# JADGardner/RENI

Hardware: AMD Instinct MI355X
Metric: directional-samples/sec (fwd+bwd), 128x256 equirect, ND=36 latent (higher is better)
Workload: dtype bf16

## Files before the change

### reni_amd/csrc/reni_capi.inc

```
#include <dlfcn.h>

#include <cmath>
#include <cstdarg>
#include <cstdio>
#include <cstdlib>
#include <atomic>
#include <cstring>
#include <mutex>
#include <new>
#include <string>
#include <vector>

#include "../../include/reni_hip.h"

struct reni_plan {
  reni_desc d;
  int F_in;
  int64_t n_params;
  int64_t n_first;
  unsigned p_off_w[reni::MAX_LAYERS + 2];
  unsigned p_off_b[reni::MAX_LAYERS + 2];
  int M_in, N_out;
  int64_t n_map_params;
  unsigned mw_off[reni::MAX_MAP_LAYERS + 1], mb_off[reni::MAX_MAP_LAYERS + 1];
  int no_persist, no_side_stream, dw1_old;
  int no_l0x;
  int env_overrides;
  size_t frag_ws_cap;
};

namespace {

thread_local std::string g_err;

std::atomic<long long> g_launches{0};
thread_local hipEvent_t g_ev_rest = nullptr;
#define RENI_LAUNCH(...) do { g_launches.fetch_add(1, std::memory_order_relaxed); hipLaunchKernelGGL(__VA_ARGS__); HIP_TRY(hipGetLastError()); } while (0)

int fail(int code, const char* fmt, ...) {
  char buf[512];
  va_list ap;
  va_start(ap, fmt);
  vsnprintf(buf, sizeof(buf), fmt, ap);
  va_end(ap);
  g_err = buf;
  return code;
}

#define HIP_TRY(expr)                                                                      \
  do {                                                                                     \
    hipError_t e_ = (expr);                                                                \
    if (e_ != hipSuccess) return fail(RENI_EHIP, "%s failed: %s", #expr, hipGetErrorString(e_)); \
  } while (0)

size_t al256(size_t x) { return (x + 255) & ~(size_t)255; }
size_t al1k(size_t x) { return (x + 1023) & ~(size_t)1023; }

bool has_persistent(int dtype, int H, int L) {
  return dtype == RENI_BF16 && H == 128 && L >= 1 && L <= 5;
}
bool has_wide(int dtype, int H, int L, uint32_t flags, bool film, bool backward) {
  if (film && (backward || L > 5)) return false;
  return dtype == RENI_BF16 && H == 256 && L >= 2 && L <= reni::MAX_LAYERS - 1 && !(flags & RENI_NEED_DW);
}
bool has_wide_train(int dtype, int H, int L, uint32_t flags, bool film) {
  if (film) return dtype == RENI_BF16 && H == 256 && L >= 2 && L <= 4;
  return dtype == RENI_BF16 && H == 256 && L >= 2 && L <= reni::MAX_LAYERS - 1 && (flags & RENI_NEED_DW);
}

int device_cus() {
  int dev = 0, n = 0;
  if (hipGetDevice(&dev) != hipSuccess) return 256;
  if (hipDeviceGetAttribute(&n, hipDeviceAttributeMultiprocessorCount, dev) != hipSuccess || n <= 0) return 256;
  return n;
}

struct GeoRt {
  int img_hid, img_hf, img_hb, bias_hid, bias_head, lds_bytes, stash_layer_bytes, nks, nrb, head_bwd_ks;
};

template <class Pol, int H>
GeoRt geo_of() {
  using G = reni::Geo<Pol, H>;
  return {G::IMG_HID, G::IMG_HF, G::IMG_HB, G::BIAS_HID, G::BIAS_HEAD, G::LDS_BYTES, G::STASH_LAYER_BYTES,
          G::NKS, G::NRB, Pol::HEAD_BWD_KS};
}

bool geo_for(const reni_plan* p, GeoRt* g) {
  const int H = p->d.hidden_features;
  if (p->d.dtype == RENI_F32) {
    if (H == 32) *g = geo_of<reni::PolF32, 32>();
    else if (H == 64) *g = geo_of<reni::PolF32, 64>();
    else if (H == 128) *g = geo_of<reni::PolF32, 128>();
    else if (H == 256) *g = geo_of<reni::PolF32, 256>();
    else return false;
  } else {
    if (H == 32) *g = geo_of<reni::PolBF16, 32>();
    else if (H == 64) *g = geo_of<reni::PolBF16, 64>();
    else if (H == 128) *g = geo_of<reni::PolBF16, 128>();
    else if (H == 256) *g = geo_of<reni::PolBF16, 256>();
    else return false;
  }
  return true;
}

struct Layout {
  int tpi, n_tiles, nwg, persist, stream, kmax, frag;
  int wide_train;
  int pdw;
  int consistent_bwd;
  size_t o_tflag, o_tlist, o_tcount, o_imgcos;
  size_t o_pcnt, o_pscan, o_plist, o_nlive;
  size_t o_skip;
  size_t o_idxc, o_Zc, o_A, o_afrag, o_xconst, o_wimg, o_stash, o_dwp, o_dA_part, o_loss_part, o_img_loss, o_stats, o_dA, o_g1, o_dw1p, o_part2, o_mcol, o_ucol, o_dfp, o_dws, o_dfr, o_runimg, o_pruns, o_prunimg, total;
  int pkmax;
  int nch, rt_chunk;
  size_t stash_per_wg, dwp_per_wg;
  unsigned fwd_off[reni::MAX_LAYERS + 2], bwd_off[reni::MAX_LAYERS + 2];
  size_t wimg_bytes;
};

Layout make_layout(const reni_plan* p, const GeoRt& g, int64_t B, int64_t P, uint32_t flags, bool backward,
                   bool allow_persist = true, int stage = 0) {
  Layout l;
  memset(&l, 0, sizeof(l));
  const int H = p->d.hidden_features, L = p->d.hidden_layers;
  l.tpi = (int)((P + 127) / 128);
  l.n_tiles = (int)(B * l.tpi);
  const bool film = p->d.conditioning == RENI_COND_FILM;
  l.wide_train = (backward && allow_persist && !p->no_persist && has_wide_train(p->d.dtype, H, L, flags, film)) ? 1 : 0;
  l.persist = (allow_persist && !p->no_persist && (has_persistent(p->d.dtype, H, L) || has_wide(p->d.dtype, H, L, flags, film, backward) || l.wide_train)) ? 1 : 0;
  l.pdw = (l.persist && !l.wide_train && (film || (flags & RENI_NEED_DW))) ? 1 : 0;
  l.consistent_bwd = (l.persist && !film && backward) ? 1 : 0;
  const int per_cu = (p->d.dtype == RENI_BF16 && !l.persist && H <= 128) ? 2 : 1;
  const int cap = device_cus() * per_cu;
  l.nwg = l.n_tiles < cap ? l.n_tiles : cap;
  if (l.pdw && l.n_tiles > cap) {
    const int rounds = (l.n_tiles + cap - 1) / cap;
    l.nwg = (l.n_tiles + rounds - 1) / rounds;
  }
  if (l.nwg < 1) l.nwg = 1;
  size_t o = 0;
  for (int st = 0; st < 2; ++st) {
    const bool mine = st == stage;
    if (mine) l.o_idxc = o;
    o += al256((size_t)B * 8);
    if (mine) l.o_Zc = o;
    o += al256((size_t)B * p->d.ndims * 3 * 4);
    if (mine) l.o_A = o;
    o += al256((size_t)B * H * 8 * 4);
    if (mine) l.o_afrag = o;
    if (l.persist) o += al256((size_t)B * (H / 32) * 1024);
    if (mine) l.o_xconst = o;
    o += al256((size_t)B * p->F_in * 4);
  }
  size_t w = 0;
  for (int i = 1; i <= L; ++i) { l.fwd_off[i] = (unsigned)w; w += al1k((size_t)g.img_hid + g.bias_hid); }
  l.fwd_off[L + 1] = (unsigned)w; w += al1k((size_t)g.img_hf + g.bias_head);
  for (int i = 1; i <= L; ++i) { l.bwd_off[i] = (unsigned)w; w += al1k((size_t)g.img_hid); }
  l.bwd_off[L + 1] = (unsigned)w; w += al1k((size_t)g.img_hb);
  l.wimg_bytes = w;
  w += 8192;
  l.o_wimg = o; o += al256(w);
  l.o_skip = o; o += 256;
  l.o_img_loss = o; o += al256((size_t)B * 16 * 4);
  l.o_stats = o; o += al256((size_t)B * 16 * 4);
  if (backward) {
    l.stash_per_wg = (size_t)(L + 1) * g.stash_layer_bytes * ((l.persist && !l.pdw && !l.wide_train) ? 2 : 1);
    l.frag = (p->d.dtype == RENI_BF16 && H == 256 && L >= 1 && (film || (flags & RENI_NEED_DW))) ? 1 : 0;
    if (p->d.dtype == RENI_F32 && H == 256 && L >= 1 && !film && (flags & RENI_NEED_DW)) l.frag = 2;
    l.o_stash = o; o += al256(l.stash_per_wg * (l.frag ? (size_t)l.n_tiles : (size_t)l.nwg));
    l.dwp_per_wg = (flags & RENI_NEED_DW) ? (size_t)(p->n_params - p->n_first) : 0;
    if (l.pdw) l.dwp_per_wg = (l.dwp_per_wg + 63) & ~(size_t)63;
    l.pkmax = ((l.n_tiles + l.nwg - 1) / l.nwg + l.tpi - 1) / l.tpi + 1;
    const size_t run_slots = (film && l.persist && !l.wide_train) ? (size_t)l.pkmax : 1;
    l.o_dwp = o; o += al256(l.dwp_per_wg * 4 * l.nwg * run_slots);
    l.o_dA_part = o; if (!l.pdw) o += al256((size_t)l.n_tiles * H * 8 * 4);
    l.o_tflag = l.o_tlist = l.o_tcount = l.o_imgcos = o;
    if (!film && !(flags & RENI_NEED_DW)) {
      l.o_tflag = o; o += al256((size_t)l.n_tiles * 4);
      l.o_tlist = o; o += al256((size_t)2 * l.n_tiles * 4);
      l.o_tcount = o; o += 256;
      l.o_imgcos = o; o += al256((size_t)B * 4);
      l.o_pcnt = o; o += al256((size_t)l.n_tiles * 4);
      l.o_pscan = o; o += al256((size_t)(l.n_tiles + 1) * 4);
      l.o_nlive = o; o += al256((size_t)B * 4);
      l.o_plist = o; o += al256((size_t)B * P * 4);
    }
    l.o_loss_part = o; o += al256((size_t)l.n_tiles * 4 * 16 * 4);
    l.o_dA = o; o += al256((size_t)B * H * 8 * 4);
    l.o_dw1p = o; if (l.pdw && (flags & RENI_NEED_DW)) o += al256((size_t)2 * l.nwg * run_slots * ((size_t)H * H + H) * 4);
    l.o_g1 = o; if (l.pdw) o += al256((size_t)((l.n_tiles + l.nwg - 1) / l.nwg) * l.nwg * (H / 16) * 4096);
    l.o_pruns = o; if (l.pdw) o += al256((size_t)l.nwg * l.pkmax * (H * 8 + 16) * 4);
    l.o_prunimg = o; if (l.pdw) o += al256((size_t)l.nwg * l.pkmax * (film ? 3 : 1) * 4);
    l.rt_chunk = reni::RT_CHUNK;
    l.nch = (l.tpi + l.rt_chunk - 1) / l.rt_chunk;
    l.o_part2 = o; o += al256((size_t)B * l.nch * (H * 8 + 16) * 4);
    l.o_mcol = o; o += al256((size_t)B * p->F_in * 4);
    l.o_ucol = o; o += al256((size_t)B * p->d.ndims * 3 * 4);
    l.o_dfp = o; if (film && !l.persist) o += al256((size_t)l.n_tiles * L * 2 * H * 4);
    const bool can = p->d.dtype == RENI_BF16 && L >= 1;
    l.stream = can && (H == 128 || H == 256) && (!l.persist || l.wide_train) && (film || (flags & RENI_NEED_DW)) ? 1 : 0;
    l.o_dws = o;
    l.o_dfr = o;
    l.o_runimg = o;
    if (l.frag == 2) o += al256((size_t)L * l.n_tiles * g.stash_layer_bytes);
    if (l.stream) {
      const int nround = (H == 256) ? 2 : 1;
      const size_t rec = (size_t)2 * (H == 256 ? 36864 : 34816);
      o += al256(l.frag ? (size_t)L * l.n_tiles * g.stash_layer_bytes + (l.wide_train ? (size_t)l.n_tiles * 2048 : 0)
                        : (size_t)L * l.n_tiles * nround * rec);
      const long long nrec = (long long)l.n_tiles * nround;
      const long long range = (nrec + l.nwg - 1) / l.nwg;
      l.kmax = (int)(range / ((long long)l.tpi * nround)) + 2;
      if (film) {
        l.o_dfr = o; o += al256((size_t)l.nwg * l.kmax * L * 2 * H * 4);
        l.o_runimg = o; o += al256((size_t)l.nwg * l.kmax * 4);
      }
    }
    if (film && l.persist && !l.wide_train) {
      l.o_dfr = o; o += al256((size_t)3 * l.nwg * l.pkmax * L * 2 * H * 4);
      l.o_runimg = l.o_prunimg;
    }
  }
  l.total = o;
  return l;
}

Layout backward_layout(const reni_plan* p, const GeoRt& g, int64_t B, int64_t P, uint32_t flags) {
  return make_layout(p, g, B, P, flags | RENI_NEED_DZ, true, true);
}

enum { PROF_FWD_BWD = 0, PROF_STATS = 1, PROF_FWD = 2, PROF_DW1 = 3, PROF_DWS = 4, PROF_COMM = 5 };
struct EvPair { hipEvent_t a, b; int kind; };
bool g_prof_on = false;
std::vector<EvPair> g_prof_pool;
size_t g_prof_used = 0;

bool prof_begin(hipStream_t s, EvPair* out, int kind) {
  if (!g_prof_on) return false;
  if (g_prof_used == g_prof_pool.size()) {
    EvPair e;
    if (hipEventCreate(&e.a) != hipSuccess || hipEventCreate(&e.b) != hipSuccess) return false;
    g_prof_pool.push_back(e);
  }
  g_prof_pool[g_prof_used].kind = kind;
  *out = g_prof_pool[g_prof_used++];
  return hipEventRecord(out->a, s) == hipSuccess;
}

template <class Go>
int timed_launch(hipStream_t s, int kind, const char* what, Go go) {
  EvPair ev;
  const bool timed = prof_begin(s, &ev, kind);
  g_launches.fetch_add(1, std::memory_order_relaxed);
  const hipError_t e = go();
  if (e != hipSuccess) return fail(RENI_EHIP, "%s launch failed: %s", what, hipGetErrorString(e));
  if (timed) HIP_TRY(hipEventRecord(ev.b, s));
  return RENI_OK;
}
int timed_launch(void (*fn)(const reni::MainArgs), int grid, int block, int lds, hipStream_t s, const reni::MainArgs& a, int kind) {
  if (lds) HIP_TRY(hipFuncSetAttribute((const void*)fn, hipFuncAttributeMaxDynamicSharedMemorySize, lds));
  return timed_launch(s, kind, "kernel", [&] { hipLaunchKernelGGL(fn, dim3(grid), dim3(block), lds, s, a); return hipGetLastError(); });
}

bool spec_head(bool need_dw, int last_linear, int act) { return need_dw && last_linear && act == RENI_ACT_TANH; }
bool train_spec(const reni::MainArgs& a, bool stats) {
  return !stats && spec_head(a.need_dw, a.last_linear, a.act) && a.loss_kind == 0 && a.out == nullptr;
}

int launch_train(const reni_plan* p, const reni::MainArgs& a, int nwg, hipStream_t s, bool stats = false, bool l0x = false) {
  using G = reni::GeoP<128>;
  const int kind = !stats ? PROF_FWD_BWD : a.target ? PROF_STATS : PROF_FWD;
  const bool film = p->d.conditioning == RENI_COND_FILM;
  if (p->d.hidden_features == 256) {
    if (film && p->d.hidden_layers > (stats ? reni::wide256_film_max_layers() : reni::wide256_film_train_max_layers()))
      return fail(RENI_EINVAL, "internal: k_reni_wide256's FiLM instances hold <= 5 (forward) / <= 4 (training form) hidden layers' tables");
    if ((a.need_dw || film) && !stats && a.gfs == nullptr) return fail(RENI_EINVAL, "internal: the training form of k_reni_wide256 needs the fragment stream");
    const int mode = film ? (stats ? 3 : 4) : stats ? 0 : a.need_dw ? 2 : 1;
    return timed_launch(s, kind, "k_reni_wide256", [&] { return reni::launch_wide256(mode, a, nwg, s); });
  }
  if (!has_persistent(p->d.dtype, p->d.hidden_features, p->d.hidden_layers))
    return fail(RENI_EUNSUPPORTED, "no persistent training kernel for this configuration");
  if (p->d.hidden_layers >= 2 && (a.fwd_off[2] - a.fwd_off[1] != G::FWD_STRIDE || a.bwd_off[2] - a.bwd_off[1] != G::BWD_STRIDE))
    return fail(RENI_EINVAL, "packed weight images are not at the stride the persistent kernels assume");
  const bool spec = train_spec(a, stats);
  const int pairs = (a.n_tiles + 1) / 2, nwg2 = nwg < pairs ? nwg : pairs;
  if (film)
    return timed_launch(s, kind, "FiLM persistent kernel", [&] { return reni::launch_train_film(stats ? 1 : spec ? 2 : 0, a, stats ? nwg2 : nwg, s); });
  if (l0x && !spec) return fail(RENI_EINVAL, "internal: the L0X form exists for the SPEC instance only");
  void (*fn)(const reni::MainArgs) = stats ? reni::k_reni_train_bf16<128, false, true>
                                     : l0x ? reni::k_reni_train_bf16<128, true, false, false, true, true>
                                     : spec ? reni::k_reni_train_bf16<128, true, false, false, true>
                                     : a.need_dw ? reni::k_reni_train_bf16<128, true> : reni::k_reni_train_bf16<128, false>;
  const int lacc = spec ? G::LACC_BYTES + (l0x ? G::L0X_TW_BYTES : 0) : 0;
#ifdef RENI_TRACE
  const int LDS = G::LDS_BYTES + lacc + 4096;
#else
  const int LDS = G::LDS_BYTES + lacc;
#endif
  if (a.need_dw && !stats) return timed_launch(fn, nwg, 256, LDS, s, a, kind);
  return timed_launch(fn, nwg2, 512, LDS, s, a, kind);
}

bool dw1_ring_plan_ok(const reni_plan* p, int64_t P) { return !p->dw1_old && p->d.conditioning != RENI_COND_FILM && P % 128 == 0; }
bool dw1_ring_call_ok(const reni::MainArgs& a) { return (((uintptr_t)a.D | (uintptr_t)(a.d_bstride * 4)) & 15) == 0; }
int dw1_slots(bool ring, int nwg) { return ring ? nwg : 2 * nwg; }
bool l0x_rows_ok(const float* base, long long s0, long long s1, long long s2) {
  if (((uintptr_t)base | (uintptr_t)(s0 * 4)) & 15) return false;
  if (s1 == 3 && s2 == 1) return true;
  return s1 == 1 && ((uintptr_t)(s2 * 4) & 15) == 0;
}
bool l0x_plan_ok(const reni_plan* p, const Layout& l, int64_t P, uint32_t flags) {
  const int L = p->d.hidden_layers;
  return l.pdw && !p->no_l0x && dw1_ring_plan_ok(p, P) && spec_head(flags & RENI_NEED_DW, p->d.last_layer_linear, p->d.output_activation) &&
         L >= 3 && (L & 1) == 1;
}
bool l0x_call_ok(const reni::MainArgs& a) {
  return dw1_ring_call_ok(a) && train_spec(a, false) && l0x_rows_ok(a.target, a.ts0, a.ts1, a.ts2) && l0x_rows_ok(a.weight, a.ws0, a.ws1, a.ws2);
}
bool side_stream_plan_ok(const reni_plan* p, const Layout& l) { return l.pdw && !p->no_side_stream; }

int launch_dw1(const reni::MainArgs& a, int nwg, bool ring, hipStream_t s, bool l0x = false) {
#ifdef RENI_TRACE_DW1
  constexpr int TRACE = 8192;
#else
  constexpr int TRACE = 0;
#endif
  if (l0x)
    return timed_launch(reni::k_reni_l0_ring<128>, nwg, reni::L0Ring::THREADS, reni::L0Ring::LDS_BYTES + TRACE, s, a, PROF_DW1);
  if (a.film != nullptr) return timed_launch(s, PROF_DW1, "k_reni_dw1 (FiLM)", [&] { return reni::launch_dw1_film(a, 2 * nwg, s); });
  if (ring)
    return timed_launch(reni::k_reni_dw1_ring<128>, nwg, reni::Dw1Ring::THREADS, reni::Dw1Ring::LDS_BYTES + TRACE, s, a, PROF_DW1);
  return timed_launch(reni::k_reni_dw1<128>, 2 * nwg, 256, 2 * reni::TS_BYTES + TRACE, s, a, PROF_DW1);
}

int reduce_partials(const float* part, size_t per_wg, int nslot, float* out, int lo, int hi, const int* valid, const reni::LayerScale& lsc,
                    hipStream_t s, int quad_H = 0) {
  if (quad_H > 0) {
    if (valid != nullptr || (per_wg & 3) || (lo & 3) || ((uintptr_t)part & 15)) return fail(RENI_EINVAL, "internal: quad-row partials need untagged, 16-byte aligned slots");
    RENI_LAUNCH(reni::k_reduce_partials_quad, dim3((unsigned)((hi - lo + reni::QUAD_BLK_WORDS - 1) / reni::QUAD_BLK_WORDS)), dim3(256), 0, s, part, per_wg, nslot, out, lo, hi, quad_H, lsc);
    return RENI_OK;
  }
  RENI_LAUNCH(reni::k_reduce_partials, dim3((unsigned)((hi - lo + 63) / 64)), dim3(256), 0, s, part, per_wg, nslot, out, lo, hi, valid, lsc);
  return RENI_OK;
}

struct SideStream { hipStream_t s; hipEvent_t ev[3]; bool ok; };
std::mutex g_side_mu;
SideStream* side_stream() {
  static SideStream tab[16];
  static std::mutex mu;
  int dev = 0;
  if (hipGetDevice(&dev) != hipSuccess || dev < 0 || dev >= 16) return nullptr;
  std::lock_guard<std::mutex> lk(mu);
  SideStream& t = tab[dev];
  if (!t.ok) {
    if (hipStreamCreateWithFlags(&t.s, hipStreamNonBlocking) != hipSuccess) return nullptr;
    for (int i = 0; i < 3; ++i)
      if (hipEventCreateWithFlags(&t.ev[i], hipEventDisableTiming) != hipSuccess) return nullptr;
    t.ok = true;
  }
  return &t;
}

int launch_main(const reni_plan* p, int mode, const reni::MainArgs& a, int nwg, hipStream_t s) {
  const int H = p->d.hidden_features;
  const bool film = p->d.conditioning == RENI_COND_FILM, f32 = p->d.dtype == RENI_F32;
  return timed_launch(s, mode == reni::MODE_FWD_BWD ? PROF_FWD_BWD : mode == reni::MODE_STATS ? PROF_STATS : PROF_FWD, "fused kernel", [&] {
    if (f32) return film ? reni::launch_film_f32(H, mode, a, nwg, s) : reni::launch_main_f32(H, mode, a, nwg, s);
    return film ? reni::launch_film_bf16(H, mode, a, nwg, s) : reni::launch_main_bf16(H, mode, a, nwg, s);
  });
}

struct DeviceGuard {
  int prev = -1;
  bool switched = false;
  int enter(const void* ptr) {
    hipPointerAttribute_t at;
    if (hipPointerGetAttributes(&at, ptr) == hipSuccess) {
      if (hipGetDevice(&prev) == hipSuccess && prev != at.device) {
        HIP_TRY(hipSetDevice(at.device));
        switched = true;
      }
    } else {
      (void)hipGetLastError();
    }
    return RENI_OK;
  }
  ~DeviceGuard() {
    if (switched) (void)hipSetDevice(prev);
  }
};

int run_prologue(const reni_plan* p, const GeoRt& g, const Layout& l, int64_t B, const float* Z,
                 const float* params, char* ws, bool backward, hipStream_t s, const int64_t* idx = nullptr,
                 const float* film_A = nullptr, int64_t n_rows = 0) {
  const int H = p->d.hidden_features, L = p->d.hidden_layers;
  const bool film = p->d.conditioning == RENI_COND_FILM;
  reni::PrepArgs pa;
  memset(&pa, 0, sizeof(pa));
  if (!film) {
    pa.idx = (const long long*)idx; pa.n_rows = (long long)n_rows; pa.Zc = (float*)(ws + l.o_Zc);
    pa.idx_copy = idx ? (long long*)(ws + l.o_idxc) : nullptr;
    pa.Z = Z; pa.W0 = params; pa.b0 = params + (size_t)H * p->F_in;
    pa.xconst = (float*)(ws + l.o_xconst); pa.A = (float*)(ws + l.o_A);
    pa.afrag = l.persist ? ws + l.o_afrag : nullptr;
    pa.afrag_scale = p->d.first_omega_0 * 0.15915494309189535f;
    pa.eq = p->d.equivariance; pa.nd = p->d.ndims; pa.F_in = p->F_in; pa.H = H;
  }

  reni::PackArgs ka;
  ka.params = params; ka.wimg = ws + l.o_wimg;
  int n = 0;
  for (int i = 1; i <= L + 1; ++i) {
    const bool head = (i == L + 1);
    reni::PackDesc d;
    d.src = p->p_off_w[i]; d.bias_src = p->p_off_b[i]; d.dst = l.fwd_off[i];
    d.M = head ? 3 : H; d.K = H; d.transposed = 0;
    d.nrb = head ? 1 : g.nrb; d.nks = g.nks;
    d.bias_n = head ? 3 : H; d.bias_n_pad = head ? 32 : H;
    d.scale = (l.persist && !head && !film) ? p->d.hidden_omega_0 * 0.15915494309189535f : 1.f;
    if (film && l.persist && H == 256 && !head) d.scale = 0.15915494309189535f;
    ka.d[n++] = d;
    if (backward) {
      d.dst = l.bwd_off[i]; d.transposed = 1;
      d.nrb = g.nrb; d.nks = head ? g.head_bwd_ks : g.nks;
      d.bias_n = 0; d.bias_n_pad = 0;
      d.scale = !l.persist ? 1.f : film ? ((i == 1 || H == 256) ? 1.f : 6.283185307179586f) : (i == 1 ? p->d.first_omega_0 : p->d.hidden_omega_0);
      if (l.consistent_bwd) d.scale = (head ? 1.f : p->d.hidden_omega_0 * 0.15915494309189535f) * 8.f;
      ka.d[n++] = d;
    }
  }
  const bool f32 = p->d.dtype == RENI_F32;
  if (!film || l.persist) {
    reni::PrologueArgs ga;
    memset(&ga, 0, sizeof(ga));
    ga.prep = pa;
    ga.prep_gy = (H + 7) / 8; ga.n_prep = (int)B * ga.prep_gy; ga.pack_gx = f32 ? 16 : 8;
    if (film) {
      ga.film_A = film_A; ga.film_afrag = ws + l.o_afrag; ga.film_scale = 0.15915494309189535f; ga.film_B = (int)B;
      ga.prep.H = H; ga.n_prep = (int)((B * H + 255) / 256);
    }
    const unsigned grid = (unsigned)(ga.n_prep + ga.pack_gx * n);
    if (f32) RENI_LAUNCH(reni::k_prologue<reni::PolF32>, dim3(grid), dim3(256), (size_t)p->F_in * 4, s, ga, ka);
    else RENI_LAUNCH(reni::k_prologue<reni::PolBF16>, dim3(grid), dim3(256), (size_t)p->F_in * 4, s, ga, ka);
    return RENI_OK;
  }
  if (f32) RENI_LAUNCH(reni::k_pack<reni::PolF32>, dim3(16, n), dim3(256), 0, s, ka);
  else RENI_LAUNCH(reni::k_pack<reni::PolBF16>, dim3(8, n), dim3(256), 0, s, ka);
  return RENI_OK;
}

void fill_main_args(reni::MainArgs& a, const reni_plan* p, const Layout& l, int64_t B, int64_t P,
                    const float* Z, const float* D, int64_t dbs, char* ws) {
  memset(&a, 0, sizeof(a));
  a.B = (int)B; a.P = (int)P; a.tiles_per_image = l.tpi; a.n_tiles = l.n_tiles;
  a.L = p->d.hidden_layers; a.last_linear = p->d.last_layer_linear; a.act = p->d.output_activation;
  a.w_first = p->d.first_omega_0; a.w_hidden = p->d.hidden_omega_0;
  a.gy_scale = 1.f;
  if (l.consistent_bwd) {
    double sc = (double)p->d.first_omega_0 / 8.0;
    for (int i = 0; i < p->d.hidden_layers; ++i) sc *= 6.283185307179586 / 8.0;
    a.gy_scale = (float)sc;
  }
  a.Z = Z; a.D = D; a.d_bstride = dbs;
  a.Apre = (const float*)(ws + l.o_A);
  a.afrag = ws + l.o_afrag;
  a.wimg = ws + l.o_wimg;
  for (int i = 0; i < reni::MAX_LAYERS + 2; ++i) {
    a.fwd_off[i] = l.fwd_off[i]; a.bwd_off[i] = l.bwd_off[i];
    a.p_off_w[i] = p->p_off_w[i] >= (unsigned)p->n_first ? p->p_off_w[i] - (unsigned)p->n_first : 0;
    a.p_off_b[i] = p->p_off_b[i] >= (unsigned)p->n_first ? p->p_off_b[i] - (unsigned)p->n_first : 0;
  }
  a.stash = ws + l.o_stash; a.stash_per_wg = l.stash_per_wg;
  a.dwp = (float*)(ws + l.o_dwp); a.dwp_per_wg = l.dwp_per_wg;
  a.dA_part = (float*)(ws + l.o_dA_part);
  a.loss_part = (float*)(ws + l.o_loss_part);
  a.g1 = ws + l.o_g1;
  a.dw1p = (float*)(ws + l.o_dw1p);
  a.stats = (const float*)(ws + l.o_stats);
  a.n_first = (unsigned)p->n_first;
  a.dfp_part = (float*)(ws + l.o_dfp);
  a.dws = l.stream ? ws + l.o_dws : nullptr;
  a.gfs = l.frag ? ws + l.o_dws : nullptr;
  a.dfr = (float*)(ws + l.o_dfr);
  a.run_image = (int*)(ws + l.o_runimg);
  a.kmax = l.kmax;
  a.pruns = (float*)(ws + l.o_pruns);
  a.prun_image = (int*)(ws + l.o_prunimg);
  a.pkmax = l.pkmax;
  a.nwg_main = l.nwg;
}

int check_common(const reni_plan* p, int64_t B, int64_t P, const void* Z, const void* D, const void* params,
                 const void* ws) {
  if (!p) return fail(RENI_EINVAL, "plan is NULL");
  if (B < 1 || P < 1) return fail(RENI_EINVAL, "B=%lld P=%lld must be >= 1", (long long)B, (long long)P);
  if (B * ((P + 127) / 128) > 0x3fffffffLL || P > 0x3fffffffLL) return fail(RENI_EINVAL, "problem too large");
  if (!Z || !D || !params) return fail(RENI_EINVAL, "Z, D and params must be non-NULL");
  if (!ws) return fail(RENI_EWORKSPACE, "workspace is NULL");
  if (((uintptr_t)ws & 255) != 0) return fail(RENI_EINVAL, "workspace must be 256-byte aligned");
  return RENI_OK;
}

struct FilmIO {
  const float* A = nullptr;
  const float* film = nullptr;
  float* dA = nullptr;
  float* dfilm = nullptr;
  const float* Zp = nullptr;
  float alpha = 0.f;
  int64_t nz = 0;
  int keep_first = 0;
};

int check_film(const reni_plan* p, const FilmIO* f, bool backward) {
  if (!p) return fail(RENI_EINVAL, "plan is NULL");
  if (p->d.conditioning != RENI_COND_FILM) return fail(RENI_EINVAL, "plan was not created with RENI_COND_FILM");
  if (!f->A) return fail(RENI_EINVAL, "A is NULL");
  if (p->d.hidden_layers > 0 && !f->film) return fail(RENI_EINVAL, "film is NULL");
  if (backward && (!f->dA || (p->d.hidden_layers > 0 && !f->dfilm))) return fail(RENI_EINVAL, "dA / dfilm is NULL");
  return RENI_OK;
}

int rccl_allreduce_inplace(void* comm, float* buf, size_t n, hipStream_t s);
int rccl_allreduce_max_i32(void* comm, int* buf, size_t n, hipStream_t s);

struct ListLayout { size_t o_hdr, o_tflag, o_tlist, o_tcount, o_imgcos, o_pcnt, o_pscan, o_nlive, o_plist, o_zstats, total; };
ListLayout make_list_layout(int64_t B, int64_t P) {
  ListLayout l;
  const size_t n_tiles = (size_t)(B * ((P + 127) / 128));
  size_t o = 0;
  l.o_hdr = o; o += 256;
  l.o_tflag = o; o += al256(n_tiles * 4);
  l.o_tlist = o; o += al256(2 * n_tiles * 4);
  l.o_tcount = o; o += 256;
  l.o_imgcos = o; o += al256((size_t)B * 4);
  l.o_pcnt = o; o += al256(n_tiles * 4);
  l.o_pscan = o; o += al256((n_tiles + 1) * 4);
  l.o_nlive = o; o += al256((size_t)B * 4);
  l.o_plist = o; o += al256((size_t)B * P * 4);
  l.o_zstats = o; o += al256((size_t)B * 16 * 4);
  l.total = o;
  return l;
}
constexpr long long LIST_MAGIC = 0x52454e494c495354ll;
struct ListDst { int *tflag, *imgcos, *tlist, *tcount, *pcnt, *pscan, *nlive, *plist; };
template <class L>
ListDst list_dst(char* base, const L& l) {
  return {(int*)(base + l.o_tflag), (int*)(base + l.o_imgcos), (int*)(base + l.o_tlist), (int*)(base + l.o_tcount),
          (int*)(base + l.o_pcnt), (int*)(base + l.o_pscan), (int*)(base + l.o_nlive), (int*)(base + l.o_plist)};
}
int build_weight_lists(const float* weight, const int64_t* wst, int64_t P, int tpi, int n_tiles, bool compact, const ListDst& d,
                       hipStream_t s) {
  RENI_LAUNCH(reni::k_tile_flags, dim3((unsigned)((n_tiles + 3) / 4)), dim3(256), 0, s, weight, (long long)wst[0], (long long)wst[1],
              (long long)wst[2], (int)P, tpi, n_tiles, d.tflag, d.imgcos, compact ? d.pcnt : (int*)nullptr);
  RENI_LAUNCH(reni::k_tile_compact, dim3(1), dim3(1024), 0, s, d.tflag, (const int*)d.imgcos, tpi, n_tiles, d.tlist, d.tlist + n_tiles,
              d.tcount, compact ? (const int*)d.pcnt : (const int*)nullptr, (int)P, d.pscan, d.nlive);
  if (compact) {
    RENI_LAUNCH(reni::k_pix_scatter, dim3((unsigned)((n_tiles + 3) / 4)), dim3(256), 0, s, weight, (long long)wst[0], (long long)wst[1],
                (long long)wst[2], (int)P, tpi, n_tiles, (const int*)d.imgcos, (const int*)d.pscan, d.plist);
  }
  return RENI_OK;
}
struct WeightLists { const char* buf; uint32_t flags; };
struct ListRecord { const void* buf; int64_t B, P; uint32_t mode; };
std::mutex g_lists_mu;
std::vector<ListRecord> g_lists;
void lists_remember(const void* buf, int64_t B, int64_t P, uint32_t mode) {
  std::lock_guard<std::mutex> lk(g_lists_mu);
  for (size_t i = 0; i < g_lists.size(); ++i)
    if (g_lists[i].buf == buf) { g_lists.erase(g_lists.begin() + (long)i); break; }
  g_lists.insert(g_lists.begin(), ListRecord{buf, B, P, mode});
  if (g_lists.size() > 64) g_lists.pop_back();
}
int lists_check(const void* buf, int64_t B, int64_t P, uint32_t mode, ListRecord* found) {
  std::lock_guard<std::mutex> lk(g_lists_mu);
  for (const ListRecord& r : g_lists)
    if (r.buf == buf) { *found = r; return (r.B == B && r.P == P && r.mode == mode) ? 0 : 2; }
  return 1;
}

struct StepFuse {
  void* comm = nullptr;
  int overlap = 0;
  float* params; float* table;
  float *m_dec, *v_dec, *m_lat, *v_lat;
  float lr, b1, b2, eps, bc1, bc2_sqrt, gscale;
  const int64_t* idx_next;
  uint32_t* state;
};

constexpr int LOSS_DOUT = 2;
struct BwdCall {
  int64_t B = 0, P = 0;
  const float *Z = nullptr, *D = nullptr, *params = nullptr;
  int64_t dbs = 0;
  const float *target = nullptr, *weight = nullptr, *dout = nullptr;
  const int64_t *ts = nullptr, *wst = nullptr;
  int loss_kind = RENI_LOSS_MSE;
  float alpha = 0.f, beta = 0.f;
  uint32_t flags = 0;
  float *out = nullptr, *loss_terms = nullptr, *dZ = nullptr, *dparams = nullptr;
  void* ws = nullptr;
  size_t ws_bytes = 0;
  void* stream = nullptr;
  const FilmIO* fio = nullptr;
  const int64_t* idx = nullptr;
  int64_t n_rows = 0;
  const StepFuse* fuse = nullptr;
  const WeightLists* lists = nullptr;
};

struct BwdPath {
  bool staged;
  int stage;
  bool use_cos;
  bool sparse;
  bool compact;
  bool cos_const;
  bool dw1_ring;
  bool l0x;
  bool part_quad;
  bool fork;
  bool early_rest;
  bool dp_early;
  bool fused_tail;
  bool fuse_on;
  bool fpers;
  bool red2;
  int n_rest;
  int n_l1;
  bool rp_in_tail;
  bool ev_rest_done;
  bool dp_early_done;
};

struct Bwd {
  const reni_plan* p;
  const BwdCall& c;
  GeoRt g; Layout l; reni::MainArgs a;
  char* ws;
  hipStream_t s, se;
  const float* Z;
  int stage_in;
  float *img_loss, *stats, *dA, *part2;
  ListDst ld;
  reni::LayerScale lsc;
  BwdPath path;
};

bool call_uses_cos(const BwdCall& c) { return c.loss_kind == RENI_LOSS_TEST && c.beta != 0.f; }

BwdPath bwd_path(const reni_plan* p, const Layout& l, const BwdCall& c, const reni::MainArgs& a, int stage_in) {
  BwdPath t{};
  const int H = p->d.hidden_features, L = p->d.hidden_layers;
  const bool need_dw = (c.flags & RENI_NEED_DW) != 0;
  t.staged = stage_in >= 0;
  t.stage = t.staged ? stage_in : 0;
  t.n_rest = (int)(p->n_params - p->n_first);
  t.n_l1 = H * H + H;
  t.use_cos = call_uses_cos(c);
  t.sparse = (c.flags & (RENI_WEIGHT_SPARSE | RENI_WEIGHT_COMPACT)) && !c.fio && !need_dw && c.loss_kind != LOSS_DOUT &&
             c.weight != nullptr && c.out == nullptr;
  t.compact = t.sparse && (c.flags & RENI_WEIGHT_COMPACT);
  t.cos_const = t.sparse && c.lists && (c.lists->flags & RENI_WEIGHT_COS_CONSTANT);
  t.dw1_ring = dw1_ring_plan_ok(p, c.P) && dw1_ring_call_ok(a);
  t.l0x = l0x_plan_ok(p, l, c.P, c.flags) && l0x_call_ok(a);
  t.part_quad = t.l0x;
  t.fork = side_stream_plan_ok(p, l) && !t.l0x && (c.fio || l.n_tiles >= 8 * l.nwg);
  t.early_rest = l.pdw && !c.fio && need_dw && L >= 1 && t.n_rest > t.n_l1;
  t.dp_early = c.fuse && c.fuse->comm && c.fuse->overlap;
  t.fused_tail = l.pdw && !c.fio;
  t.fuse_on = c.fuse && !c.fuse->comm && t.fused_tail && need_dw && (c.flags & RENI_NEED_DZ) && L >= 1;
  t.fpers = l.persist && !l.wide_train;
  t.red2 = L > 0 && t.fpers && need_dw;
  return t;
}

int bwd_validate(Bwd& x) {
  const reni_plan* p = x.p; const BwdCall& c = x.c;
  if (const int rc = c.fio ? check_film(p, c.fio, true) : RENI_OK) return rc;
  if (!c.fio && p && p->d.conditioning != RENI_COND_CONCAT) return fail(RENI_EINVAL, "FiLM plan: use the reni_film_* entry points");
  if (const int rc = check_common(p, c.B, c.P, c.fio ? c.fio->A : c.Z, c.D, c.params, c.ws)) return rc;
  if ((c.flags & RENI_NEED_DW) && !c.dparams) return fail(RENI_EINVAL, "RENI_NEED_DW set but dparams is NULL");
  if (!c.fio && (c.flags & RENI_NEED_DZ) && !c.dZ) return fail(RENI_EINVAL, "RENI_NEED_DZ set but dZ is NULL");
  if (c.loss_kind == LOSS_DOUT) {
    if (!c.dout) return fail(RENI_EINVAL, "dout is NULL");
  } else {
    if (c.loss_kind != RENI_LOSS_MSE && c.loss_kind != RENI_LOSS_TEST) return fail(RENI_EINVAL, "unknown loss_kind %d", c.loss_kind);
    if (!c.target || !c.weight || !c.ts || !c.wst) return fail(RENI_EINVAL, "target/weight (and their strides) must be non-NULL");
    if (!c.loss_terms) return fail(RENI_EINVAL, "loss_terms is NULL");
  }
  if (!geo_for(p, &x.g)) return fail(RENI_EUNSUPPORTED, "hidden_features=%d unsupported", p->d.hidden_features);
  return RENI_OK;
}

int bwd_layout(Bwd& x) {
  const BwdCall& c = x.c;
  const bool staged = c.fuse && (*c.fuse->state & 1u);
  x.stage_in = staged ? (int)((*c.fuse->state >> 1) & 1u) : -1;
  x.l = make_layout(x.p, x.g, c.B, c.P, c.flags, true, true, staged ? x.stage_in : 0);
  const Layout& l = x.l;
  if (c.ws_bytes < l.total) return fail(RENI_EWORKSPACE, "workspace too small: need %zu bytes, got %zu", l.total, c.ws_bytes);
  if (c.fuse) *c.fuse->state = 0;
  x.ws = (char*)c.ws;
  x.s = x.se = (hipStream_t)c.stream;
  x.Z = c.idx ? (const float*)(x.ws + l.o_Zc) : c.Z;
  x.img_loss = (float*)(x.ws + l.o_img_loss); x.stats = (float*)(x.ws + l.o_stats);
  x.dA = c.fio ? c.fio->dA : (float*)(x.ws + l.o_dA); x.part2 = (float*)(x.ws + l.o_part2);
  return RENI_OK;
}

void bwd_layer_scales(Bwd& x) {
  const reni_plan* p = x.p; reni::LayerScale& lsc = x.lsc;
  lsc.n_hid = p->d.hidden_features * p->d.hidden_features + p->d.hidden_features; lsc.L = p->d.hidden_layers;
  for (int i = 0; i <= reni::MAX_LAYERS; ++i) lsc.c[i] = 1.f;
  if (x.l.consistent_bwd && (x.c.flags & RENI_NEED_DW)) {
    double gy = (double)p->d.first_omega_0 / 8.0, cl = (double)p->d.hidden_omega_0 / (double)p->d.first_omega_0;
    for (int i = 0; i < p->d.hidden_layers; ++i) {
      gy *= 6.283185307179586 / 8.0;
      cl *= 8.0 / 6.283185307179586;
      lsc.c[i] = (float)cl;
    }
    lsc.c[p->d.hidden_layers] = (float)(1.0 / gy);
  }
}

void bwd_main_args(Bwd& x) {
  const BwdCall& c = x.c; reni::MainArgs& a = x.a;
  fill_main_args(a, x.p, x.l, c.B, c.P, x.Z, c.D, c.dbs, x.ws);
  if (c.fio) { a.Apre = c.fio->A; a.film = c.fio->film; a.params = c.params; a.Z = nullptr; }
  a.need_dw = (c.flags & RENI_NEED_DW) ? 1 : 0;
#ifdef RENI_DEBUG
  if (const char* e = getenv("RENI_DEBUG_MASK")) a.dbg = c.fio ? 0 : atoi(e);
#endif
#if defined(RENI_TRACE) || defined(RENI_TRACE_DW1)
  if (const char* e = getenv("RENI_TRACE_PTR")) a.trace = (long long*)strtoull(e, nullptr, 0);
#endif
  a.out = c.out; a.dout = c.dout; a.beta = c.beta;
  if (c.loss_kind != LOSS_DOUT) {
    a.target = c.target; a.ts0 = c.ts[0]; a.ts1 = c.ts[1]; a.ts2 = c.ts[2];
    a.weight = c.weight; a.ws0 = c.wst[0]; a.ws1 = c.wst[1]; a.ws2 = c.wst[2];
  }
  a.loss_kind = (c.loss_kind == LOSS_DOUT) ? LOSS_DOUT : (call_uses_cos(c) ? 1 : 0);
  x.path = bwd_path(x.p, x.l, c, a, x.stage_in);
}

int bwd_weight_lists(Bwd& x) {
  const BwdCall& c = x.c; const BwdPath& path = x.path; reni::MainArgs& a = x.a;
  if (!path.sparse) return RENI_OK;
  if (c.lists) {
    x.ld = list_dst(const_cast<char*>(c.lists->buf), make_list_layout(c.B, c.P));
  } else {
    x.ld = list_dst(x.ws, x.l);
    if (const int rc = build_weight_lists(c.weight, c.wst, c.P, x.l.tpi, x.l.n_tiles, path.compact, x.ld, x.s)) return rc;
  }
  a.tlist = x.ld.tlist; a.tcount = x.ld.tcount;
  if (path.compact) { a.plist = x.ld.plist; a.nlive = x.ld.nlive; }
  if (path.cos_const) a.stats = x.stats = (float*)(const_cast<char*>(c.lists->buf) + make_list_layout(c.B, c.P).o_zstats);
  return RENI_OK;
}

int bwd_stats_pass(Bwd& x) {
  const BwdCall& c = x.c; const Layout& l = x.l;
  if (!x.path.use_cos || x.path.cos_const) return RENI_OK;
  reni::MainArgs st = x.a;
  st.out = nullptr; st.loss_kind = 0;
  if (x.path.sparse) { st.tlist = x.a.tlist + l.n_tiles; st.tcount = x.a.tcount + 1; }
  if (const int rc = l.persist ? launch_train(x.p, st, l.nwg, x.s, true) : launch_main(x.p, reni::MODE_STATS, st, l.nwg, x.s)) return rc;
  RENI_LAUNCH(reni::k_stats_image, dim3((unsigned)c.B), dim3(256), 0, x.s, (const float*)x.a.loss_part, l.tpi, c.weight, (long long)c.wst[0],
                     (long long)c.wst[2], c.beta, x.img_loss, x.stats, (const int*)x.ld.imgcos);
  return RENI_OK;
}

struct SideJoin {
  SideStream* side = nullptr;
  hipStream_t s = nullptr;
  ~SideJoin() { if (side && hipEventRecord(side->ev[2], side->s) == hipSuccess) (void)hipStreamWaitEvent(s, side->ev[2], 0); }
};

int bwd_fork_dw1(Bwd& x, std::unique_lock<std::mutex>& side_lock, SideJoin& side_join) {
  const reni_plan* p = x.p; const BwdCall& c = x.c; const Layout& l = x.l; BwdPath& path = x.path; hipStream_t s = x.s;
  if (!l.pdw) return RENI_OK;
  SideStream* side = path.fork ? side_stream() : nullptr;
  if (side) {
    side_lock.lock();
    HIP_TRY(hipEventRecord(side->ev[0], s));
    HIP_TRY(hipStreamWaitEvent(side->s, side->ev[0], 0));
    x.se = side->s;
    side_join.side = side; side_join.s = s;
  }
  path.rp_in_tail = path.early_rest && !side && !g_ev_rest && !path.dp_early;
  if (path.early_rest && !path.rp_in_tail) {
    int rc = reduce_partials(x.a.dwp, l.dwp_per_wg, l.nwg, c.dparams + p->n_first, path.n_l1, path.n_rest, nullptr, x.lsc, s, path.part_quad ? p->d.hidden_features : 0);
    if (rc) return rc;
    if (g_ev_rest) { HIP_TRY(hipEventRecord(g_ev_rest, s)); path.ev_rest_done = true; }
    if (path.dp_early) {
      SideStream* cs = side_stream();
      if (!cs) return fail(RENI_EHIP, "no communication stream");
      if (!side_lock.owns_lock()) side_lock.lock();
      HIP_TRY(hipEventRecord(cs->ev[1], s));
      HIP_TRY(hipStreamWaitEvent(cs->s, cs->ev[1], 0));
      rc = rccl_allreduce_inplace(c.fuse->comm, c.dparams + p->n_first + path.n_l1, (size_t)(path.n_rest - path.n_l1), cs->s);
      if (rc) return rc;
      if (!side_join.side) { side_join.side = cs; side_join.s = s; }
      path.dp_early_done = true;
    }
  }
  return launch_dw1(x.a, l.nwg, path.dw1_ring, s, path.l0x);
}

int bwd_dw_consumers(Bwd& x) {
  const Layout& l = x.l; const reni::MainArgs& a = x.a; hipStream_t s = x.s;
  const int H = x.p->d.hidden_features;
  if (l.frag == 2) {
    const int lds = 4 * ((reni::Geo<reni::PolF32, 256>::T_BYTES + 1023) & ~1023);
    if (const int rc = timed_launch(reni::k_dw_frag32<256>, l.nwg, 256, lds, s, a, PROF_DWS)) return rc;
  }
  if (l.wide_train && (x.c.flags & RENI_NEED_DW)) {
    if (const int rc = timed_launch(s, PROF_DWS, "k_wide_head_dw", [&] { return reni::launch_wide_head_dw(a, l.nwg, s); })) return rc;
  }
  if (l.stream) {
    static_assert(reni::Geo<reni::PolBF16, 256>::T_BYTES_AL == 36864 && reni::Geo<reni::PolBF16, 128>::T_BYTES_AL == 34816,
                  "stream record sizes (make_layout)");
    const bool film = x.c.fio != nullptr;
    void (*fn)(const reni::MainArgs) = nullptr;
    if (H == 256) fn = film ? reni::k_dw_frag<256, true> : reni::k_dw_frag<256, false>;
    else fn = film ? reni::k_dw_stream<128, true> : reni::k_dw_stream<128, false>;
    if (film) HIP_TRY(hipMemsetAsync(a.run_image, 0xff, (size_t)l.nwg * l.kmax * 4, s));
    return timed_launch(fn, l.nwg, 256, 4 * (H == 256 ? 36864 : 34816), s, a, PROF_DWS);
  }
  return RENI_OK;
}

int bwd_image_sums(Bwd& x) {
  const BwdCall& c = x.c; const Layout& l = x.l; const reni::MainArgs& a = x.a;
  const int H = x.p->d.hidden_features;
  if (x.path.fused_tail) return RENI_OK;
  if (l.pdw) {
    RENI_LAUNCH(reni::k_reduce_runs, dim3((unsigned)c.B, c.B < 16 ? (unsigned)((H * 8 + 16 + 63) / 64) : 1u), dim3(256), 0, x.se, (const float*)a.pruns, (const int*)a.prun_image,
                       l.nwg, l.pkmax, H, l.tpi, l.n_tiles, x.dA, x.img_loss);
    return RENI_OK;
  }
  RENI_LAUNCH(reni::k_reduce_tiles_a, dim3((unsigned)c.B, (unsigned)l.nch), dim3(256), 0, x.se, (const float*)a.dA_part,
                     (const float*)a.loss_part, l.tpi, H, x.part2, 1, l.rt_chunk, (const int*)x.ld.tflag);
  RENI_LAUNCH(reni::k_reduce_tiles_b, dim3((unsigned)c.B, (unsigned)((H * 8 + 16 + 255) / 256)), dim3(256), 0, x.se, (const float*)x.part2, l.nch, H, x.dA, x.img_loss, 1);
  return RENI_OK;
}

int bwd_epilogue_film(Bwd& x) {
  const reni_plan* p = x.p; const BwdCall& c = x.c; const Layout& l = x.l; const BwdPath& path = x.path; const reni::MainArgs& a = x.a;
  hipStream_t s = x.s, se = x.se;
  const int H = p->d.hidden_features, L = p->d.hidden_layers;
  if (path.red2) {
  } else if (L > 0 && (l.stream || path.fpers)) {
    RENI_LAUNCH(reni::k_reduce_film_runs, dim3((unsigned)c.B, (unsigned)((L * H + 255) / 256)), dim3(256), 0, s, a, H,
                       path.fpers ? 3 * l.nwg * l.pkmax : l.nwg * l.kmax, c.fio->dfilm);
  } else if (L > 0) {
    RENI_LAUNCH(reni::k_reduce_film, dim3((unsigned)c.B, (unsigned)((L * 2 * H + 255) / 256)), dim3(256), 0, s,
                       (const float*)a.dfp_part, l.tpi, L * 2 * H, c.fio->dfilm);
  }
  if (c.flags & RENI_NEED_DW) {
    if (!c.fio->keep_first) HIP_TRY(hipMemsetAsync(c.dparams, 0, (size_t)p->n_first * 4, s));
    if (path.fpers) {
      const int n_l1 = path.n_l1, nslot = l.nwg * l.pkmax;
      reni::FilmReduce2 r2;
      r2.H = H; r2.nruns = 3 * l.nwg * l.pkmax; r2.B = (int)c.B; r2.gy = (L * H + 255) / 256; r2.dfilm = c.fio->dfilm;
      r2.part = a.dw1p; r2.per_wg = (size_t)n_l1; r2.nslot = 2 * nslot; r2.dparams = c.dparams + p->n_first; r2.n = n_l1;
      r2.valid = (const int*)a.prun_image + nslot;
      RENI_LAUNCH(reni::k_film_reduce2, dim3((unsigned)(r2.B * r2.gy + (n_l1 + 63) / 64)), dim3(256), 0, s, a, r2);
      if (const int rc = reduce_partials(a.dwp, l.dwp_per_wg, nslot, c.dparams + p->n_first, n_l1, path.n_rest, a.prun_image, x.lsc, se)) return rc;
    } else if (const int rc = reduce_partials(a.dwp, l.dwp_per_wg, l.nwg, c.dparams + p->n_first, 0, path.n_rest, nullptr, x.lsc, s)) {
      return rc;
    }
  }
  if (c.loss_kind != LOSS_DOUT) {
    RENI_LAUNCH(reni::k_finalize_loss, dim3(1), dim3(256), 0, se, (const float*)x.img_loss, (const float*)x.stats,
                       c.fio->Zp, (int)c.B, (int)c.P, (int)c.fio->nz, path.use_cos ? 1 : 0,
                       (c.fio->Zp != nullptr && c.loss_kind == RENI_LOSS_TEST) ? 1 : 0, c.fio->alpha, c.beta, c.loss_terms);
  }
  return RENI_OK;
}

int bwd_epilogue_concat(Bwd& x) {
  const reni_plan* p = x.p; const BwdCall& c = x.c; const Layout& l = x.l; const BwdPath& path = x.path; const reni::MainArgs& a = x.a;
  hipStream_t s = x.s, se = x.se;
  const int H = p->d.hidden_features;
  const bool need_dw = (c.flags & RENI_NEED_DW) != 0;
  reni::TailArgs t;
  t.dA = x.dA; t.W0 = c.params; t.Z = x.Z; t.xconst = (const float*)(x.ws + l.o_xconst);
  t.mcol = (float*)(x.ws + l.o_mcol); t.ucol = (float*)(x.ws + l.o_ucol);
  t.dZ = c.dZ; t.dW0 = c.dparams; t.db0 = c.dparams ? c.dparams + (size_t)H * p->F_in : nullptr;
  t.alpha2 = (c.loss_kind == RENI_LOSS_TEST) ? c.alpha : 0.f;
  t.eq = p->d.equivariance; t.nd = p->d.ndims; t.F_in = p->F_in; t.H = H; t.B = (int)c.B;
  if (!path.fuse_on && need_dw && l.pdw && p->d.hidden_layers >= 1) {
    if (const int rc = reduce_partials(a.dw1p, (size_t)path.n_l1, dw1_slots(path.dw1_ring, l.nwg), c.dparams + p->n_first, 0, path.n_l1, nullptr, x.lsc, s)) return rc;
  }
  reni::TailFusedArgs f;
  memset(&f, 0, sizeof(f));
  f.t = t;
  f.img_loss = x.img_loss; f.stats = x.stats; f.P = (int)c.P; f.nz = (int)(c.B * p->d.ndims * 3); f.has_cos = path.use_cos ? 1 : 0;
  f.has_prior = (c.loss_kind == RENI_LOSS_TEST) ? 1 : 0; f.alpha = c.alpha; f.beta = c.beta;
  f.loss_terms = (c.loss_kind != LOSS_DOUT) ? c.loss_terms : nullptr;
  f.need_dz = (c.flags & RENI_NEED_DZ) ? 1 : 0;
  f.need_dw0 = need_dw ? 1 : 0;
  f.dw0_gx = (p->F_in + 1 + 255) / 256;
  f.idx_now = path.staged ? (const long long*)c.idx : nullptr;
  f.idx_staged = path.staged ? (const long long*)(x.ws + l.o_idxc) : nullptr;
  f.skip_flag = c.fuse ? (int*)(x.ws + l.o_skip) : nullptr;
  const unsigned nb = (unsigned)((f.need_dz ? c.B : 0) + 1 + (f.need_dw0 ? f.dw0_gx * H : 0));
  if (path.fused_tail) {
    f.pruns = a.pruns; f.prun_image = a.prun_image; f.nwg = l.nwg; f.kmax = l.pkmax; f.tpi = l.tpi; f.n_tiles = l.n_tiles;
    f.dA_out = x.dA;
    const unsigned ny = f.need_dz ? (unsigned)((p->F_in + 63) / 64) : 1u;
    unsigned gx = (unsigned)c.B;
    if (path.rp_in_tail) {
      f.rp_part = a.dwp; f.rp_per_wg = l.dwp_per_wg; f.rp_nwg = l.nwg; f.rp_out = c.dparams + p->n_first; f.rp_lo = path.n_l1; f.rp_n = path.n_rest; f.rp_ls = x.lsc;
      f.rp_quad = path.part_quad ? 1 : 0;
      if (f.rp_quad && ((l.dwp_per_wg | (size_t)path.n_l1) & 3)) return fail(RENI_EINVAL, "internal: quad-row partials need 16-byte aligned slots");
      const int per_blk = f.rp_quad ? reni::QUAD_BLK_WORDS : 64;
      gx += ((unsigned)((path.n_rest - path.n_l1 + per_blk - 1) / per_blk) + ny - 1) / ny;
    }
    RENI_LAUNCH(reni::k_tail_a, dim3(gx, ny), dim3(256), (size_t)reni::tail_a_lds_bytes(H), se, f);
  } else if (c.flags & RENI_NEED_DZ) {
    RENI_LAUNCH(reni::k_tail_m, dim3((unsigned)c.B, (unsigned)((p->F_in + 63) / 64)), dim3(256), 0, se, t);
  }
  RENI_LAUNCH(reni::k_tail_b, dim3(nb), dim3(256), 0, se, f);
  if (need_dw && !path.fused_tail && path.n_rest > 0) {
    if (const int rc = reduce_partials(a.dwp, l.dwp_per_wg, l.nwg, c.dparams + p->n_first, 0, path.n_rest, nullptr, x.lsc, s)) return rc;
  }
  if (g_ev_rest && !path.ev_rest_done) HIP_TRY(hipEventRecord(g_ev_rest, s));
  return RENI_OK;
}

int bwd_fused_step(Bwd& x, SideJoin& side_join) {
  const reni_plan* p = x.p; const BwdCall& c = x.c; const Layout& l = x.l; const BwdPath& path = x.path; hipStream_t s = x.s;
  const StepFuse& fu = *c.fuse;
  if (side_join.side) {
    HIP_TRY(hipEventRecord(side_join.side->ev[2], side_join.side->s));
    HIP_TRY(hipStreamWaitEvent(s, side_join.side->ev[2], 0));
    side_join.side = nullptr;
  }
  if (fu.comm) {
    const size_t n_early = path.dp_early_done ? (size_t)(path.n_rest - path.n_l1) : 0;
    EvPair ev;
    const bool timed = prof_begin(s, &ev, PROF_COMM);
    int rc = rccl_allreduce_max_i32(fu.comm, (int*)(x.ws + l.o_skip), 1, s);
    if (rc) return rc;
    rc = rccl_allreduce_inplace(fu.comm, c.dparams, (size_t)p->n_params - n_early, s);
    if (rc) return rc;
    if (timed) HIP_TRY(hipEventRecord(ev.b, s));
  }
  reni::Adam2Args ad;
  ad.p = fu.params; ad.g = c.dparams; ad.m = fu.m_dec; ad.v = fu.v_dec; ad.n = p->n_params;
  ad.nb_dec = (int)((p->n_params + 255) / 256);
  ad.tp = fu.table; ad.g_rows = c.dZ; ad.idx = (const long long*)c.idx; ad.B = (int)c.B; ad.row_len = p->d.ndims * 3;
  ad.tm = fu.m_lat; ad.tv = fu.v_lat; ad.tn = c.n_rows * ad.row_len;
  ad.lr = fu.lr; ad.b1 = fu.b1; ad.b2 = fu.b2; ad.eps = fu.eps; ad.gscale = fu.gscale;
  ad.bc1 = fu.bc1; ad.bc2_sqrt = fu.bc2_sqrt;
  ad.skip_lo = 0; ad.skip_hi = 0; ad.l1_part = nullptr; ad.l1_per_wg = 0; ad.l1_nwg = 0; ad.nb_l1 = 0; ad.l1_scale = x.lsc.c[0];
  ad.skip_step = (const int*)(x.ws + l.o_skip);
  if (path.fuse_on) {
    ad.skip_lo = p->n_first; ad.skip_hi = p->n_first + path.n_l1;
    ad.l1_part = x.a.dw1p; ad.l1_per_wg = (size_t)path.n_l1; ad.l1_nwg = dw1_slots(path.dw1_ring, l.nwg); ad.nb_l1 = (path.n_l1 + 63) / 64;
  }
  RENI_LAUNCH(reni::k_adam2, dim3((unsigned)(ad.nb_dec + (ad.tn + 255) / 256 + ad.nb_l1)), dim3(256), 0, s, ad);
  if (fu.idx_next) {
    const Layout ln = make_layout(p, x.g, c.B, c.P, c.flags, true, true, 1 - path.stage);
    if (const int rc = run_prologue(p, x.g, ln, c.B, fu.table, fu.params, x.ws, true, s, fu.idx_next, nullptr, c.n_rows)) return rc;
    *fu.state = 1u | ((uint32_t)(1 - path.stage) << 1);
  }
  return RENI_OK;
}

int run_backward(const reni_plan* p, const BwdCall& c) {
  Bwd x{p, c};
  int rc = bwd_validate(x);
  if (rc) return rc;
  DeviceGuard dev_guard;
  if ((rc = dev_guard.enter(c.params))) return rc;
  if ((rc = bwd_layout(x))) return rc;
  bwd_layer_scales(x);
  bwd_main_args(x);
  if (!x.path.staged && (rc = run_prologue(p, x.g, x.l, c.B, c.Z, c.params, x.ws, true, x.s, c.idx, c.fio ? c.fio->A : nullptr, c.n_rows))) return rc;
  if ((rc = bwd_weight_lists(x))) return rc;
  if ((rc = bwd_stats_pass(x))) return rc;
  rc = x.l.persist ? launch_train(p, x.a, x.l.nwg, x.s, false, x.path.l0x) : launch_main(p, reni::MODE_FWD_BWD, x.a, x.l.nwg, x.s);
  if (rc) return rc;
  std::unique_lock<std::mutex> side_lock(g_side_mu, std::defer_lock);
  SideJoin side_join;
  if ((rc = bwd_fork_dw1(x, side_lock, side_join))) return rc;
  if ((rc = bwd_dw_consumers(x))) return rc;
  if ((rc = bwd_image_sums(x))) return rc;
  if (c.fio) return bwd_epilogue_film(x);
  if ((rc = bwd_epilogue_concat(x))) return rc;
  return c.fuse ? bwd_fused_step(x, side_join) : RENI_OK;
}

int64_t frag_chunk_images(const reni_plan* p, int64_t B, int64_t P, uint32_t flags) {
  GeoRt g;
  if (!p || p->d.conditioning != RENI_COND_CONCAT || p->d.hidden_features != 256 || !(flags & RENI_NEED_DW) || !geo_for(p, &g)) return B;
  const Layout l = backward_layout(p, g, 1, P, flags);
  if (!l.frag) return B;
  const size_t per_image = (size_t)l.tpi * (size_t)(2 * p->d.hidden_layers + 1) * g.stash_layer_bytes;
  int64_t bc = (int64_t)(p->frag_ws_cap / (per_image ? per_image : 1));
  if (bc < 1) bc = 1;
  if (bc >= B) return B;
  const int64_t n_chunks = (B + bc - 1) / bc;
  return (B + n_chunks - 1) / n_chunks;
}

int run_backward_chunked(const reni_plan* p, const BwdCall& c) {
  const int64_t B = c.B, P = c.P;
  const int64_t bc = (p && B >= 1 && P >= 1) ? frag_chunk_images(p, B, P, c.flags) : B;
  if (bc >= B) return run_backward(p, c);
  GeoRt g;
  geo_for(p, &g);
  DeviceGuard dev_guard;
  if (const int rcg = dev_guard.enter(c.params)) return rcg;
  const size_t core = al256(backward_layout(p, g, bc, P, c.flags).total);
  if (B % bc != 0 && backward_layout(p, g, B % bc, P, c.flags).total > core)
    return fail(RENI_EWORKSPACE, "internal: the last chunk's layout exceeds a full chunk's");
  const size_t extra = al256((size_t)p->n_params * 4) + 256;
  if (!c.ws) return fail(RENI_EWORKSPACE, "workspace is NULL");
  if (c.ws_bytes < core + extra) return fail(RENI_EWORKSPACE, "workspace too small: need %zu bytes, got %zu", core + extra, c.ws_bytes);
  float* dp_c = (float*)((char*)c.ws + core);
  float* lt_c = (float*)((char*)c.ws + core + al256((size_t)p->n_params * 4));
  hipStream_t s = (hipStream_t)c.stream;
  const int nd3 = p->d.ndims * 3;
  for (int64_t b0 = 0; b0 < B; b0 += bc) {
    const bool first = b0 == 0;
    BwdCall k = c;
    k.B = (B - b0 < bc) ? B - b0 : bc;
    if (c.idx) k.idx = c.idx + b0;
    else if (c.Z) k.Z = c.Z + b0 * nd3;
    if (c.D) k.D = c.D + b0 * c.dbs;
    if (c.target) k.target = c.target + b0 * c.ts[0];
    if (c.weight) k.weight = c.weight + b0 * c.wst[0];
    if (c.dout) k.dout = c.dout + b0 * P * 3;
    if (c.out) k.out = c.out + b0 * P * 3;
    if (c.dZ) k.dZ = c.dZ + b0 * nd3;
    if (c.loss_terms && !first) k.loss_terms = lt_c;
    if (c.dparams && !first) k.dparams = dp_c;
    k.ws_bytes = core;
    const int rc = run_backward(p, k);
    if (rc) return rc;
    if (!first) {
      if (c.dparams) {
        RENI_LAUNCH(reni::k_add_into, dim3((unsigned)((p->n_params + 255) / 256)), dim3(256), 0, s, c.dparams, (const float*)dp_c, (size_t)p->n_params);
      }
      if (c.loss_terms) {
        RENI_LAUNCH(reni::k_add_into, dim3(1), dim3(256), 0, s, c.loss_terms, (const float*)lt_c, (size_t)4);
      }
    }
  }
  return RENI_OK;
}

struct GlueLayout {
  size_t o_A, o_film, o_dA, o_dfilm, o_mapm, o_mapx, o_fo, o_dAb, o_dm, o_dly, total;
  unsigned dly_off[reni::MAX_MAP_LAYERS + 1];
};

GlueLayout make_glue_layout(const reni_plan* p, int64_t B) {
  GlueLayout g;
  memset(&g, 0, sizeof(g));
  const int H = p->d.hidden_features, L = p->d.hidden_layers, ML = p->d.mapping_layers, Hm = p->d.mapping_features;
  size_t o = 0;
  g.o_A = o; o += al256((size_t)B * H * 8 * 4);
  g.o_film = o; o += al256((size_t)B * (L > 0 ? L : 1) * 2 * H * 4);
  g.o_dA = o; o += al256((size_t)B * H * 8 * 4);
  g.o_dfilm = o; o += al256((size_t)B * (L > 0 ? L : 1) * 2 * H * 4);
  g.o_mapm = o; o += al256((size_t)B * p->M_in * 4);
  g.o_mapx = o; o += al256((size_t)B * ML * Hm * 4);
  g.o_fo = o; o += al256((size_t)B * p->N_out * 4);
  g.o_dAb = o; o += al256((size_t)B * H * 8 * 4);
  g.o_dm = o; o += al256((size_t)B * p->M_in * 4);
  g.o_dly = o;
  size_t d = 0;
  for (int i = 0; i <= ML; ++i) { g.dly_off[i] = (unsigned)d; d += (size_t)B * ((i < ML) ? Hm : p->N_out); }
  o += al256(d * 4);
  g.total = o;
  return g;
}

int check_film_model(const reni_plan* p, const void* Z, const void* map_params) {
  if (!p) return fail(RENI_EINVAL, "plan is NULL");
  if (p->d.conditioning != RENI_COND_FILM || p->d.mapping_layers < 1)
    return fail(RENI_EINVAL, "plan was not created with RENI_COND_FILM and a mapping network");
  if (!Z || !map_params) return fail(RENI_EINVAL, "Z and map_params must be non-NULL");
  return RENI_OK;
}

void fill_glue(reni::FilmGlueArgs& g, const reni_plan* p, const GlueLayout& gl, int64_t B, const float* Z,
               const float* params, const float* mparams, char* gw) {
  memset(&g, 0, sizeof(g));
  g.Z = Z; g.params = params; g.mparams = mparams;
  g.A = (float*)(gw + gl.o_A); g.film = (float*)(gw + gl.o_film);
  g.mapm = (float*)(gw + gl.o_mapm); g.mapx = (float*)(gw + gl.o_mapx); g.fo = (float*)(gw + gl.o_fo);
  g.dA = (const float*)(gw + gl.o_dA); g.dfilm = (const float*)(gw + gl.o_dfilm);
  g.dAb = (float*)(gw + gl.o_dAb); g.dly = (float*)(gw + gl.o_dly);
  g.eq = p->d.equivariance; g.nd = p->d.ndims; g.H = p->d.hidden_features; g.L = p->d.hidden_layers;
  g.F0 = p->F_in; g.M_in = p->M_in; g.Hm = p->d.mapping_features; g.ML = p->d.mapping_layers; g.N_out = p->N_out;
  g.B = (int)B;
  for (int i = 0; i <= g.ML; ++i) { g.mw_off[i] = p->mw_off[i]; g.mb_off[i] = p->mb_off[i]; g.dly_off[i] = gl.dly_off[i]; }
}

int run_film_glue_fwd(const reni::FilmGlueArgs& g, hipStream_t s) {
  const int B = g.B;
  RENI_LAUNCH(reni::k_film_minput, dim3((unsigned)B), dim3(256), 0, s, g);
  for (int i = 0; i <= g.ML; ++i) {
    const int N = (i < g.ML) ? g.Hm : g.N_out, K = (i == 0) ? g.M_in : g.Hm;
    const float* x = (i == 0) ? g.mapm : g.mapx + (size_t)(i - 1) * g.Hm;
    const int ldx = (i == 0) ? g.M_in : g.ML * g.Hm;
    float* y = (i < g.ML) ? g.mapx + (size_t)i * g.Hm : g.fo;
    const int ldy = (i < g.ML) ? g.ML * g.Hm : g.N_out;
    if ((long long)N * B >= 65536)
      RENI_LAUNCH(reni::k_film_linear<4>, dim3((unsigned)((N + 15) / 16), (unsigned)B), dim3(256), 0, s, x, ldx,
                         g.mparams + g.mw_off[i], g.mparams + g.mb_off[i], y, ldy, N, K, i < g.ML ? 1 : 0);
    else
      RENI_LAUNCH(reni::k_film_linear<1>, dim3((unsigned)((N + 3) / 4), (unsigned)B), dim3(256), 0, s, x, ldx,
                         g.mparams + g.mw_off[i], g.mparams + g.mb_off[i], y, ldy, N, K, i < g.ML ? 1 : 0);
  }
  RENI_LAUNCH(reni::k_film_fold, dim3((unsigned)B), dim3(256), 0, s, g);
  return RENI_OK;
}

size_t core_ws_bytes(const reni_plan* p, int64_t B, int64_t P, uint32_t flags) {
  GeoRt g;
  if (!geo_for(p, &g)) return 0;
  return al256(backward_layout(p, g, B, P, flags).total);
}

int film_model_backward(const reni_plan* p, const BwdCall& c, const float* mparams, float* dmparams) {
  const int64_t B = c.B;
  const uint32_t flags = c.flags;
  float* const dparams = c.dparams;
  int rc = check_film_model(p, c.Z, mparams);
  if (rc) return rc;
  if ((flags & RENI_NEED_DW) && (!dparams || !dmparams)) return fail(RENI_EINVAL, "RENI_NEED_DW set but dparams / dmap_params is NULL");
  if (!c.dZ) return fail(RENI_EINVAL, "dZ is NULL");
  if (!c.ws) return fail(RENI_EWORKSPACE, "workspace is NULL");
  const size_t core = core_ws_bytes(p, B, c.P, flags);
  const GlueLayout gl = make_glue_layout(p, B);
  if (core == 0 || c.ws_bytes < core + gl.total)
    return fail(RENI_EWORKSPACE, "workspace too small: need %zu bytes, got %zu", core + gl.total, c.ws_bytes);
  DeviceGuard dev_guard;
  rc = dev_guard.enter(c.params);
  if (rc) return rc;
  char* gw = (char*)c.ws + core;
  hipStream_t s = (hipStream_t)c.stream;
  reni::FilmGlueArgs g;
  fill_glue(g, p, gl, B, c.Z, c.params, mparams, gw);
  g.dZ = c.dZ;
  g.alpha2 = (c.loss_kind == RENI_LOSS_TEST) ? 2.f * c.alpha : 0.f;
  rc = run_film_glue_fwd(g, s);
  if (rc) return rc;
  FilmIO fio;
  fio.A = g.A; fio.film = g.film; fio.dA = (float*)(gw + gl.o_dA); fio.dfilm = (float*)(gw + gl.o_dfilm);
  fio.Zp = c.Z; fio.alpha = c.alpha; fio.nz = B * p->d.ndims * 3; fio.keep_first = 1;
  BwdCall k = c;
  k.Z = nullptr; k.dZ = nullptr; k.alpha = 0.f; k.flags = flags & RENI_NEED_DW;
  k.ws_bytes = core; k.fio = &fio;
  rc = run_backward(p, k);
  if (rc) return rc;
  RENI_LAUNCH(reni::k_film_dout, dim3((unsigned)B), dim3(256), 0, s, g);
  float* dm = (float*)(gw + gl.o_dm);
  for (int i = g.ML; i >= 0; --i) {
    const int N = (i < g.ML) ? g.Hm : g.N_out, K = (i == 0) ? g.M_in : g.Hm;
    const float* xact = (i == 0) ? nullptr : g.mapx + (size_t)(i - 1) * g.Hm;
    float* dx = (i == 0) ? dm : g.dly + gl.dly_off[i - 1];
    RENI_LAUNCH(reni::k_film_linear_t, dim3((unsigned)((K + 63) / 64), (unsigned)B), dim3(64 * reni::FLT_NG), 0, s,
                       (const float*)(g.dly + gl.dly_off[i]), N, g.mparams + g.mw_off[i], N, K, xact, g.ML * g.Hm, dx, K);
  }
  reni::FilmWgradAll wa;
  memset(&wa, 0, sizeof(wa));
  reni::FilmGrads fg;
  memset(&fg, 0, sizeof(fg));
  fg.dm = dm; fg.need_dw = (flags & RENI_NEED_DW) ? 1 : 0;
  unsigned nblk = (unsigned)B;
  if (flags & RENI_NEED_DW) {
    const int H = g.H, ML = g.ML, Hm = g.Hm;
    int nw = 0;
    for (int i = 0; i <= ML; ++i) {
      const int N = (i < ML) ? Hm : g.N_out, K = (i == 0) ? g.M_in : Hm;
      wa.delta[i] = g.dly + gl.dly_off[i]; wa.ldd[i] = N; wa.N[i] = N; wa.K[i] = K;
      wa.x[i] = (i == 0) ? g.mapm : g.mapx + (size_t)(i - 1) * Hm;
      wa.ldx[i] = (i == 0) ? g.M_in : ML * Hm;
      wa.out_w[i] = dmparams + p->mw_off[i]; wa.out_b[i] = dmparams + p->mb_off[i];
      fg.gxw[i] = (K + 1 + 255) / 256;
      nw += fg.gxw[i] * N;
      fg.blk_end[i] = nw;
    }
    wa.B = (int)B;
    fg.dW0 = dparams; fg.db0 = dparams + (size_t)H * g.F0;
    fg.gx0 = (g.F0 + 1 + 255) / 256; fg.nlayers = ML + 1;
    nblk += (unsigned)(fg.gx0 * H + nw);
  }
  RENI_LAUNCH(reni::k_film_grads, dim3(nblk), dim3(256), 0, s, g, wa, fg);
  return RENI_OK;
}

}

namespace reni {
int reni_set_error(int code, const char* msg) { return fail(code, "%s", msg); }
void note_launches(int n) { g_launches.fetch_add(n, std::memory_order_relaxed); }
}

extern "C" {

const char* reni_last_error(void) { return g_err.c_str(); }

int reni_plan_create(const reni_desc* d, reni_plan** out) {
  if (!d || !out) return fail(RENI_EINVAL, "desc/out_plan is NULL");
  *out = nullptr;
  if (d->equivariance < 0 || d->equivariance > 2) return fail(RENI_EINVAL, "equivariance %d not in {NONE,SO2,SO3}", d->equivariance);
  if (d->ndims < 1 || d->ndims > 256) return fail(RENI_EINVAL, "ndims=%d out of range", d->ndims);
  if (d->out_features != 3) return fail(RENI_EUNSUPPORTED, "out_features=%d (only 3 supported)", d->out_features);
  if (d->hidden_layers < 0 || d->hidden_layers > reni::MAX_LAYERS - 1) return fail(RENI_EUNSUPPORTED, "hidden_layers=%d unsupported", d->hidden_layers);
  if (d->hidden_features != 32 && d->hidden_features != 64 && d->hidden_features != 128 && d->hidden_features != 256)
    return fail(RENI_EUNSUPPORTED, "hidden_features=%d unsupported (32, 64, 128, 256)", d->hidden_features);
  if (d->output_activation < 0 || d->output_activation > 2) return fail(RENI_EINVAL, "output_activation %d", d->output_activation);
  if (d->dtype != RENI_F32 && d->dtype != RENI_BF16) return fail(RENI_EINVAL, "dtype %d", d->dtype);
  if (d->conditioning != RENI_COND_CONCAT && d->conditioning != RENI_COND_FILM) return fail(RENI_EINVAL, "conditioning %d", d->conditioning);
  if (d->conditioning == RENI_COND_FILM) {
    if (d->equivariance == RENI_EQ_NONE) return fail(RENI_EUNSUPPORTED, "FiLM with equivariance None is not runnable in the reference either");
    if (!d->last_layer_linear) return fail(RENI_EINVAL, "FiLM decoders end in a linear layer (RENI.py:570)");
  }
  reni_plan* p = new (std::nothrow) reni_plan;
  if (!p) return fail(RENI_EINVAL, "out of host memory");
  memset(p, 0, sizeof(*p));
  p->d = *d;
  auto env_on = [](const char* name) { const char* e = getenv(name); return e != nullptr && e[0] != '\0' && !(e[0] == '0' && e[1] == '\0'); };
  p->no_persist = env_on("RENI_NO_PERSIST");
  p->no_side_stream = env_on("RENI_NO_SIDE_STREAM");
  p->dw1_old = env_on("RENI_DW1_OLD");
  p->no_l0x = env_on("RENI_NO_L0X");
  p->frag_ws_cap = (size_t)16 << 30;
  {
    size_t fr = 0, tot = 0;
    if (hipMemGetInfo(&fr, &tot) == hipSuccess) {
      const size_t quarter = fr / 4 > ((size_t)1 << 30) ? fr / 4 : ((size_t)1 << 30);
      if (quarter < p->frag_ws_cap) p->frag_ws_cap = quarter;
    } else {
      (void)hipGetLastError();
    }
  }
  if (const char* e = getenv("RENI_FRAG_WS_CAP_MB")) { const long long mb = atoll(e); if (mb > 0) { p->frag_ws_cap = (size_t)mb << 20; p->env_overrides |= 4; } }
  p->env_overrides |= (p->no_persist ? 1 : 0) | (p->no_side_stream ? 2 : 0) | (p->dw1_old ? 8 : 0) | (p->no_l0x ? 16 : 0);
  const int nd = d->ndims, H = d->hidden_features, L = d->hidden_layers;
  if (d->conditioning == RENI_COND_FILM) {
    p->F_in = d->equivariance == RENI_EQ_SO2 ? 2 + nd : nd;
    p->d.first_omega_0 = 1.f;
  } else {
    p->F_in = d->equivariance == RENI_EQ_SO2 ? 2 * nd + nd * nd + 2 : d->equivariance == RENI_EQ_SO3 ? nd + nd * nd : 4 * nd;
  }
  size_t o = 0;
  p->p_off_w[0] = 0; o += (size_t)H * p->F_in;
  p->p_off_b[0] = (unsigned)o; o += H;
  p->n_first = (int64_t)o;
  for (int i = 1; i <= L; ++i) {
    p->p_off_w[i] = (unsigned)o; o += (size_t)H * H;
    p->p_off_b[i] = (unsigned)o; o += H;
  }
  p->p_off_w[L + 1] = (unsigned)o; o += 3 * (size_t)H;
  p->p_off_b[L + 1] = (unsigned)o; o += 3;
  p->n_params = (int64_t)o;
  if (d->conditioning == RENI_COND_FILM && d->mapping_layers > 0) {
    if (d->mapping_layers > reni::MAX_MAP_LAYERS) { delete p; return fail(RENI_EUNSUPPORTED, "mapping_layers=%d unsupported", d->mapping_layers); }
    if (d->mapping_features < 1 || d->mapping_features > 4096) { delete p; return fail(RENI_EINVAL, "mapping_features=%d", d->mapping_features); }
    p->M_in = d->equivariance == RENI_EQ_SO2 ? nd * nd + nd : nd * nd;
    p->N_out = 2 * (L + 1) * H;
    size_t m = 0;
    for (int i = 0; i <= d->mapping_layers; ++i) {
      const size_t N = (i < d->mapping_layers) ? d->mapping_features : p->N_out;
      const size_t K = (i == 0) ? p->M_in : d->mapping_features;
      p->mw_off[i] = (unsigned)m; m += N * K;
      p->mb_off[i] = (unsigned)m; m += N;
    }
    p->n_map_params = (int64_t)m;
  }
  *out = p;
  return RENI_OK;
}

void reni_plan_destroy(reni_plan* p) { delete p; }

int64_t reni_param_count(const reni_plan* p) { return p ? p->n_params : 0; }
int32_t reni_in_features(const reni_plan* p) { return p ? p->F_in : 0; }

size_t reni_workspace_bytes(const reni_plan* p, int64_t B, int64_t P, uint32_t flags) {
  GeoRt g;
  if (!p || B < 1 || P < 1 || !geo_for(p, &g)) return 0;
  size_t n = backward_layout(p, g, B, P, flags).total;
  const int64_t bc = frag_chunk_images(p, B, P, flags);
  if (bc < B) n = al256(backward_layout(p, g, bc, P, flags).total) + al256((size_t)p->n_params * 4) + 256;
  if (p->d.conditioning == RENI_COND_FILM && p->d.mapping_layers > 0) n = al256(n) + make_glue_layout(p, B).total;
  return n;
}

int reni_launch_info(const reni_plan* p, int64_t B, int64_t P, int32_t* info4) {
  GeoRt g;
  if (!p || !info4 || !geo_for(p, &g)) return fail(RENI_EINVAL, "bad argument");
  const Layout l = make_layout(p, g, B, P, RENI_NEED_DW | RENI_NEED_DZ, true);
  info4[0] = l.nwg; info4[1] = 256; info4[2] = l.persist ? -1 : g.lds_bytes; info4[3] = l.n_tiles;
  return RENI_OK;
}

int reni_path_info(const reni_plan* p, int64_t B, int64_t P, uint32_t flags, int32_t* info8) {
  GeoRt g;
  if (!p || !info8 || B < 1 || P < 1 || !geo_for(p, &g)) return fail(RENI_EINVAL, "bad argument");
  const Layout l = make_layout(p, g, B, P, flags, true);
  info8[0] = l.persist;
  info8[1] = !l.pdw ? 0 : l0x_plan_ok(p, l, P, flags) ? 3 : dw1_ring_plan_ok(p, P) ? 1 : 2;
  info8[2] = side_stream_plan_ok(p, l) ? 1 : 0;
  info8[3] = (int32_t)frag_chunk_images(p, B, P, flags);
  info8[4] = l.stream;
  info8[5] = l.frag;
  info8[6] = p->env_overrides;
  info8[7] = l.nwg;
  return RENI_OK;
}

int reni_set_grad_ready_event(void* hip_event) {
  g_ev_rest = (hipEvent_t)hip_event;
  return RENI_OK;
}

int64_t reni_launch_count(int32_t reset) {
  return reset ? g_launches.exchange(0, std::memory_order_relaxed) : g_launches.load(std::memory_order_relaxed);
}

static int forward_impl(const reni_plan* p, int64_t B, int64_t P, const float* Z, const float* D, int64_t dbs,
                        const float* params, float* out, void* ws_v, size_t ws_bytes, void* stream, const FilmIO* fio) {
  int rc = fio ? check_film(p, fio, false) : RENI_OK;
  if (rc) return rc;
  if (!fio && p && p->d.conditioning != RENI_COND_CONCAT) return fail(RENI_EINVAL, "FiLM plan: use the reni_film_* entry points");
  rc = check_common(p, B, P, fio ? fio->A : Z, D, params, ws_v);
  if (rc) return rc;
  if (!out) return fail(RENI_EINVAL, "out is NULL");
  GeoRt g;
  if (!geo_for(p, &g)) return fail(RENI_EUNSUPPORTED, "hidden_features=%d unsupported", p->d.hidden_features);
  DeviceGuard dev_guard;
  rc = dev_guard.enter(params);
  if (rc) return rc;
  const Layout l = make_layout(p, g, B, P, 0, false);
  if (ws_bytes < l.total) return fail(RENI_EWORKSPACE, "workspace too small: need %zu bytes, got %zu", l.total, ws_bytes);
  char* ws = (char*)ws_v;
  hipStream_t s = (hipStream_t)stream;
  rc = run_prologue(p, g, l, B, Z, params, ws, false, s, nullptr, fio ? fio->A : nullptr);
  if (rc) return rc;
  reni::MainArgs a;
  fill_main_args(a, p, l, B, P, Z, D, dbs, ws);
  if (fio) { a.Apre = fio->A; a.film = fio->film; a.params = params; a.Z = nullptr; }
  a.out = out;
  if (l.persist) return launch_train(p, a, l.nwg, s, true);
  return launch_main(p, reni::MODE_FWD, a, l.nwg, s);
}

int reni_forward(const reni_plan* p, int64_t B, int64_t P, const float* Z, const float* D, int64_t dbs,
                 const float* params, float* out, void* ws, size_t ws_bytes, void* stream) {
  return forward_impl(p, B, P, Z, D, dbs, params, out, ws, ws_bytes, stream, nullptr);
}

int reni_film_forward(const reni_plan* p, int64_t B, int64_t P, const float* D, int64_t dbs, const float* A,
                      const float* film, const float* params, float* out, void* ws, size_t ws_bytes, void* stream) {
  FilmIO fio;
  fio.A = A; fio.film = film;
  return forward_impl(p, B, P, nullptr, D, dbs, params, out, ws, ws_bytes, stream, &fio);
}

int reni_film_forward_loss_backward(const reni_plan* p, int64_t B, int64_t P, const float* D, int64_t dbs,
                                    const float* A, const float* film, const float* params, const float* target,
                                    const int64_t ts[3], const float* weight, const int64_t wst[3],
                                    int32_t loss_kind, float beta, uint32_t flags, float* out, float* loss_terms,
                                    float* dA, float* dfilm, float* dparams, void* ws, size_t ws_bytes,
                                    void* stream) {
  FilmIO fio;
  fio.A = A; fio.film = film; fio.dA = dA; fio.dfilm = dfilm;
  BwdCall c;
  c.B = B; c.P = P; c.D = D; c.dbs = dbs; c.params = params;
  c.target = target; c.ts = ts; c.weight = weight; c.wst = wst; c.loss_kind = loss_kind; c.beta = beta;
  c.flags = flags; c.out = out; c.loss_terms = loss_terms; c.dparams = dparams;
  c.ws = ws; c.ws_bytes = ws_bytes; c.stream = stream; c.fio = &fio;
  return run_backward(p, c);
}

int reni_film_backward(const reni_plan* p, int64_t B, int64_t P, const float* D, int64_t dbs, const float* A,
                       const float* film, const float* params, const float* dout, uint32_t flags, float* dA,
                       float* dfilm, float* dparams, void* ws, size_t ws_bytes, void* stream) {
  FilmIO fio;
  fio.A = A; fio.film = film; fio.dA = dA; fio.dfilm = dfilm;
  BwdCall c;
  c.B = B; c.P = P; c.D = D; c.dbs = dbs; c.params = params;
  c.dout = dout; c.loss_kind = LOSS_DOUT;
  c.flags = flags; c.dparams = dparams;
  c.ws = ws; c.ws_bytes = ws_bytes; c.stream = stream; c.fio = &fio;
  return run_backward(p, c);
}

int reni_forward_loss_backward(const reni_plan* p, int64_t B, int64_t P, const float* Z, const float* D,
// ... 466 lines not shown
```

### reni_amd/csrc/reni_dev_small.inc

```

DEV void reduce_film_runs_body(const MainArgs& a, int H, int nruns, float* dfilm, const int bx, const int by) {
  const float* dfr = a.dfr;
  const int* run_image = a.run_image;
  const int L = a.L;
  const float* params = a.params;
  const unsigned n_first = a.n_first;
  const unsigned* p_off_b = a.p_off_b;
  const int b = bx, i = by * 256 + threadIdx.x;
  const bool live = i < L * H;
  const int l = live ? i / H : 0, f = i - l * H;
  __shared__ int vl[1024];
  __shared__ int nv;
  float s0 = 0.f, s1 = 0.f;
  for (int base = 0; base < nruns; base += 1024) {
    const int cnt = nruns - base < 1024 ? nruns - base : 1024;
    __syncthreads();
    if (threadIdx.x < 64) {
      int c = 0;
      for (int w0 = 0; w0 < cnt; w0 += 64) {
        const int w = w0 + (int)threadIdx.x;
        const bool ok = w < cnt && run_image[base + w] == b;
        const unsigned long long m = __ballot(ok);
        if (ok) vl[c + __popcll(m & ((1ull << threadIdx.x) - 1ull))] = base + w;
        c += __popcll(m);
// ... 208 lines not shown
    film_row0(a, z, f, c);
    const float* g = a.dA + ((size_t)b * H + f) * 8;
    const float b0 = a.params[(size_t)H * a.F0 + f], fr = 15.f * fo[f] + 30.f;
    d[f] = 15.f * (g[0] * c[0] + g[1] * c[1] + g[2] * c[2] + g[3] * c[3] + g[4] * b0);
    d[nF * H + f] = g[4];
    float* o = a.dAb + ((size_t)b * H + f) * 8;
#pragma unroll
    for (int q = 0; q < 5; ++q) o[q] = fr * g[q];
    o[5] = 0.f; o[6] = 0.f; o[7] = 0.f;
  }
}

constexpr int FLT_NG = 16;
__global__ void __launch_bounds__(64 * FLT_NG) k_film_linear_t(const float* dy, int ldd, const float* W, int N, int K,
                                                              const float* xact, int ldxa, float* dx, int ldo) {
  __shared__ float red[FLT_NG][64];
  const int b = blockIdx.y, lane = threadIdx.x & 63, q = threadIdx.x >> 6;
  const int k = blockIdx.x * 64 + lane;
  const float* d = dy + (size_t)b * ldd;
  const int n0 = (int)((long long)q * N / FLT_NG), n1 = (int)((long long)(q + 1) * N / FLT_NG);
  float s[8];
#pragma unroll
  for (int u = 0; u < 8; ++u) s[u] = 0.f;
  if (k < K) {
    int n = n0;
    for (; n + 7 < n1; n += 8) {
      float w[8];
#pragma unroll
      for (int u = 0; u < 8; ++u) w[u] = W[(size_t)(n + u) * K + k];
#pragma unroll
      for (int u = 0; u < 8; ++u) s[u] += w[u] * d[n + u];
    }
    for (; n < n1; ++n) s[0] += W[(size_t)n * K + k] * d[n];
  }
  red[q][lane] = ((s[0] + s[1]) + (s[2] + s[3])) + ((s[4] + s[5]) + (s[6] + s[7]));
  __syncthreads();
  if (q == 0 && k < K) {
    float s = 0.f;
#pragma unroll
    for (int u = 0; u < FLT_NG; u += 4) s += (red[u][lane] + red[u + 1][lane]) + (red[u + 2][lane] + red[u + 3][lane]);
    if (xact != nullptr) s *= (xact[(size_t)b * ldxa + k] > 0.f) ? 1.f : 0.2f;
    dx[(size_t)b * ldo + k] = s;
  }
}

DEV void film_dz_body(const FilmGlueArgs& a, const float* dm_all, const int bx) {
  const int b = bx, nd = a.nd, H = a.H;
  const float* z = a.Z + (size_t)b * nd * 3;
  const float* dm = dm_all + (size_t)b * a.M_in;
  const float* dab = a.dAb + (size_t)b * H * 8;
  for (int t = threadIdx.x; t < nd * 3; t += 256) {
    const int k = t / 3, c = t - 3 * k;
    float v = 0.f;
    if (a.eq == 2 || c != 1) {
#pragma unroll 6
      for (int q = 0; q < nd; ++q) v += (dm[k * nd + q] + dm[q * nd + k]) * z[q * 3 + c];
      const int wcol = (a.eq == 1) ? 2 + k : k;
#pragma unroll 16
      for (int f = 0; f < H; ++f) v += dab[f * 8 + c] * a.params[(size_t)f * a.F0 + wcol];
    } else {
      v = dm[nd * nd + k];
    }
    a.dZ[(size_t)b * nd * 3 + t] = v + a.alpha2 * z[t];
  }
}

struct FilmWgradAll {
  const float* delta[MAX_MAP_LAYERS + 1]; const float* x[MAX_MAP_LAYERS + 1];
  float* out_w[MAX_MAP_LAYERS + 1]; float* out_b[MAX_MAP_LAYERS + 1];
  int ldd[MAX_MAP_LAYERS + 1], ldx[MAX_MAP_LAYERS + 1], N[MAX_MAP_LAYERS + 1], K[MAX_MAP_LAYERS + 1];
  int B;
};
DEV void film_wgrad_all_body(const FilmWgradAll& a, const int bx, const int by, const int bz) {
  const int i = bz, k = bx * 256 + threadIdx.x, n = by, K = a.K[i];
  if (n >= a.N[i] || k > K) return;
  const float* delta = a.delta[i];
  const size_t ldd = (size_t)a.ldd[i];
  float s = 0.f;
  if (k == K) {
#pragma unroll 8
    for (int b = 0; b < a.B; ++b) s += delta[(size_t)b * ldd + n];
    a.out_b[i][n] = s;
    return;
  }
  const float* x = a.x[i];
  const size_t ldx = (size_t)a.ldx[i];
#pragma unroll 8
  for (int b = 0; b < a.B; ++b) s += delta[(size_t)b * ldd + n] * x[(size_t)b * ldx + k];
  a.out_w[i][(size_t)n * K + k] = s;
}

DEV void film_w0grad_body(const FilmGlueArgs& a, float* dW0, float* db0, const int bx, const int by) {
  const int col = bx * 256 + threadIdx.x, f = by, nd = a.nd;
  if (col > a.F0) return;
  const float* g0 = a.dAb + (size_t)f * 8;
  const size_t gs = (size_t)a.H * 8;
  float s = 0.f;
  if (col == a.F0) {
#pragma unroll 8
    for (int b = 0; b < a.B; ++b) s += g0[b * gs + 4];
    db0[f] = s;
    return;
  }
  if (a.eq == 1 && col < 2) {
    const int q = (col == 0) ? 3 : 1;
#pragma unroll 8
    for (int b = 0; b < a.B; ++b) s += g0[b * gs + q];
  } else {
    const int k = (a.eq == 1) ? col - 2 : col;
    const float wy = (a.eq == 1) ? 0.f : 1.f;
#pragma unroll 8
    for (int b = 0; b < a.B; ++b) {
      const float* g = g0 + b * gs;
      const float* z = a.Z + ((size_t)b * nd + k) * 3;
      s += g[0] * z[0] + wy * g[1] * z[1] + g[2] * z[2];
    }
  }
  dW0[(size_t)f * a.F0 + col] = s;
}

struct FilmGrads { const float* dm; float* dW0; float* db0; int need_dw, gx0, nlayers; int gxw[MAX_MAP_LAYERS + 1], blk_end[MAX_MAP_LAYERS + 1]; };
__global__ void __launch_bounds__(256) k_film_grads(const FilmGlueArgs a, const FilmWgradAll wa, const FilmGrads r) {
  int i = (int)blockIdx.x;
  if (i < a.B) { film_dz_body(a, r.dm, i); return; }
  i -= a.B;
  if (!r.need_dw) return;
  const int n0 = r.gx0 * a.H;
  if (i < n0) { film_w0grad_body(a, r.dW0, r.db0, i % r.gx0, i / r.gx0); return; }
  i -= n0;
  int ly = 0, first = 0;
  while (ly < r.nlayers - 1 && i >= r.blk_end[ly]) { first = r.blk_end[ly]; ++ly; }
  i -= first;
  film_wgrad_all_body(wa, i % r.gxw[ly], i / r.gxw[ly], ly);
}

template <class Pol>
DEV void pack_body(const PackArgs& a, const int bx, const int by, const int gx) {
  const PackDesc d = a.d[by];
  const int nfrag_lanes = d.nrb * d.nks * 64;
  for (int t = bx * 256 + threadIdx.x; t < nfrag_lanes; t += gx * 256) {
    const int lane = t & 63, fr = t >> 6;
    const int ks = fr % d.nks, rb = fr / d.nks;
    const int R = 32 * rb + (lane & 31), hi = lane >> 5;
    if constexpr (Pol::BF) {
      bf16x8 o;
#pragma unroll
      for (int e = 0; e < 8; ++e) {
        const int Fk = kfeat<Pol>(ks, hi, e);
        float val = 0.f;
        if (!d.transposed) { if (R < d.M && Fk < d.K) val = a.params[d.src + (size_t)R * d.K + Fk]; }
        else { if (Fk < d.M && R < d.K) val = a.params[d.src + (size_t)Fk * d.K + R]; }
        o[e] = (__bf16)(val * d.scale);
      }
      *(bf16x8*)(a.wimg + d.dst + (size_t)t * 16) = o;
    } else {
      const int Fk = kfeat<Pol>(ks, hi, 0);
      float val = 0.f;
      if (!d.transposed) { if (R < d.M && Fk < d.K) val = a.params[d.src + (size_t)R * d.K + Fk]; }
      else { if (Fk < d.M && R < d.K) val = a.params[d.src + (size_t)Fk * d.K + R]; }
      *(float*)(a.wimg + d.dst + (size_t)t * 4) = val * d.scale;
    }
  }
  if (d.bias_n_pad > 0 && bx == 0) {
    float* bo = (float*)(a.wimg + d.dst + (size_t)nfrag_lanes * Pol::FRAGB);
    for (int i = threadIdx.x; i < d.bias_n_pad; i += 256) bo[i] = (i < d.bias_n) ? a.params[d.bias_src + i] * d.scale : 0.f;
  }
}
template <class Pol>
__global__ void __launch_bounds__(256) k_pack(const PackArgs a) { pack_body<Pol>(a, (int)blockIdx.x, (int)blockIdx.y, (int)gridDim.x); }
template __global__ void k_pack<PolF32>(const PackArgs);
template __global__ void k_pack<PolBF16>(const PackArgs);

struct PrologueArgs {
  PrepArgs prep;
  int prep_gy, n_prep, pack_gx;
  const float* film_A; char* film_afrag; float film_scale; int film_B;
};
template <class Pol>
__global__ void __launch_bounds__(256) k_prologue(const PrologueArgs a, const PackArgs ka) {
  extern __shared__ __attribute__((aligned(16))) char smem[];
  const int i = (int)blockIdx.x;
  if (i < a.n_prep && a.film_A != nullptr) afrag_from_A_body(a.film_A, a.film_afrag, a.film_scale, a.prep.H, a.film_B, i);
  else if (i < a.n_prep) prep_image_body(a.prep, i / a.prep_gy, i % a.prep_gy, smem);
  else pack_body<Pol>(ka, (i - a.n_prep) % a.pack_gx, (i - a.n_prep) / a.pack_gx, a.pack_gx);
}
template __global__ void k_prologue<PolF32>(const PrologueArgs, const PackArgs);
template __global__ void k_prologue<PolBF16>(const PrologueArgs, const PackArgs);

struct LayerScale { int n_hid, L; float c[MAX_LAYERS + 1]; };
DEV float layer_scale(const LayerScale& ls, int e) {
  int k = ls.n_hid > 0 ? e / ls.n_hid : 0;
  k = k < ls.L ? k : ls.L;
  return ls.c[k];
}
DEV void reduce_partials_body(const float* part, size_t per_wg, int nwg, float* dparams, int lo, int n, int blk, float (*red2)[64],
                              const LayerScale& ls) {
  const int lane = threadIdx.x & 63, grp = threadIdx.x >> 6;
  const int e = lo + blk * 64 + lane;
  float s[8];
#pragma unroll
  for (int q = 0; q < 8; ++q) s[q] = 0.f;
  if (e < n) {
    int q = grp;
    for (; q + 28 < nwg; q += 32) {
#pragma unroll
      for (int u = 0; u < 8; ++u) s[u] += part[(size_t)(q + 4 * u) * per_wg + e];
    }
    for (; q < nwg; q += 4) s[0] += part[(size_t)q * per_wg + e];
  }
  red2[grp][lane] = ((s[0] + s[1]) + (s[2] + s[3])) + ((s[4] + s[5]) + (s[6] + s[7]));
  __syncthreads();
  if (grp == 0 && e < n) dparams[e] = ((red2[0][lane] + red2[1][lane]) + (red2[2][lane] + red2[3][lane])) * layer_scale(ls, e);
}
DEV int quad_word_to_flat(int w, int H, int n_hid, int L) {
  const int k = w / n_hid, t = w - k * n_hid;
  if (k >= L || t >= H * H) return w;
  const int q = t >> 2, rq = q / H, col = q - rq * H;
  return k * n_hid + (4 * rq + (t & 3)) * H + col;
}
constexpr int QUAD_BLK_WORDS = 64;
template <class Emit>
DEV void reduce_partials_quad_body(const float* part, size_t per_wg, int nwg, int lo, int n, int blk, f32x4 (*red4)[64], int H, int n_hid, int L,
                                   Emit&& emit) {
  const int lane = threadIdx.x & 63, grp = threadIdx.x >> 6;
  const int l16 = lane & 15, uq = lane >> 4;
  const int w = lo + blk * QUAD_BLK_WORDS + 4 * l16;
  f32x4 s0 = f32x4{0.f, 0.f, 0.f, 0.f}, s1 = s0;
  if (w < n) {
    const float* const p = part + w + (size_t)(8 * uq) * per_wg;
    int q = grp;
    for (; q + 124 < nwg; q += 128) {
      f32x4 v[8];
#pragma unroll
      for (int k = 0; k < 4; ++k) {
        v[2 * k] = *(const f32x4*)(p + (size_t)(q + 32 * k) * per_wg);
        v[2 * k + 1] = *(const f32x4*)(p + (size_t)(q + 32 * k + 4) * per_wg);
      }
      __builtin_amdgcn_sched_barrier(0);
#pragma unroll
      for (int k = 0; k < 4; ++k) { s0 += v[2 * k]; s1 += v[2 * k + 1]; }
    }
    for (; q + 28 < nwg; q += 32) {
      const f32x4 a = *(const f32x4*)(p + (size_t)q * per_wg), b = *(const f32x4*)(p + (size_t)(q + 4) * per_wg);
      s0 += a; s1 += b;
    }
    if (uq == 0) {
      for (; q < nwg; q += 4) s0 += *(const f32x4*)(p + (size_t)q * per_wg);
    }
  }
  red4[grp][lane] = s0 + s1;
  __syncthreads();
  if (threadIdx.x < QUAD_BLK_WORDS) {
    const int m = (int)threadIdx.x >> 2, c = (int)threadIdx.x & 3, ww = lo + blk * QUAD_BLK_WORDS + (int)threadIdx.x;
    float g[4];
#pragma unroll
    for (int gg = 0; gg < 4; ++gg) g[gg] = (red4[gg][m][c] + red4[gg][16 + m][c]) + (red4[gg][32 + m][c] + red4[gg][48 + m][c]);
    if (ww < n) emit(quad_word_to_flat(ww, H, n_hid, L), (g[0] + g[1]) + (g[2] + g[3]));
  }
}
DEV void reduce_partials_valid_body(const float* part, size_t per_wg, int nwg, float* dparams, int lo, int n, const int* valid, int blk) {
  __shared__ int vl[2048];
  __shared__ int nv;
  __shared__ float red[4][64];
  const int lane = threadIdx.x & 63, grp = threadIdx.x >> 6;
  const int e = lo + blk * 64 + lane;
  float s[8];
#pragma unroll
  for (int q = 0; q < 8; ++q) s[q] = 0.f;
  for (int base = 0; base < nwg; base += 2048) {
    const int cnt = nwg - base < 2048 ? nwg - base : 2048;
    __syncthreads();
    if (threadIdx.x < 64) {
      int c = 0;
      for (int w0 = 0; w0 < cnt; w0 += 64) {
        const int w = w0 + (int)threadIdx.x;
        const bool ok = w < cnt && valid[base + w] >= 0;
        const unsigned long long m = __ballot(ok);
        if (ok) vl[c + __popcll(m & ((1ull << threadIdx.x) - 1ull))] = base + w;
        c += __popcll(m);
      }
      if (threadIdx.x == 0) nv = c;
    }
    __syncthreads();
    if (e < n) {
      const int m = nv;
      int q = grp;
      for (; q + 28 < m; q += 32) {
#pragma unroll
        for (int u = 0; u < 8; ++u) s[u] += part[(size_t)vl[q + 4 * u] * per_wg + e];
      }
      for (; q < m; q += 4) s[0] += part[(size_t)vl[q] * per_wg + e];
    }
  }
  red[grp][lane] = ((s[0] + s[1]) + (s[2] + s[3])) + ((s[4] + s[5]) + (s[6] + s[7]));
  __syncthreads();
  if (grp == 0 && e < n) dparams[e] = (red[0][lane] + red[1][lane]) + (red[2][lane] + red[3][lane]);
}
__global__ void __launch_bounds__(256) k_reduce_partials(const float* part, size_t per_wg, int nwg,
                                                          float* dparams, int lo, int n, const int* valid, const LayerScale ls) {
  const int i = lo + blockIdx.x * 256 + threadIdx.x;
  if (valid != nullptr) {
    reduce_partials_valid_body(part, per_wg, nwg, dparams, lo, n, valid, (int)blockIdx.x);
    return;
  }
  (void)i;
  __shared__ float red2[4][64];
  reduce_partials_body(part, per_wg, nwg, dparams, lo, n, (int)blockIdx.x, red2, ls);
// ... 764 lines not shown
```

### reni_amd/csrc/reni_dev_train.inc

```

constexpr int TAIL_RB2 = 1, TAIL_DWDX = 1, TAIL_DWDX_A = 1;
#ifdef RENI_TU_TRAIN_FILM
constexpr int TAIL_RB1 = 5;
#else
constexpr int TAIL_RB1 = 3;
#endif
template <int N, class F>
DEV void static_for_down(F&& f) {
  if constexpr (N >= 1) {
    f(std::integral_constant<int, N>{});
    static_for_down<N - 1>(f);
  }
}

template <int I, int N, class F>
DEV void static_for_up(F&& f) {
  if constexpr (I < N) {
    f(std::integral_constant<int, I>{});
    static_for_up<I + 1, N>(f);
  }
}

template <int H>
struct GeoP {
  using G = Geo<PolBF16, H>;
  static constexpr int WBSZ = ((G::IMG_HID + G::BIAS_HID + 3071) / 3072 * 3072 + 1023) & ~1023;
  static constexpr int TSZ = 128 * 256;
  static constexpr int HFSZ = (G::IMG_HF + G::BIAS_HEAD + 3071) / 3072 * 3072, HBSZ = (G::IMG_HB + 3071) / 3072 * 3072;
  static constexpr int DASZ = H * 8 * 4;
  static constexpr int LDS_BYTES = 2 * WBSZ + 2 * TSZ + 2048 + HFSZ + HBSZ + DASZ;
  static constexpr int LACC_BYTES = 128 * 16;
  static constexpr int L0X_TW_BYTES = 1536;
  static constexpr unsigned FWD_STRIDE = (G::IMG_HID + G::BIAS_HID + 1023) & ~1023, BWD_STRIDE = (G::IMG_HID + 1023) & ~1023;
};


template <int BYTES>
DEV void dma_image(char* lds_dst, const char* gsrc, int wave, int lane16) {
  constexpr int NP = (BYTES + 1023) / 1024;
  const unsigned dst = __builtin_amdgcn_readfirstlane((unsigned)(size_t)lds_dst);
#pragma unroll
  for (int pi = 0; pi < (NP + 3) / 4; ++pi) {
    const int piece = pi * 4 + wave;
    if (piece < NP) glds16(gsrc + piece * 1024, (unsigned)lane16, dst + piece * 1024);
  }
}

struct DmaJob {
  const char* src;
  unsigned lane_off;
  unsigned dst;
  int ng;
};
DEV void glds16x3(const char* gsrc_uniform, unsigned lane_off, unsigned lds_dst_uniform) {
  unsigned keep;
  asm volatile("s_mov_b32 %0, m0\n\ts_mov_b32 m0, %3\n\ts_nop 0\n\t"
               "global_load_lds_dwordx4 %1, %2\n\t"
               "global_load_lds_dwordx4 %1, %2 offset:1024\n\t"
               "global_load_lds_dwordx4 %1, %2 offset:2048\n\t"
               "s_mov_b32 m0, %0"
               : "=&s"(keep) : "v"(lane_off), "s"(gsrc_uniform), "s"(lds_dst_uniform) : "memory");
}
DEV void dma_group(const DmaJob& jb, int g, int wave, int nwaves = 4) {
  const int gi = g * nwaves + wave;
  if (gi < jb.ng) glds16x3(jb.src + gi * 3072, jb.lane_off, jb.dst + gi * 3072);
}
constexpr int DMA_GROUPS = 3;
struct NoFill { DEV void operator()(int) const {} DEV void operator()(int, int) const {} };

template <int NKS>
DEV f32x16 gemm_rb(const char* wb, int rbo, const bf16x8 (&bop)[NKS], f32x16 acc, int lane) {
  constexpr int D = NKS;
  bf16x8 a[D];
#pragma unroll
  for (int ks = 0; ks < D; ++ks) a[ks] = *(const bf16x8*)(wb + ((rbo * NKS + ks) * 64 + lane) * 16);
#pragma unroll
  for (int ks = 0; ks < NKS; ++ks) {
    const bf16x8 ak = a[ks % D];
    if (ks + D < NKS) a[ks % D] = *(const bf16x8*)(wb + ((rbo * NKS + ks + D) * 64 + lane) * 16);
    if (ks == NKS - 1) mfma_bf16_pin_v<true, NKS == 1>(acc, ak, bop[ks]);
    else if (ks == 0) mfma_bf16_pin_v<false, true>(acc, ak, bop[ks]);
    else mfma_bf16_pin_v<false, false>(acc, ak, bop[ks]);
  }
  return acc;
}

template <int NKS, class F = NoFill, bool ZERO = false>
DEV void gemm_rb2(const char* wb, int rbo0, const bf16x8 (&bop)[NKS], f32x16& acc0, f32x16& acc1, int lane,
                  const F& fill = F()) {
  auto fa = [&](int r, int ks) { return *(const bf16x8*)(wb + (((rbo0 + r) * NKS + ks) * 64 + lane) * 16); };
  constexpr int D = NKS >= 2 ? 2 : 1;
  bf16x8 q0[D], q1[D];
#pragma unroll
  for (int d = 0; d < D; ++d) { q0[d] = fa(0, d); q1[d] = fa(1, d); }
#pragma unroll
  for (int ks = 0; ks < NKS; ++ks) {
    const bf16x8 a0 = q0[ks % D], a1 = q1[ks % D];
    if (ks + D < NKS) { q0[ks % D] = fa(0, ks + D); q1[ks % D] = fa(1, ks + D); }
    if (ks == 0 && ZERO) mfma_bf16_zero_v<false>(acc0, a0, bop[ks]);
    else if (ks == 0) mfma_bf16_pin_v<false, true>(acc0, a0, bop[ks]);
    else mfma_bf16_pin_v<false, false>(acc0, a0, bop[ks]);
    fill(ks, 0);
    __builtin_amdgcn_sched_barrier(0);
    if (ks == 0 && ZERO) mfma_bf16_zero_v<NKS == 1>(acc1, a1, bop[ks]);
    else if (ks == NKS - 1) mfma_bf16_pin_v<true, NKS == 1, NKS == 1 ? -1 : TAIL_RB2>(acc1, a1, bop[ks]);
    else if (ks == 0) mfma_bf16_pin_v<false, true>(acc1, a1, bop[ks]);
    else mfma_bf16_pin_v<false, false>(acc1, a1, bop[ks]);
    fill(ks, 1);
    __builtin_amdgcn_sched_barrier(0);
  }
}

template <int NKS, class F = NoFill, bool ZERO = false>
DEV void gemm_rb1(const char* wb, int rbo, const bf16x8 (&bop)[NKS], f32x16& acc, int lane, const F& fill = F()) {
  auto fa = [&](int ks) { return *(const bf16x8*)(wb + ((rbo * NKS + ks) * 64 + lane) * 16); };
  constexpr int D = NKS >= 4 ? 3 : NKS >= 2 ? 2 : 1;
  bf16x8 q[D];
#pragma unroll
  for (int d = 0; d < D; ++d) q[d] = fa(d);
#pragma unroll
  for (int ks = 0; ks < NKS; ++ks) {
    const bf16x8 a = q[ks % D];
    if (ks + D < NKS) q[ks % D] = fa(ks + D);
    if (ks == 0 && ZERO) mfma_bf16_zero_v<NKS == 1>(acc, a, bop[ks]);
    else if (ks == NKS - 1) mfma_bf16_pin_v<true, NKS == 1, NKS == 1 ? -1 : TAIL_RB1>(acc, a, bop[ks]);
    else if (ks == 0) mfma_bf16_pin_v<false, true>(acc, a, bop[ks]);
    else mfma_bf16_pin_v<false, false>(acc, a, bop[ks]);
    fill(ks);
    __builtin_amdgcn_sched_barrier(0);
  }
}

template <int H, int NB>
DEV void t_write_b(char* T, const bf16x8 (&xb)[2 * NB], int wave, int hi, int j) {
  using G = Geo<PolBF16, H>;
#pragma unroll
  for (int rb = 0; rb < NB; ++rb)
#pragma unroll
    for (int r = 0; r < 16; ++r)
      *(__bf16*)(T + (32 * rb + rowmap(r, hi)) * G::T_ROWB + (wave * 32 + j) * 2) = xb[2 * rb + (r >> 3)][r & 7];
}


typedef short s16x4 __attribute__((ext_vector_type(4)));
typedef unsigned int u32x2 __attribute__((ext_vector_type(2)));
constexpr int TS_BYTES = 128 * 256;
DEV int tswz(int s) { return ((s & 1) << 4) | ((s & 2) << 2) | ((s & 1) << 2) | ((s & 8) >> 2) | ((s & 4) >> 2); }

DEV unsigned lds_u32(const char* p) { return (unsigned)(size_t)p; }
typedef __attribute__((address_space(3))) u32x2* lds_u32x2_p;

template <int NB>
DEV void ts_write(char* T, const bf16x8 (&xb)[2 * NB], int s, int hi) {
  unsigned base = lds_u32(T) + s * 256 + ((tswz(s) ^ hi) << 3);
  asm volatile("" : "+v"(base));
#pragma unroll
  for (int rb = 0; rb < NB; ++rb)
#pragma unroll
    for (int u = 0; u < 4; ++u) {
      const u32x4 w = __builtin_bit_cast(u32x4, xb[2 * rb + (u >> 1)]);
      const u32x2 h = (u & 1) ? u32x2{w[2], w[3]} : u32x2{w[0], w[1]};
      *(lds_u32x2_p)(uintptr_t)(base ^ (unsigned)((8 * rb + 2 * u) << 3)) = h;
    }
}
DEV unsigned ts_write_base(char* T, int s, int hi) {
  unsigned base = lds_u32(T) + s * 256 + ((tswz(s) ^ hi) << 3);
  asm volatile("" : "+v"(base));
  return base;
}
DEV void ts_write_chunk(unsigned base, bf16x8 v, int c) {
  const u32x4 w = __builtin_bit_cast(u32x4, v);
  const int rb = c >> 1, u0 = 2 * (c & 1);
  *(lds_u32x2_p)(uintptr_t)(base ^ (unsigned)((8 * rb + 2 * u0) << 3)) = u32x2{w[0], w[1]};
  *(lds_u32x2_p)(uintptr_t)(base ^ (unsigned)((8 * rb + 2 * (u0 + 1)) << 3)) = u32x2{w[2], w[3]};
}
struct TsBase { unsigned q[2]; };
DEV TsBase ts_base(const char* T, int lane) {
  const int khi = lane >> 5, g = (lane >> 4) & 1, u = lane & 15;
  const int s0 = (u >> 2) & 1, s1 = (u >> 3) & 1;
  TsBase b;
#pragma unroll
  for (int q = 0; q < 2; ++q) {
    const int x = (s0 << 4) | (s1 << 3) | (s0 << 2) | (khi << 1) | q;
    const int phys = ((4 * g + (u & 3)) ^ (x & 7)) | ((x >> 3) << 3);
    b.q[q] = lds_u32(T) + (8 * khi + 4 * q + (u >> 2)) * 256 + phys * 8;
  }
  asm volatile("" : "+v"(b.q[0]), "+v"(b.q[1]));
  return b;
}
DEV bf16x8 ts_read(const TsBase& b, int blk, int ks) {
  typedef __attribute__((address_space(3))) s16x4* lp;
  const s16x4 lo = __builtin_amdgcn_ds_read_tr16_b64_v4i16((lp)(uintptr_t)((b.q[0] ^ (unsigned)(blk << 6)) + (unsigned)(ks * 4096)));
  const s16x4 hi = __builtin_amdgcn_ds_read_tr16_b64_v4i16((lp)(uintptr_t)((b.q[1] ^ (unsigned)(blk << 6)) + (unsigned)(ks * 4096)));
  typedef short s16x8 __attribute__((ext_vector_type(8)));
  const s16x8 v = {lo[0], lo[1], lo[2], lo[3], hi[0], hi[1], hi[2], hi[3]};
  return __builtin_bit_cast(bf16x8, v);
}

template <int NBC, int KIND, int PIN, class F = NoFill>
DEV void dw_gemm_s(const char* TA, const char* TB, f32x16 (&acc)[NBC], float& dbacc, int wave, int lane,
                   const F& fill = F()) {
  const TsBase bA = ts_base(TA, lane), bB = ts_base(TB, lane);
  constexpr int PF = NBC == 1 ? 4 : 1;
  bf16x8 ra[PF], rbf[PF][NBC];
#pragma unroll
  for (int d = 0; d < PF; ++d) {
    ra[d] = ts_read(bA, wave, d);
#pragma unroll
    for (int m = 0; m < NBC; ++m) rbf[d][m] = ts_read(bB, m, d);
  }
#pragma unroll
  for (int ks = 0; ks < 8; ++ks) {
    const bf16x8 fa = ra[ks % PF];
    bf16x8 fbv[NBC];
#pragma unroll
    for (int m = 0; m < NBC; ++m) fbv[m] = rbf[ks % PF][m];
    if (ks + PF < 8) {
      ra[ks % PF] = ts_read(bA, wave, ks + PF);
#pragma unroll
      for (int m = 0; m < NBC; ++m) rbf[ks % PF][m] = ts_read(bB, m, ks + PF);
    }
#pragma unroll
    for (int m = 0; m < NBC; ++m) {
      const bf16x8 fb = fbv[m];
      if constexpr (PIN == 2) {
        if (ks == 7 && m == NBC - 1) mfma_bf16_pin_v<true, false>(acc[m], fa, fb);
        else if (ks == 0) mfma_bf16_zero_v<false>(acc[m], fa, fb);
        else mfma_bf16_pin_v<false, false>(acc[m], fa, fb);
      } else {
        acc[m] = PolBF16::mfma(fa, fb, acc[m]);
      }
      if (KIND == DW_HEAD && m == 0 && wave == 0) dbacc = frag_sum<PolBF16>(fb, dbacc);
    }
    if (KIND == DW_HIDDEN) dbacc = frag_sum<PolBF16>(fa, dbacc);
    fill(ks);
    if constexpr (PIN != 0) __builtin_amdgcn_sched_barrier(0);
  }
}

template <int H, bool DW, bool STATS = false, bool FILM = false, bool SPEC = false, bool L0X = false>
__global__ void __launch_bounds__(DW ? 256 : 512, 1) k_reni_train_bf16(const MainArgs a) {
  static_assert(!(DW && STATS), "the statistics instance has no backward pass");
  static_assert(!SPEC || DW, "SPEC is an instance of the training kernel");
  static_assert(!L0X || (SPEC && !FILM), "L0X is a form of the concat SPEC instance");
  static_assert(!FILM || DW || STATS, "FiLM: the training instance serves the frozen decoder too");
  using Pol = PolBF16;
  using G = Geo<Pol, H>;
  using GP = GeoP<H>;
  static_assert(H == 128, "sample-major transposition image is laid out for H = 128");
  constexpr int NRB = G::NRB, NKS = G::NKS;
  constexpr int MYB_H = (NRB * NRB + 3) / 4;
  constexpr int PMAX = 5;
  extern __shared__ __attribute__((aligned(1024))) char smem[];
  char* const TA = smem + 2 * GP::WBSZ;
  char* const TB = TA + GP::TSZ;
  float* const hdw = (float*)(TB + GP::TSZ);
  char* const HF = TB + GP::TSZ + 2048;
  char* const HB = HF + GP::HFSZ;
  float* const dAacc = (float*)(HB + GP::HBSZ);
  constexpr int FT_FLOATS = (PMAX + 1) * 2 * H;
  float* const ftab_base = FILM ? (DW ? dAacc + H * 8 : (float*)TB) : nullptr;

#ifdef RENI_TRACE
  unsigned long long* const trace_lds = (unsigned long long*)(smem + GP::LDS_BYTES + GP::LACC_BYTES);
  int trace_n = 0;
#ifndef RENI_TRACE_WAVE
#define RENI_TRACE_WAVE 0
#endif
  const bool trace_on = a.trace != nullptr && blockIdx.x == 0 && __builtin_amdgcn_readfirstlane(threadIdx.x >> 6) == RENI_TRACE_WAVE;
#define TRACE(tag) do { __builtin_amdgcn_sched_barrier(0); if (trace_on && trace_n < 500) { trace_lds[trace_n] = ((unsigned long long)__builtin_amdgcn_s_memtime() & 0xffffffffffffull) | ((unsigned long long)(tag) << 48); ++trace_n; } __builtin_amdgcn_sched_barrier(0); } while (0)
#define TRACE_FLUSH(slot, tag) do { __builtin_amdgcn_sched_barrier(0); if (trace_on) trace_lds[slot] = ((unsigned long long)__builtin_amdgcn_s_memtime() & 0xffffffffffffull) | ((unsigned long long)(tag) << 48); __builtin_amdgcn_sched_barrier(0); } while (0)
#else
#define TRACE(tag) do {} while (0)
#define TRACE_FLUSH(slot, tag) do {} while (0)
#endif
  const int tid = threadIdx.x;
  constexpr int NW = DW ? 4 : 8, NHALF = NW / 4, DG = DW ? DMA_GROUPS : 2;
  const int wave = __builtin_amdgcn_readfirstlane(tid >> 6);
  const int wq = wave & 3, half = wave >> 2;
  const int lane = tid & 63, hi = lane >> 5, j = lane & 31;
  char* const stash = a.stash + (size_t)blockIdx.x * (G::STASH_LAYER_BYTES * (DW ? 1 : 2));
  const size_t stash_layer_stride = (size_t)gridDim.x * (G::STASH_LAYER_BYTES * (DW ? 1 : 2));
  float* const dwp = a.dwp + (size_t)blockIdx.x * a.dwp_per_wg;
  const int L = a.L;
  const int nstep = L0X ? 2 * L + 1 : 2 * L + 2;
  int wpar_v = 0;

  static_assert(MYB_H == 4, "sixteen AGPR tiles = 4 layers x 4 column blocks");
  if constexpr (DW) agpr_zero_seq(std::make_integer_sequence<int, 256>{});
  float pdb[PMAX];
#pragma unroll
  for (int l = 0; l < PMAX; ++l) pdb[l] = 0.f;
  if constexpr (DW) {
    for (int i = tid; i < 3 * H + 32; i += 256) hdw[i] = 0.f;
    for (int i = tid; i < H * 8; i += 256) dAacc[i] = 0.f;
  }
  constexpr bool LACC = SPEC;
  f32x4* const lacc = (f32x4*)(dAacc + H * 8 + (FILM ? FT_FLOATS : 0));
  float* const hdb = hdw + 3 * H + 16;
  float* const loss_run = hdw + 3 * H + 8;
  if constexpr (DW) { if (tid < 4) loss_run[tid] = 0.f; }
  if constexpr (LACC) { if (tid < 128) lacc[tid] = f32x4{0.f, 0.f, 0.f, 0.f}; }
  const int act = SPEC ? 1 : a.act;
  const bool last_linear = SPEC ? true : (a.last_linear != 0);
  const int loss_kind = SPEC ? 0 : a.loss_kind;
  float* const out_img = SPEC ? nullptr : a.out;
  const float inv3p = 1.0f / (3.0f * (float)a.P);
  int run_k = 0;

  int lane16 = lane * 16, tid16 = tid * 16;
  const char* wimg_f1 = a.wimg + a.fwd_off[1];
  const char* wimg_b1 = a.wimg + a.bwd_off[1];
  auto make_job = [&](int k, bool next_tile = false) -> DmaJob {
    if (k == L || k == L + 1) k = STATS ? 0 : L + 2;
    const int wpar = L0X ? (wpar_v ^ (next_tile ? 1 : 0)) : 0;
    const unsigned dst = __builtin_amdgcn_readfirstlane((unsigned)(size_t)(smem + ((k ^ wpar) & 1) * GP::WBSZ));
    const char* img;
    int bytes;
    if constexpr (FILM && DW && !SPEC) {
      if (k < L) { img = a.wimg + a.fwd_off[k + 1]; bytes = G::IMG_HID + G::BIAS_HID; }
      else { img = a.wimg + a.bwd_off[2 * L + 2 - k]; bytes = G::IMG_HID; }
    } else {
      if (k < L) { img = wimg_f1 + (unsigned)k * GP::FWD_STRIDE; bytes = G::IMG_HID + G::BIAS_HID; }
      else { img = wimg_b1 + (unsigned)(2 * L + 1 - k) * GP::BWD_STRIDE; bytes = G::IMG_HID; }
    }
    return DmaJob{img, (unsigned)lane16, dst, (bytes + 3071) / 3072};
  };
  auto issue_dma = [&](int k) {
    const DmaJob jb = make_job(k);
#pragma unroll
    for (int g = 0; g < DG; ++g) dma_group(jb, g, wave, NW);
  };
  issue_dma(0);
  {
    const DmaJob jf{a.wimg + a.fwd_off[L + 1], (unsigned)lane16, (unsigned)__builtin_amdgcn_readfirstlane((unsigned)(size_t)HF), GP::HFSZ / 3072};
    const DmaJob jb{a.wimg + a.bwd_off[L + 1], (unsigned)lane16, (unsigned)__builtin_amdgcn_readfirstlane((unsigned)(size_t)HB), GP::HBSZ / 3072};
#pragma unroll
    for (int g = 0; g < DG; ++g) { dma_group(jf, g, wave, NW); dma_group(jb, g, wave, NW); }
  }
  dma_wait();

  constexpr bool CONTIG = DW || FILM;
  const int* const tlist = CONTIG ? nullptr : a.tlist;
  const int n_walk = (!CONTIG && tlist != nullptr) ? __builtin_amdgcn_readfirstlane(*a.tcount) : a.n_tiles;
  auto tile_at = [&](int i) -> int { return tlist != nullptr ? __builtin_amdgcn_readfirstlane(tlist[i]) : i; };
  const int t_first = CONTIG ? (int)((long long)blockIdx.x * a.n_tiles / gridDim.x) : (int)blockIdx.x * NHALF;
  const int t_stop = CONTIG ? (int)((long long)(blockIdx.x + 1) * a.n_tiles / gridDim.x) : n_walk;
  const int t_step = CONTIG ? NHALF : (int)gridDim.x * NHALF;
  if (!CONTIG && t_first >= t_stop) return;
  int ft_img0 = -1, ft_img1 = -1;
  bf16x8 aop0_n[NRB];
  float d3_n[3];
  constexpr bool INCR = DW && (!FILM || SPEC);
  int cur_b = 0, cur_tin = 0;
  if constexpr (INCR) { cur_b = t_first / a.tiles_per_image; cur_tin = t_first - cur_b * a.tiles_per_image; }
  int tile_pref = 0;
  int p_pref = 0;
  const int* const plist = CONTIG ? nullptr : a.plist;
  auto prefetch_tile = [&](int t0, int inc_b = -1, int inc_tin = 0) {
    const int tl = CONTIG ? (t0 + half < t_stop ? t0 + half : t_stop - 1) : tile_at(t0 + half < t_stop ? t0 + half : t_stop - 1);
    if constexpr (!CONTIG) tile_pref = tl;
    const int bi = (INCR && inc_b >= 0) ? inc_b : tl / a.tiles_per_image;
    int pi = ((INCR && inc_b >= 0) ? inc_tin : (tl - bi * a.tiles_per_image)) * 128 + wq * 32 + j;
    if constexpr (!CONTIG) {
      if (plist != nullptr) {
        const bool pv = pi < __builtin_amdgcn_readfirstlane(a.nlive[bi]);
        pi = pv ? plist[(size_t)bi * a.P + pi] : a.P;
      }
      p_pref = pi;
    }
    const float* dp = a.D + (size_t)bi * a.d_bstride + (size_t)((t0 + half < t_stop && pi < a.P) ? pi : 0) * 3;
#pragma unroll
    for (int rbo = 0; rbo < NRB; ++rbo) aop0_n[rbo] = *(const bf16x8*)(a.afrag + ((size_t)(bi * NRB + rbo) * 64) * 16 + (unsigned)(lane * 16));
    d3_n[0] = dp[0]; d3_n[1] = dp[1]; d3_n[2] = dp[2];
  };
  constexpr bool PREF = !(FILM && DW) || SPEC;
  if constexpr (PREF) prefetch_tile(t_first);
  char* const dnext = (char*)dAacc;
  auto dma_dirs = [&](int bi, int tin) {
    const char* src = (const char*)(a.D + (size_t)bi * a.d_bstride + (size_t)(tin * 128 + wq * 32) * 3);
    const unsigned dst = __builtin_amdgcn_readfirstlane((unsigned)(size_t)(dnext + wq * 384));
    if (lane < 24) glds16(src, (unsigned)lane16, dst);
  };
  char* const tnext = dnext + 1536;
  char* const wnext = (char*)lacc + GP::LACC_BYTES;
  const bool t_planar = a.ts1 == 1, w_planar = a.ws1 == 1;
  auto dma_rows = [&](const float* base, long long s0, long long s2, bool planar, char* buf, int bi, int tin) {
    if (planar) {
#pragma unroll
      for (int c = 0; c < 3; ++c) {
        const char* src = (const char*)(base + (size_t)bi * s0 + (size_t)c * s2 + (size_t)(tin * 128 + wq * 32));
        const unsigned dst = __builtin_amdgcn_readfirstlane((unsigned)(size_t)(buf + (c * 128 + wq * 32) * 4));
        if (lane < 8) glds16(src, (unsigned)lane16, dst);
      }
    } else {
      const char* src = (const char*)(base + (size_t)bi * s0 + (size_t)(tin * 128 + wq * 32) * 3);
      const unsigned dst = __builtin_amdgcn_readfirstlane((unsigned)(size_t)(buf + wq * 384));
      if (lane < 24) glds16(src, (unsigned)lane16, dst);
    }
  };
  auto dma_tw = [&](int bi, int tin) {
    dma_rows(a.target, a.ts0, a.ts2, t_planar, tnext, bi, tin);
    dma_rows(a.weight, a.ws0, a.ws2, w_planar, wnext, bi, tin);
  };
  if constexpr (L0X) { dma_dirs(cur_b, cur_tin); dma_tw(cur_b, cur_tin); dma_wait(); }
#pragma unroll 1
  for (int tile0 = t_first; tile0 < t_stop; tile0 += t_step) {
    const bool last_tile = tile0 + t_step >= t_stop;
    asm volatile("" : "+v"(lane16), "+v"(tid16));
    const int jx = L0X ? (int)(((unsigned)lane16 >> 4) & 31u) : j, hix = L0X ? (int)((unsigned)lane16 >> 9) : hi;
    const int j = jx, hi = hix;
    TRACE(1);
    const bool tvalid = tile0 + half < t_stop;
    const int tile = CONTIG ? (tvalid ? tile0 + half : t_stop - 1) : tile_pref;
    const int b = INCR ? cur_b : tile / a.tiles_per_image;
    const bool wrap = cur_tin + 1 == a.tiles_per_image;
    const int nxt_b = wrap ? cur_b + 1 : cur_b, nxt_tin = wrap ? 0 : cur_tin + 1;
    if constexpr (FILM) {
      const int i0 = INCR ? cur_b : tile0 / a.tiles_per_image;
      const int i1 = (tile0 + 1 < t_stop ? tile0 + 1 : t_stop - 1) / a.tiles_per_image;
      if (i0 != ft_img0 || (NHALF == 2 && i1 != ft_img1)) {
        __syncthreads();
        int t0 = tid;
        asm volatile("" : "+v"(t0));
        for (int hsel = 0; hsel < NHALF; ++hsel) {
          const int im = hsel == 0 ? i0 : i1;
          float* ft = ftab_base + hsel * FT_FLOATS;
#pragma unroll 1
          for (int i = t0; i < 2 * H; i += NW * 64) ft[i] = (i < H) ? 1.f : 0.f;
          const float* src = a.film + (size_t)im * L * 2 * H;
#pragma unroll 1
          for (int i = t0; i < L * 2 * H; i += NW * 64) ft[2 * H + i] = src[i] * 0.15915494309189535f;
        }
        __syncthreads();
        ft_img0 = i0; ft_img1 = i1;
      }
    }
    unsigned ft_off = FILM ? (unsigned)(half * FT_FLOATS) : 0u;
    if constexpr (FILM) asm volatile("" : "+s"(ft_off));
    const float* const ftab = FILM ? ftab_base + ft_off : nullptr;
    const int p = CONTIG ? (INCR ? cur_tin : (tile - b * a.tiles_per_image)) * 128 + wq * 32 + j : p_pref;
    const bool valid = tvalid && p < a.P;
    auto load_d = [&](float (&d3)[3]) {
      const float* dp = a.D + (size_t)b * a.d_bstride + (size_t)(valid ? p : 0) * 3;
      d3[0] = dp[0]; d3[1] = dp[1]; d3[2] = dp[2];
    };
    auto split_x = [&](const float (&d3)[3], __bf16 (&xh)[5], __bf16 (&xl)[4]) {
      float x[5];
      x[0] = d3[0]; x[1] = d3[1]; x[2] = d3[2];
      x[3] = sqrtf(x[0] * x[0] + x[2] * x[2]);
      x[4] = 1.f;
#pragma unroll
      for (int k = 0; k < 5; ++k) xh[k] = (__bf16)x[k];
#pragma unroll
      for (int k = 0; k < 4; ++k) xl[k] = (__bf16)(x[k] - (float)xh[k]);
    };
    bf16x8 aop0[NRB];
#pragma unroll
    for (int rbo = 0; rbo < NRB; ++rbo) {
      if constexpr (PREF) aop0[rbo] = aop0_n[rbo];
      else aop0[rbo] = *(const bf16x8*)(a.afrag + ((size_t)(b * NRB + rbo) * 64) * 16 + (unsigned)lane16);
    }
    bf16x8 bop0;
    {
      float d3[3] = {d3_n[0], d3_n[1], d3_n[2]};
      if constexpr (!PREF) load_d(d3);
      if constexpr (L0X) {
        typedef __attribute__((address_space(3))) float* lfp;
        const lfp dl = (lfp)(uintptr_t)(lds_u32(dnext) + (unsigned)((wq * 32 + j) * 12));
        d3[0] = dl[0]; d3[1] = dl[1]; d3[2] = dl[2];
      }
      __bf16 xh[5], xl[4];
      split_x(d3, xh, xl);
      if (hi == 0) { bop0[0] = xh[0]; bop0[1] = xh[1]; bop0[2] = xh[2]; bop0[3] = xh[3]; bop0[4] = xh[4]; bop0[5] = xh[0]; bop0[6] = xh[1]; bop0[7] = xh[2]; }
      else { bop0[0] = xh[3]; bop0[1] = xh[4]; bop0[2] = xl[0]; bop0[3] = xl[1]; bop0[4] = xl[2]; bop0[5] = xl[3]; bop0[6] = (__bf16)0.f; bop0[7] = (__bf16)0.f; }
    }
    asm volatile("" : "+v"(bop0) :: "memory");
    const bool owner = valid && (hi == 0);
    float tgt[3] = {0.f, 0.f, 0.f}, swt[3] = {0.f, 0.f, 0.f};
    if (!L0X && owner && (!STATS || a.target != nullptr)) {
      if (loss_kind == 2) {
#pragma unroll
        for (int c = 0; c < 3; ++c) tgt[c] = a.dout[((size_t)b * a.P + p) * 3 + c];
      } else {
#pragma unroll
        for (int c = 0; c < 3; ++c) {
          tgt[c] = a.target[(size_t)b * a.ts0 + (size_t)p * a.ts1 + (size_t)c * a.ts2];
          swt[c] = a.weight[(size_t)b * a.ws0 + (size_t)p * a.ws1 + (size_t)c * a.ws2];
        }
      }
    }

    bf16x8 hb[NKS];
    u32x4 wA[NRB * 2], wB[NRB * 2];
    constexpr bool KEEP1 = !STATS && !FILM;
    u32x4 qst[NRB * 2];

    auto red = [](float x) { if constexpr (!FILM) return x; else return __builtin_amdgcn_fractf(x); };
    struct FilmQ { f32x4 fq, ph; };
    auto act_pair = [&](const f32x16& acc, int rb, int q, bf16x8 (&dst)[NKS], const float* tp = nullptr, FilmQ* fs = nullptr) {
      float v0 = acc[2 * q], v1 = acc[2 * q + 1];
      if constexpr (FILM) {
        if ((q & 1) == 0) {
          const float* f4 = tp + 32 * rb + 4 * q + 4 * hi;
          fs->fq = *(const f32x4*)f4;
          fs->ph = *(const f32x4*)(f4 + H);
        }
        v0 = __builtin_fmaf(v0, fs->fq[2 * (q & 1)], fs->ph[2 * (q & 1)]);
        v1 = __builtin_fmaf(v1, fs->fq[2 * (q & 1) + 1], fs->ph[2 * (q & 1) + 1]);
      }
      const float t0 = red(v0), t1 = red(v1);
      unsigned pk, s1, ph;
      asm volatile("v_sin_f32 %0, %3\n\tv_sin_f32 %1, %4\n\tv_cvt_pk_f16_f32 %2, %3, %4\n\tv_cvt_pk_bf16_f32 %0, %0, %1"
                   : "=&v"(pk), "=&v"(s1), "=&v"(ph) : "v"(t0), "v"(t1));
      u32x4 d4 = __builtin_bit_cast(u32x4, dst[2 * rb + (q >> 2)]);
      d4[q & 3] = pk;
      dst[2 * rb + (q >> 2)] = __builtin_bit_cast(bf16x8, d4);
      qst[2 * rb + (q >> 2)][q & 3] = ph;
    };
    auto activate = [&](const f32x16& acc, int rb, auto sc, bf16x8 (&dst)[NKS], const float* tp = nullptr) {
      if constexpr (!FILM) {
#pragma unroll
        for (int q = 0; q < 8; ++q) act_pair(acc, rb, q, dst);
        return;
      }
      float th[16];
#pragma unroll
      for (int r = 0; r < 16; ++r) {
        float v = acc[r];
        if constexpr (FILM) { if (tp != nullptr) { const int f = 32 * rb + rowmap(r, hi); v = __builtin_fmaf(v, tp[f], tp[H + f]); } }
        if constexpr (std::is_same<decltype(sc), float>::value) th[r] = red(v * sc);
        else th[r] = red(v);
        dst[2 * rb + (r >> 3)][r & 7] = (__bf16)__builtin_amdgcn_sinf(th[r]);
      }
#pragma unroll
      for (int c = 0; c < 2; ++c)
#pragma unroll
        for (int d = 0; d < 4; ++d) qst[2 * rb + c][d] = phase_pack(th[8 * c + 2 * d], th[8 * c + 2 * d + 1]);
    };
    typedef __attribute__((address_space(1))) char gchar;
    typedef __attribute__((address_space(1))) u32x4 gu32x4;
    struct StashAt { gchar* base; unsigned off; };
    auto stash_mid = [&](int layer) -> StashAt {
      const unsigned off = ((unsigned)tid16 & 0x1f0u) | (((unsigned)tid16 >> 9) << 12);
      unsigned long long base = (unsigned long long)(stash + (size_t)layer * stash_layer_stride);
      base = ((unsigned long long)(unsigned)__builtin_amdgcn_readfirstlane((int)(base >> 32)) << 32) |
             (unsigned)__builtin_amdgcn_readfirstlane((int)(unsigned)base);
      asm volatile("" : "+s"(base));
      return StashAt{(gchar*)base, off};
    };
    auto stash_chunk = [&](const StashAt& sa, int c) -> gu32x4* { return (gu32x4*)(sa.base + (size_t)(sa.off + (unsigned)(c * 512))); };

    f32x16 pa, pb;
    {
#pragma unroll
      for (int rbo = 0; rbo < NRB; ++rbo) {
        f32x16 acc;
        mfma_bf16_zero_v<true>(acc, aop0[rbo], bop0);
        if (rbo == 2) pa = acc;
        else if (rbo == 3) pb = acc;
        else activate(acc, rbo, std::true_type{}, hb);
      }
    }

    TRACE(2);
    auto fwd_layer = [&](int l, bf16x8 (&hin)[NKS], bf16x8 (&hout)[NKS], f32x16& pia, f32x16& pib, f32x16& poa, f32x16& pob) {
      if (l == 1) {
        asm volatile("" ::: "memory");
        __builtin_amdgcn_s_barrier();
        asm volatile("" ::: "memory");
      } else {
        dma_wait();
        __syncthreads();
      }
      TRACE(10 + l);
      DmaJob jb = make_job(l);
      if (STATS && l == L && ((L & 1) || last_tile)) jb.ng = 0;
      const StashAt sl_prev = stash_mid(l - 1);
      const float* const tp_prev = FILM ? ftab + (l - 1) * 2 * H : nullptr;
      const float* const tp_cur = FILM ? ftab + l * 2 * H : nullptr;
      FilmQ fs0, fsA, fsB;
      const char* wb = smem + (((l - 1) ^ (L0X ? wpar_v : 0)) & 1) * GP::WBSZ;
      const float* bias = (const float*)(wb + G::IMG_HID);
      auto fill = [&](int ks, int part) {
        if (part == 0 && ks < DG) dma_group(jb, ks, wave, NW);
        constexpr bool SPREAD = !FILM || SPEC;
        if constexpr (SPREAD) {
          const int sl = 2 * ks + part;
          if (sl < 8) act_pair(pia, 2, sl, hin, tp_prev, &fsA);
          if (sl < 8 && (sl & 1) == 0) act_pair(pib, 3, sl >> 1, hin, tp_prev, &fsB);
          if (sl >= 8 && sl < 12) act_pair(pib, 3, sl - 4, hin, tp_prev, &fsB);
          if (sl >= 12) {
#pragma unroll
            for (int r = 0; r < 8; ++r) {
              if (sl < 14) poa[8 * (sl - 12) + r] = bias[64 + rowmap(8 * (sl - 12) + r, hi)];
              else pob[8 * (sl - 14) + r] = bias[96 + rowmap(8 * (sl - 14) + r, hi)];
            }
          }
        } else {
        if (part == 1 && ks >= 4) {
#pragma unroll
          for (int r = 0; r < 8; ++r) {
            if (ks < 6) poa[8 * (ks - 4) + r] = bias[64 + rowmap(8 * (ks - 4) + r, hi)];
            else pob[8 * (ks - 6) + r] = bias[96 + rowmap(8 * (ks - 6) + r, hi)];
          }
        }
        if (ks < 4) {
          FilmQ fs;
          if (part == 0) { act_pair(pia, 2, 2 * ks, hin, tp_prev, &fs); act_pair(pia, 2, 2 * ks + 1, hin, tp_prev, &fs); }
          else { act_pair(pib, 3, 2 * ks, hin, tp_prev, &fs); act_pair(pib, 3, 2 * ks + 1, hin, tp_prev, &fs); }
        }
        }
        if constexpr (!STATS) {
          if constexpr (KEEP1) {
            if (part == 1) {
              if (l == L) wB[ks] = qst[ks];
              else if (!(l == 1 && L >= 2)) *stash_chunk(sl_prev, ks) = qst[ks];
            }
          } else if constexpr (!FILM) { if (part == 1 && !(l == 1 && L >= 2)) *stash_chunk(sl_prev, ks) = qst[ks]; }
          else { if (part == 1) *stash_chunk(sl_prev, ks) = qst[ks]; }
        }
      };
      f32x16 acc0, acc1;
#pragma unroll
      for (int r = 0; r < 16; ++r) {
        acc0[r] = bias[rowmap(r, hi)];
        acc1[r] = bias[32 + rowmap(r, hi)];
      }
      TRACE(100 + l);
      gemm_rb2<NKS>(wb, 0, hin, acc0, acc1, lane, fill);
      TRACE(110 + l);
      gemm_rb2<NKS>(wb, 2, hin, poa, pob, lane, [&](int ks, int part) {
        if constexpr (FILM) {
          if ((ks & 1) == 0) act_pair(acc0, 0, ks + part, hout, tp_cur, &fs0);
          else act_pair(acc1, 1, ks - 1 + part, hout, tp_cur, &fs0);
        } else {
          if (part == 0) act_pair(acc0, 0, ks, hout); else act_pair(acc1, 1, ks, hout);
        }
      });
      TRACE(120 + l);
      if (STATS && l == L && (L & 1) && !last_tile) {
        __syncthreads();
        issue_dma(0);
      }
    };
    {
      bf16x8 hb2[NKS];
      f32x16 pa2, pb2;
      int l = 1;
#pragma unroll 1
      for (; l + 1 <= L; l += 2) {
        fwd_layer(l, hb, hb2, pa, pb, pa2, pb2);
        fwd_layer(l + 1, hb2, hb, pa2, pb2, pa, pb);
      }
      if (l == L) {
        fwd_layer(L, hb, hb2, pa, pb, pa2, pb2);
        pa = pa2; pb = pb2;
#pragma unroll
        for (int ks = 0; ks < NKS / 2; ++ks) hb[ks] = hb2[ks];
      }
    }
    {
      activate(pa, 2, std::true_type{}, hb, FILM ? ftab + L * 2 * H : nullptr);
      activate(pb, 3, std::true_type{}, hb, FILM ? ftab + L * 2 * H : nullptr);
      asm volatile("s_nop 1" : "+v"(hb[4]), "+v"(hb[5]), "+v"(hb[6]), "+v"(hb[7]));
    }

    TRACE(3);
    float ylin[3], outv[3];
    {
      TRACE(4);
      const char* wb = HF;
      const float* bias = (const float*)(wb + G::IMG_HF);
      f32x16 acc;
#pragma unroll
      for (int r = 0; r < 16; ++r) acc[r] = bias[rowmap(r, hi)];
      acc = gemm_rb<NKS>(wb, 0, hb, acc, lane);
#pragma unroll
      for (int c = 0; c < 3; ++c) {
        ylin[c] = acc[c];
        const float yv = last_linear ? ylin[c] : sin_f32(a.w_hidden * ylin[c]);
        const float y2 = yv * 2.885390081777927f;
        const float e2 = __builtin_amdgcn_exp2f(y2 > 60.f ? 60.f : y2);
        outv[c] = (act == 1) ? (1.f - 2.f * __builtin_amdgcn_rcpf(e2 + 1.f)) : (act == 2) ? expf(yv) : yv;
      }
    }
    if (out_img != nullptr && owner) {
      float* op = out_img + ((size_t)b * a.P + p) * 3;
      op[0] = outv[0]; op[1] = outv[1]; op[2] = outv[2];
    }

    TRACE(5);
    if constexpr (STATS) {
      if (a.target != nullptr) {
        float s9[9];
#pragma unroll
        for (int c = 0; c < 3; ++c) {
          const float t = owner ? tgt[c] : 0.f, o = owner ? outv[c] : 0.f;
          s9[c] = o * t; s9[3 + c] = o * o; s9[6 + c] = t * t;
        }
#pragma unroll
        for (int q = 0; q < 9; ++q) {
          const float sq = wave_sum(s9[q]);
          if (lane == 0 && tvalid) a.loss_part[((size_t)tile * 4 + wq) * 16 + 1 + q] = sq;
        }
      }
      dma_wait();
      if constexpr (PREF) prefetch_tile(tile0 + t_step);
      continue;
    }
    if constexpr (L0X) {
      typedef __attribute__((address_space(3))) float* lfp;
      const int sl = wq * 32 + j;
      const unsigned to = lds_u32(tnext) + (unsigned)(t_planar ? sl * 4 : sl * 12), ts = t_planar ? 512u : 4u;
      const unsigned wo = lds_u32(wnext) + (unsigned)(w_planar ? sl * 4 : sl * 12), wsx = w_planar ? 512u : 4u;
      if (owner) {
#pragma unroll
        for (int c = 0; c < 3; ++c) {
          tgt[c] = *(lfp)(uintptr_t)(to + (unsigned)c * ts);
          swt[c] = *(lfp)(uintptr_t)(wo + (unsigned)c * wsx);
        }
      }
    }
    float gy[3] = {0.f, 0.f, 0.f};
    {
      float e = 0.f;
      if (loss_kind == 2) {
#pragma unroll
        for (int c = 0; c < 3; ++c) gy[c] = tgt[c];
      } else {
#pragma unroll
        for (int c = 0; c < 3; ++c) {
          if (owner) {
            const float t = tgt[c], sw = swt[c];
            const float d = outv[c] - t;
            e += sw * d * d;
            gy[c] = 2.f * sw * d * inv3p;
            if (loss_kind == 1) {
              const float cA = a.stats[(size_t)b * 16 + c], cB = a.stats[(size_t)b * 16 + 4 + c];
              gy[c] += cA * t - cB * outv[c];
            }
          }
        }
      }
      if constexpr (!LACC) {
        const float es = wave_sum(e);
        if constexpr (DW) { if (lane == 0) loss_run[wave] += es; }
        else if (lane == 0 && tvalid) a.loss_part[((size_t)tile * 4 + wq) * 16] = es;
      }
#pragma unroll
      for (int c = 0; c < 3; ++c) {
        if (act == 1) gy[c] *= (1.f - outv[c] * outv[c]);
        else if (act == 2) gy[c] *= outv[c];
        if (!last_linear) gy[c] *= a.w_hidden * cos_f32(a.w_hidden * ylin[c]);
        if (!owner) gy[c] = 0.f;
        if constexpr (!FILM) gy[c] *= a.gy_scale;
      }
      if constexpr (LACC) {
        if (hi == 0) {
          f32x4 v = lacc[wave * 32 + jx];
          v[0] += e; v[1] += gy[0]; v[2] += gy[1]; v[3] += gy[2];
          lacc[wave * 32 + jx] = v;
        }
      }
    }

    TRACE(6);
    bf16x8 gA[NKS], gB[NKS];
    auto dx_rowblock_g = [&](const char* wb, int rbi, auto& bop, auto nks_tag, const auto& fill, const u32x4 (&w)[NRB * 2], bf16x8 (&ghb)[NKS],
                             const float* tq = nullptr) {
      constexpr int NK = decltype(nks_tag)::value;
      f32x16 acc0, acc1;
      gemm_rb2<NK, std::decay_t<decltype(fill)>, true>(wb, rbi, bop, acc0, acc1, lane, fill);
#pragma unroll
      for (int r = 0; r < 16; r += 2) {
        float r0, r1;
        cos_mul2(w[2 * rbi + (r >> 3)][(r & 7) >> 1], acc0[r], acc0[r + 1], r0, r1);
        if constexpr (FILM) { const int f = 32 * rbi + rowmap(r, hi); r0 *= tq[f]; r1 *= tq[f + 1]; }
        ghb[2 * rbi + (r >> 3)][r & 7] = (__bf16)r0;
        ghb[2 * rbi + (r >> 3)][(r & 7) + 1] = (__bf16)r1;
        cos_mul2(w[2 * rbi + 2 + (r >> 3)][(r & 7) >> 1], acc1[r], acc1[r + 1], r0, r1);
        if constexpr (FILM) { const int f = 32 * (rbi + 1) + rowmap(r, hi); r0 *= tq[f]; r1 *= tq[f + 1]; }
        ghb[2 * rbi + 2 + (r >> 3)][r & 7] = (__bf16)r0;
        ghb[2 * rbi + 2 + (r >> 3)][(r & 7) + 1] = (__bf16)r1;
      }
    };
    auto epi_pair = [&](const f32x16& acc, int rb, int q, const u32x4 (&w)[NRB * 2], bf16x8 (&ghb)[NKS], const float* tq, f32x4& fq4) {
      const int r = 2 * q;
      if constexpr (!FILM) {
        u32x4 d4 = __builtin_bit_cast(u32x4, ghb[2 * rb + (r >> 3)]);
        d4[(r & 7) >> 1] = cos_mul2_pk(w[2 * rb + (r >> 3)][(r & 7) >> 1], acc[r], acc[r + 1]);
        ghb[2 * rb + (r >> 3)] = __builtin_bit_cast(bf16x8, d4);
        return;
      }
      float r0, r1;
      cos_mul2(w[2 * rb + (r >> 3)][(r & 7) >> 1], acc[r], acc[r + 1], r0, r1);
      if constexpr (FILM) {
        if ((q & 1) == 0) fq4 = *(const f32x4*)(tq + 32 * rb + 4 * q + 4 * hi);
        r0 *= fq4[2 * (q & 1)];
        r1 *= fq4[2 * (q & 1) + 1];
      }
      ghb[2 * rb + (r >> 3)][r & 7] = (__bf16)r0;
      ghb[2 * rb + (r >> 3)][(r & 7) + 1] = (__bf16)r1;
    };
    auto dx_layer = [&](const char* wb, const bf16x8 (&bop)[NKS], const auto& fillv, const u32x4 (&w)[NRB * 2], bf16x8 (&ghb)[NKS],
                        const float* tq = nullptr, int ltag = 0) {
      f32x16 a0, a1, a2, a3;
      f32x4 fq4;
      auto f0 = [&](int ks) { fillv(0, ks); };
      gemm_rb1<NKS, decltype(f0), true>(wb, 0, bop, a0, lane, f0);
      TRACE(200 + 10 * ltag);
      auto f1 = [&](int ks) { epi_pair(a0, 0, ks, w, ghb, tq, fq4); fillv(1, ks); };
      gemm_rb1<NKS, decltype(f1), true>(wb, 1, bop, a1, lane, f1);
      TRACE(201 + 10 * ltag);
      auto f2 = [&](int ks) { epi_pair(a1, 1, ks, w, ghb, tq, fq4); fillv(2, ks); };
      gemm_rb1<NKS, decltype(f2), true>(wb, 2, bop, a2, lane, f2);
      TRACE(202 + 10 * ltag);
      auto f3 = [&](int ks) { epi_pair(a2, 2, ks, w, ghb, tq, fq4); fillv(3, ks); };
      gemm_rb1<NKS, decltype(f3), true>(wb, 3, bop, a3, lane, f3);
      TRACE(203 + 10 * ltag);
#pragma unroll
      for (int q = 0; q < 8; ++q) epi_pair(a3, 3, q, w, ghb, tq, fq4);
      TRACE(204 + 10 * ltag);
    };
    auto dwdx_layer = [&](auto base_tag, const char* wb, const bf16x8 (&bop)[NKS], const DmaJob& jb, const u32x4 (&w)[NRB * 2],
                          bf16x8 (&ghb)[NKS], const float* tq, float& dbacc) {
      constexpr int BASE = decltype(base_tag)::value;
      constexpr bool G1ST = L0X && BASE == 0;
      unsigned long long g1b = 0;
      if constexpr (G1ST) {
        g1b = (unsigned long long)(a.g1 + ((size_t)(tile - t_first) * gridDim.x + blockIdx.x) * (NKS * 4096));
        g1b = ((unsigned long long)(unsigned)__builtin_amdgcn_readfirstlane((int)(g1b >> 32)) << 32) |
              (unsigned)__builtin_amdgcn_readfirstlane((int)(unsigned)g1b);
        asm volatile("" : "+s"(g1b));
      }
      auto g1_store = [&](int c) {
        unsigned t = (unsigned)tid16;
        asm volatile("" : "+v"(t));
        const unsigned off = ((t ^ ((t >> 3) & 64u)) ^ (unsigned)((c & 1) << 7)) + (unsigned)(c * 4096);
        asm volatile("global_store_dwordx4 %0, %1, %2" :: "v"(off), "v"(ghb[c]), "s"(g1b) : "memory");
      };
      const TsBase bA = ts_base(TA, lane), bB = ts_base(TB, lane);
      auto fx = [&](int i) { return *(const bf16x8*)(wb + (((i >> 3) * NKS + (i & 7)) * 64 + lane) * 16); };
      constexpr int D = 2;
      bf16x8 q[D];
#pragma unroll
      for (int d = 0; d < D; ++d) q[d] = fx(d);
      bf16x8 fa = ts_read(bA, wave, 0), fan = fa, fb0 = ts_read(bB, 0, 0), fb1 = ts_read(bB, 1, 0), fb2 = ts_read(bB, 2, 0), fb3 = ts_read(bB, 3, 0);
      f32x16 a0, a1, a2, a3;
      f32x4 fq4;
      auto slot = [&](auto ic, f32x16& acc, const f32x16& accp) {
        constexpr int i = decltype(ic)::value, rb = i >> 3, ks = i & 7, kk = i >> 2, m = i & 3;
        const bf16x8 ax = q[i % D];
        if (i + D < 32) q[i % D] = fx(i + D);
        if (ks == 0) mfma_bf16_zero_v<false>(acc, ax, bop[ks]);
        else if (ks == 7) mfma_bf16_pin_v<true, false, TAIL_DWDX>(acc, ax, bop[ks]);
        else mfma_bf16_pin_v<false, false>(acc, ax, bop[ks]);
        if constexpr (rb >= 1) epi_pair(accp, rb - 1, ks, w, ghb, tq, fq4);
        __builtin_amdgcn_sched_barrier(0);
        const bf16x8 bx = m == 0 ? fb0 : m == 1 ? fb1 : m == 2 ? fb2 : fb3;
        if (i == 31) mfma_bf16_agpr_tile<BASE + m, true, TAIL_DWDX_A>(fa, bx);
        else mfma_bf16_agpr_tile<BASE + m, false>(fa, bx);
        if constexpr (kk < 7) {
          if (m == 0) { fb0 = ts_read(bB, 0, kk + 1); fan = ts_read(bA, wave, kk + 1); }
          else if (m == 1) fb1 = ts_read(bB, 1, kk + 1);
          else if (m == 2) fb2 = ts_read(bB, 2, kk + 1);
          else fb3 = ts_read(bB, 3, kk + 1);
        }
        if constexpr (m == 3) { dbacc = frag_sum<PolBF16>(fa, dbacc); fa = fan; }
        if constexpr (i % 4 == 2 && i / 4 < DG) dma_group(jb, i / 4, wave, NW);
        if constexpr (G1ST && i >= 12 && i % 4 == 0) g1_store((i - 12) / 4);
        __builtin_amdgcn_sched_barrier(0);
      };
      static_for_up<0, 8>([&](auto ic) { slot(ic, a0, a0); });
      static_for_up<8, 16>([&](auto ic) { slot(ic, a1, a0); });
      static_for_up<16, 24>([&](auto ic) { slot(ic, a2, a1); });
      static_for_up<24, 32>([&](auto ic) { slot(ic, a3, a2); });
      if constexpr (G1ST) g1_store(5);
#pragma unroll
      for (int qq = 0; qq < 8; ++qq) epi_pair(a3, 3, qq, w, ghb, tq, fq4);
      if constexpr (G1ST) { g1_store(6); g1_store(7); }
    };
    auto load_phases = [&](const StashAt& sl, u32x4 (&w)[NRB * 2]) {
#pragma unroll
      for (int c = 0; c < NRB * 2; ++c) {
        w[c] = *stash_chunk(sl, c);
      }
      __builtin_amdgcn_sched_barrier(0);
    };
#pragma unroll
    for (int c = 0; c < NRB * 2; ++c) wA[c] = qst[c];
    {
      bf16x8 gyb[2];
#pragma unroll
      for (int e = 0; e < 8; ++e) { gyb[0][e] = (__bf16)((e < 3) ? gy[e] : 0.f); gyb[1][e] = (__bf16)0.f; }
      if constexpr (DW) {
        if constexpr (!LACC) {
          const float s0 = wave_sum(gy[0]), s1 = wave_sum(gy[1]), s2 = wave_sum(gy[2]);
          if (lane == 0) {
            f32x4 o = *(f32x4*)(hdb + 4 * wave);
            o[0] += s0; o[1] += s1; o[2] += s2;
            *(f32x4*)(hdb + 4 * wave) = o;
          }
        }
        ts_write<NRB>(TA, hb, wq * 32 + jx, hix);
        if constexpr (L0X) {
          const unsigned gbase = ts_write_base(TB, wq * 32 + jx, hix);
          u32x2 zz;
          asm volatile("v_mov_b32 %0, 0\n\tv_mov_b32 %1, 0" : "=v"(zz[0]), "=v"(zz[1]));
          const u32x4 w0 = __builtin_bit_cast(u32x4, gyb[0]);
          *(lds_u32x2_p)(uintptr_t)(gbase) = u32x2{w0[0], w0[1]};
          *(lds_u32x2_p)(uintptr_t)(gbase ^ 16u) = zz;
          *(lds_u32x2_p)(uintptr_t)(gbase ^ 32u) = zz;
          *(lds_u32x2_p)(uintptr_t)(gbase ^ 48u) = zz;
        } else
        ts_write<1>(TB, gyb, wq * 32 + jx, hix);
      }
      dma_wait();
      if constexpr (DW) __syncthreads();
      TRACE(7);
      if constexpr (!KEEP1) load_phases(stash_mid(L - 1), wB);
      if constexpr (DW) {
        f32x16 ah[1];
        float dbh = 0.f;
        TRACE(91);
        const int lane_h = L0X ? (int)((unsigned)lane16 >> 4) : lane;
        dw_gemm_s<1, DW_L0, 2>(TA, TB, ah, dbh, wave, lane_h);
        TRACE(92);
        if (j < 3) {
          float old[16];
#pragma unroll
          for (int r = 0; r < 16; ++r) old[r] = hdw[j * H + 32 * wave + rowmap(r, hi)];
#pragma unroll
          for (int r = 0; r < 16; ++r) hdw[j * H + 32 * wave + rowmap(r, hi)] = old[r] + ah[0][r];
        }

        TRACE(93);
      }
      const char* wb = HB;
      const bf16x8 g1[1] = {gyb[0]};
#pragma unroll
      for (int rbi = 0; rbi < NRB; rbi += 2)
        dx_rowblock_g(wb, rbi, g1, std::integral_constant<int, 1>{}, NoFill{}, wA, gA, FILM ? ftab + L * 2 * H : nullptr);
    }
    float dre[3] = {0.f, 0.f, 0.f};
    auto step = [&](int l, bf16x8 (&gb)[NKS], bf16x8 (&ghb)[NKS], u32x4 (&wph)[NRB * 2], u32x4 (&wnx)[NRB * 2]) {
      const bool LASTSTEP = L0X && l == 2;
      const int k = 2 * L + 2 - l;
      TRACE(20 + l);
      if constexpr (!FILM && !STATS && !L0X) {
        if (l == 1 && L >= 2) {
          const bf16x8 bop = bop0;
#pragma unroll
          for (int rbo = 0; rbo < NRB; ++rbo) {
            f32x16 acc;
            mfma_bf16_zero_v<true>(acc, __builtin_bit_cast(bf16x8, wph[2 * rbo]), bop);
#pragma unroll
            for (int c = 0; c < 2; ++c) {
              u32x4 w;
#pragma unroll
              for (int d = 0; d < 4; ++d)
                w[d] = phase_pack(red(acc[8 * c + 2 * d]), red(acc[8 * c + 2 * d + 1]));
              wph[2 * rbo + c] = w;
            }
          }
        }
      }
      if (DW && FILM && l == 1) {
        char* gp = a.g1 + ((size_t)(tile - t_first) * gridDim.x + blockIdx.x) * (NKS * 4096);
#pragma unroll
        for (int c = 0; c < NKS; ++c) {
          *(bf16x8*)(gp + c * 4096 + (unsigned)tid16) = gb[c];
        }
      }
      TRACE(30 + l);
      if (DW && l >= 2) {
        __syncthreads();
        TRACE(40 + l);
        ts_write<NRB>(TA, gb, wave * 32 + jx, hix);
        TRACE(80 + l);
        const unsigned hbase = ts_write_base(TB, wave * 32 + jx, hix);
#pragma unroll
        for (int c = 0; c < NRB * 2; ++c) {
          bf16x8 hv;
#pragma unroll
          for (int d = 0; d < 4; ++d) {
            hv[2 * d] = (__bf16)__builtin_amdgcn_sinf(phase_lo(wph[c][d]));
            hv[2 * d + 1] = (__bf16)__builtin_amdgcn_sinf(phase_hi(wph[c][d]));
          }
          ts_write_chunk(hbase, hv, c);
        }
      }
      TRACE(50 + l);
      dma_wait();
      __syncthreads();
      TRACE(60 + l);
      if (!DW && l >= 2) {
        if constexpr (!FILM) {
          load_phases(l == 2 ? StashAt{(gchar*)(unsigned long long)(a.afrag + (size_t)b * (NRB * 1024)), (unsigned)lane16} : stash_mid(l - 2), wnx);
        } else {
          load_phases(stash_mid(l - 2), wnx);
        }
      }
      DmaJob jb = make_job(k + 1 < nstep ? k + 1 : 0, LASTSTEP);
      if (k + 1 >= nstep && last_tile) jb.ng = 0;
      TRACE(70 + l);
      const StashAt sl_nx = [&]() -> StashAt {
        if constexpr (L0X) { if (l == 2) return StashAt{(gchar*)(unsigned long long)(a.afrag + (size_t)(last_tile ? cur_b : nxt_b) * (NRB * 1024)), (unsigned)lane16}; }
        if constexpr (DW && !FILM && !L0X) { if (l == 2) return StashAt{(gchar*)(unsigned long long)(a.afrag + (size_t)b * (NRB * 1024)), (unsigned)lane16}; }
        return stash_mid(l >= 2 ? l - 2 : 0);
      }();
      if constexpr (DW) load_phases(sl_nx, wnx);
      if constexpr (!L0X) { if (l == 1) load_d(dre); }
      if constexpr (L0X) { if (l == 2) dma_dirs(last_tile ? cur_b : nxt_b, last_tile ? cur_tin : nxt_tin); }
      if constexpr (L0X) { if (l == L) dma_tw(last_tile ? cur_b : nxt_b, last_tile ? cur_tin : nxt_tin); }
      const char* wb = smem + ((k ^ (L0X ? wpar_v : 0)) & 1) * GP::WBSZ;
      const float* const tq_prev = FILM ? ftab + (l - 1) * 2 * H : nullptr;
      {
        const bool had_dw = DW && l >= 2;
        auto fillv = [&](int rb, int ks) {
          if (!had_dw && rb == 0 && ks < DG) dma_group(jb, ks, wave, NW);
          if constexpr (DW && !FILM) {
            if (l == 1 && (ks & 3) == 2) {
              const int c = 2 * rb + (ks >> 2);
              *(bf16x8*)(a.g1 + ((size_t)(tile - t_first) * gridDim.x + blockIdx.x) * (NKS * 4096) + (size_t)((unsigned)tid16 + (unsigned)(c * 4096))) = gb[c];
            }
          }
        };
        TRACE(190 + l);
        if constexpr (DW) {
          switch (l) {
            case 5: dwdx_layer(std::integral_constant<int, 12>{}, wb, gb, jb, wph, ghb, tq_prev, pdb[4]); break;
            case 4: dwdx_layer(std::integral_constant<int, 8>{}, wb, gb, jb, wph, ghb, tq_prev, pdb[3]); break;
            case 3: dwdx_layer(std::integral_constant<int, 4>{}, wb, gb, jb, wph, ghb, tq_prev, pdb[2]); break;
            case 2: dwdx_layer(std::integral_constant<int, 0>{}, wb, gb, jb, wph, ghb, tq_prev, pdb[1]); break;
            default: if constexpr (!L0X) dx_layer(wb, gb, fillv, wph, ghb, tq_prev, l); break;
          }
        } else {
          dx_layer(wb, gb, fillv, wph, ghb, tq_prev, l);
        }
      }
    };
    {
      if constexpr (L0X) {
        int l = L;
#pragma unroll 1
        do { step(l, gA, gB, wB, wA); step(l - 1, gB, gA, wA, wB); } while ((l -= 2) >= 3);
      } else {
      int l = L;
      if ((L & 1) == 0) {
        step(l, gA, gB, wB, wA);
        --l;
#pragma unroll
        for (int c = 0; c < NKS; ++c) gA[c] = gB[c];
#pragma unroll
        for (int c = 0; c < NRB * 2; ++c) wB[c] = wA[c];
      }
#pragma unroll 1
      for (; l >= 3; l -= 2) { step(l, gA, gB, wB, wA); step(l - 1, gB, gA, wA, wB); }
      step(1, gA, gB, wB, wA);
      }
    }
    bf16x8 (&gb)[NKS] = gB;
    TRACE(8);
    if constexpr (L0X) {
      asm volatile("s_waitcnt vmcnt(8)" ::: "memory");
#pragma unroll
      for (int rbo = 0; rbo < NRB; ++rbo) aop0_n[rbo] = __builtin_bit_cast(bf16x8, wB[2 * rbo]);
      wpar_v ^= 1;
    } else
    {
      bf16x8 xcb[2];
#pragma unroll
      for (int e = 0; e < 8; ++e) { xcb[0][e] = (__bf16)0.f; xcb[1][e] = (__bf16)0.f; }
      {
        __bf16 xh[5], xl[4];
        split_x(dre, xh, xl);
        if (hi == 0) {
#pragma unroll
          for (int k2 = 0; k2 < 4; ++k2) { xcb[0][k2] = xh[k2]; xcb[0][4 + k2] = xl[k2]; }
        } else {
          xcb[0][0] = (__bf16)1.f;
        }
      }
#pragma unroll
      for (int hsel = 0; hsel < NHALF; ++hsel) {
        if (hsel > 0) __syncthreads();
        if (half == hsel) {
          ts_write<NRB>(TA, gb, wq * 32 + j, hi);
          ts_write<1>(TB, xcb, wq * 32 + j, hi);
        }
        if (hsel == 0) {
          if constexpr (DW && !FILM) asm volatile("s_waitcnt vmcnt(8)" ::: "memory");
          else dma_wait();
          if constexpr (INCR) {
            prefetch_tile(tile0 + t_step, last_tile ? cur_b : nxt_b, last_tile ? cur_tin : nxt_tin);
          } else if constexpr (PREF) prefetch_tile(tile0 + t_step);
        }
        TRACE(94);
        __syncthreads();
        TRACE(95);
        if (half == hsel) {
          f32x16 accA[1];
          float dummy = 0.f;
          dw_gemm_s<1, DW_L0, 2>(TA, TB, accA, dummy, wq, lane);
          TRACE(96);
          int lane_o = lane;
          asm volatile("" : "+v"(lane_o));
          if constexpr (DW) {
            float* const dl = dAacc + (32 * wq + 4 * (lane_o >> 5)) * 8 + (lane_o & 31);
            float add[16];
#pragma unroll
            for (int r = 0; r < 16; ++r) {
              const float lo = __builtin_bit_cast(float, __builtin_amdgcn_update_dpp(0, __builtin_bit_cast(int, accA[0][r]), 0x108, 0xf, 0xf, true));
              add[r] = accA[0][r] + (((lane_o & 31) < 4) ? lo : 0.f);
            }
            if ((lane_o & 31) < 8) {
              float old[16];
#pragma unroll
              for (int r = 0; r < 16; ++r) old[r] = dl[((r & 3) + 8 * (r >> 2)) * 8];
#pragma unroll
              for (int r = 0; r < 16; ++r) dl[((r & 3) + 8 * (r >> 2)) * 8] = old[r] + add[r];
            }
          } else {
            if (tvalid) dw_flush<Pol, H, NRB, 1, DW_L0, 1>(accA, 0.f, a.dA_part + (size_t)tile * H * 8, nullptr, 16, true, wq, lane_o);
          }
        }
      }
    }
    if constexpr (DW) {
      if (last_tile || (INCR ? nxt_b : (tile0 + 1) / a.tiles_per_image) != b) {
        char* const run = (char*)(a.pruns + ((size_t)blockIdx.x * a.pkmax + run_k) * (H * 8 + 16));
        unsigned eb = (unsigned)((32 * wave + 4 * hi) * 8 + j) * 4u;
        asm volatile("" : "+v"(eb));
        if (!L0X && j < 8) {
#pragma unroll
          for (int r = 0; r < 16; ++r) {
            const unsigned e = eb + (unsigned)(((r & 3) + 8 * (r >> 2)) * 32);
            float* const q = (float*)((char*)dAacc + e);
            *(float*)(run + e) = *q;
            *q = 0.f;
          }
        }
        if constexpr (LACC) {
          float ev = 0.f;
          if (hi == 0) { ev = lacc[wave * 32 + j][0]; lacc[wave * 32 + j][0] = 0.f; }
          const float es = wave_sum(ev);
          if (lane == 0) *(float*)(run + (H * 8 + wave) * 4) = es;
        } else {
          if (lane == 0) { *(float*)(run + (H * 8 + wave) * 4) = loss_run[wave]; loss_run[wave] = 0.f; }
        }
        if (tid == 0) a.prun_image[blockIdx.x * a.pkmax + run_k] = b;
        if constexpr (FILM) {
          const size_t slot = (size_t)blockIdx.x * a.pkmax + run_k;
          float* const dwr = a.dwp + slot * a.dwp_per_wg;
          float* const fr = a.dfr + slot * (size_t)L * 2 * H;
          for (int i = tid; i < 2 * H; i += 256) fr[i] = 0.f;
          if (a.need_dw && run_k > 0) {
            for (int i = tid; i < 3 * H; i += 256) dwr[a.p_off_w[L + 1] + i] = 0.f;
            if (tid < 3) dwr[a.p_off_b[L + 1] + tid] = 0.f;
          }
          asm volatile("s_nop 15\n\ts_nop 15" ::: "memory");
          int hio = hi, jo = j;
          asm volatile("" : "+v"(hio), "+v"(jo));
          auto film_flush = [&](auto lc) {
            constexpr int l = decltype(lc)::value;
            if (l <= L) {
              f32x16 t[MYB_H] = {agpr_read_tile<4 * (l - 2) + 0>(), agpr_read_tile<4 * (l - 2) + 1>(),
                                 agpr_read_tile<4 * (l - 2) + 2>(), agpr_read_tile<4 * (l - 2) + 3>()};
              const float* const tq = ftab + l * 2 * H;
              const float* const Wl = a.params + a.n_first + a.p_off_w[l];
              float dbs = pdb[l - 1];
              dbs += __shfl_xor(dbs, 32, 64);
#pragma unroll
              for (int r = 0; r < 16; ++r) {
                const int row = 32 * wave + rowmap(r, hio);
                float pr = 0.f;
#pragma unroll
                for (int m = 0; m < MYB_H; ++m) pr = __builtin_fmaf(Wl[(unsigned)(row * H + 32 * m + jo)], t[m][r], pr);
                pr = half_sum(pr);
                const float fq = tq[row] * 6.283185307179586f;
                if (jo == r) fr[(unsigned)((l - 1) * 2 * H + row)] = (fq != 0.f) ? pr / fq : 0.f;
              }
              if (hio == 0) {
                const int row = 32 * wave + jo;
                const float fq = tq[row] * 6.283185307179586f;
                fr[(unsigned)((l - 1) * 2 * H + H + row)] = (fq != 0.f) ? dbs / fq : 0.f;
              }
              if (a.need_dw) dw_flush<Pol, H, NRB, NRB, DW_HIDDEN, MYB_H>(t, pdb[l - 1], dwr + a.p_off_w[l], dwr + a.p_off_b[l], H, true, wave, hio * 32 + jo);
              agpr_zero_range<64 * (l - 2)>(std::make_integer_sequence<int, 64>{});
              pdb[l - 1] = 0.f;
            }
          };
          film_flush(std::integral_constant<int, 2>{});
          film_flush(std::integral_constant<int, 3>{});
          film_flush(std::integral_constant<int, 4>{});
          film_flush(std::integral_constant<int, 5>{});
        }
        ++run_k;
      }
    }
    if constexpr (INCR) { cur_b = nxt_b; cur_tin = nxt_tin; }
    TRACE(9);
  }
  int tid_e = L0X ? (int)((unsigned)tid16 >> 4) : tid;
  asm volatile("" : "+v"(tid_e));
  if constexpr (DW) {
    for (int k = run_k + tid_e; k < a.pkmax; k += 256) a.prun_image[blockIdx.x * a.pkmax + k] = -1;
  }
  if constexpr (DW && FILM) {
    if (a.need_dw) {
      if constexpr (LACC) {
        f32x4 v = f32x4{0.f, 0.f, 0.f, 0.f};
        if ((tid_e & 63) < 32) v = lacc[(tid_e >> 6) * 32 + (tid_e & 31)];
        const float s0 = wave_sum(v[1]), s1 = wave_sum(v[2]), s2 = wave_sum(v[3]);
        if ((tid_e & 63) == 0) { float* o = hdb + 4 * (tid_e >> 6); o[0] = s0; o[1] = s1; o[2] = s2; }
      }
      __syncthreads();
      float* const dw0 = a.dwp + (size_t)blockIdx.x * a.pkmax * a.dwp_per_wg;
      for (int i = tid_e; i < 3 * H; i += 256) dw0[a.p_off_w[L + 1] + i] = hdw[i];
      if (tid_e < 3) dw0[a.p_off_b[L + 1] + tid_e] = (hdb[tid_e] + hdb[4 + tid_e]) + (hdb[8 + tid_e] + hdb[12 + tid_e]);
    }
  } else if constexpr (DW) {
// ... 440 lines not shown
```

### reni_amd/csrc/reni_internal.h

```cpp
#pragma once
#include <hip/hip_runtime.h>
#include <stddef.h>
#include <stdint.h>

#include "../../include/reni_hip.h"

namespace reni {

constexpr int MAX_LAYERS = 15;

struct MainArgs {
  int B, P, tiles_per_image, n_tiles;
  int L, last_linear, act, loss_kind, need_dw;
  int dbg;
  float w_first, w_hidden, beta;
  float gy_scale;
  const float* Z;
  const float* D;
  long long d_bstride;
  const float* Apre;
  const char* afrag;
  const char* wimg;
  unsigned fwd_off[MAX_LAYERS + 2];
  unsigned bwd_off[MAX_LAYERS + 2];
  const float* target;
  long long ts0, ts1, ts2;
  const float* weight;
  long long ws0, ws1, ws2;
  const float* dout;
  const float* stats;
  float* out;
  char* stash;
  size_t stash_per_wg;
  float* dwp;
  size_t dwp_per_wg;
  unsigned p_off_w[MAX_LAYERS + 2];
  unsigned p_off_b[MAX_LAYERS + 2];
  float* dA_part;
  float* loss_part;
  char* g1;
  float* dw1p;
  long long* trace;
  const float* film;
  float* dfp_part;
  const float* params;
  unsigned n_first;
  char* dws;
  char* gfs;
  float* dfr;
  int* run_image;
  int kmax;
  float* pruns;
  int* prun_image;
  int pkmax;
  int nwg_main;
  const int* tlist;
  const int* tcount;
  const int* plist;
  const int* nlive;
};

int reni_set_error(int code, const char* msg);
void note_launches(int n);
inline int hip_status() {
  const hipError_t e = hipGetLastError();
  return e != hipSuccess ? reni_set_error(RENI_EHIP, hipGetErrorString(e)) : RENI_OK;
}

hipError_t launch_main_f32(int H, int mode, const MainArgs& a, int nwg, hipStream_t s);
hipError_t launch_main_bf16(int H, int mode, const MainArgs& a, int nwg, hipStream_t s);
hipError_t launch_film_f32(int H, int mode, const MainArgs& a, int nwg, hipStream_t s);
hipError_t launch_film_bf16(int H, int mode, const MainArgs& a, int nwg, hipStream_t s);
hipError_t launch_train_film(int which, const MainArgs& a, int grid, hipStream_t s);
hipError_t launch_dw1_film(const MainArgs& a, int grid, hipStream_t s);
int train_film_lds_bytes(int which);
hipError_t launch_wide256(int which, const MainArgs& a, int grid, hipStream_t s);
int wide256_film_max_layers();
int wide256_film_train_max_layers();
hipError_t launch_wide_head_dw(const MainArgs& a, int grid, hipStream_t s);

struct PrepArgs {
  const long long* idx;
  long long n_rows;
  float* Zc;
  long long* idx_copy;
  const float* Z;
  const float* W0;
  const float* b0;
  float* xconst;
  float* A;
  char* afrag;
  float afrag_scale;
  int eq, nd, F_in, H;
};

struct PackDesc {
  unsigned src;
  unsigned bias_src;
  unsigned dst;
  int M, K;
  int transposed;
  int nrb, nks;
  int bias_n, bias_n_pad;
  float scale;
};

struct PackArgs {
  const float* params;
  char* wimg;
  PackDesc d[2 * (MAX_LAYERS + 1)];
};

struct TailArgs {
  const float* dA;
  const float* W0;
  const float* Z;
  const float* xconst;
  float* mcol;
  float* ucol;
  float* dZ;
  float* dW0;
  float* db0;
  float alpha2;
  int eq, nd, F_in, H, B;
};

constexpr int MAX_MAP_LAYERS = 8;
struct FilmGlueArgs {
  const float* Z;
  const float* params;
  const float* mparams;
  float* A;
  float* film;
  float* mapm;
  float* mapx;
  float* fo;
  const float* dA;
  const float* dfilm;
  float* dAb;
  float* dly;
  float* dZ;
  float alpha2;
  int eq, nd, H, L, F0, M_in, Hm, ML, N_out, B;
  unsigned mw_off[MAX_MAP_LAYERS + 1], mb_off[MAX_MAP_LAYERS + 1];
  unsigned dly_off[MAX_MAP_LAYERS + 1];
};

}
```

### reni_amd/ops.py

```python
from __future__ import annotations

import ctypes
import math
import types
from typing import Optional, Tuple

import torch

from . import _lib


def _require_cuda(*tensors):
    for t in tensors:
        if t is not None and not t.is_cuda:
            raise _lib.RENILibraryError(
                "RENI HIP ops need tensors on a GPU device (got a CPU tensor); there is no CPU fallback")


def _f32c(t: torch.Tensor) -> torch.Tensor:
    if t.dtype != torch.float32:
        t = t.float()
    return t.contiguous()


def _loss_views(target, weight, B, P):
    target = (target if target.dtype == torch.float32 else target.float()).expand(B, P, 3)
    weight = (weight if weight.dtype == torch.float32 else weight.float()).expand(B, P, 3)
    return target, weight, (ctypes.c_int64 * 3)(*target.stride()), (ctypes.c_int64 * 3)(*weight.stride())


def _sparse_flags(sparse_weight):
    if sparse_weight not in (False, True, None, "tiles", "pixels"):
        raise ValueError('sparse_weight must be False, True / "tiles", or "pixels"')
    return _lib.WEIGHT_COMPACT if sparse_weight == "pixels" else _lib.WEIGHT_SPARSE if sparse_weight else 0


def _call(fn, device, *args):
    with torch.cuda.device(device):
        _lib.check(fn(*args, torch.cuda.current_stream(device).cuda_stream))


class Plan:

    def __init__(self, equivariance: str, ndims: int, hidden_features: int, hidden_layers: int,
                 out_features: int = 3, last_layer_linear: bool = True, output_activation=None,
                 first_omega_0: float = 30.0, hidden_omega_0: float = 30.0, dtype: str = "f32",
                 conditioning: str = "concat", mapping_layers: int = 0, mapping_features: int = 0):
        lib = _lib.load()
        if equivariance not in _lib.EQ:
            raise ValueError(f"equivariance {equivariance!r}")
        if output_activation not in _lib.ACT:
            raise ValueError(f"output_activation {output_activation!r}")
        self.desc = _lib.reni_desc(_lib.EQ[equivariance], ndims, hidden_features, hidden_layers, out_features,
                                   1 if last_layer_linear else 0, _lib.ACT[output_activation],
                                   float(first_omega_0), float(hidden_omega_0), _lib.DTYPE[dtype],
                                   {"concat": _lib.COND_CONCAT, "film": _lib.COND_FILM}[conditioning],
                                   int(mapping_layers), int(mapping_features))
        self.conditioning = conditioning
        self.hidden_features = hidden_features
        self.hidden_layers = hidden_layers
        self._h = ctypes.c_void_p()
        _lib.check(lib.reni_plan_create(ctypes.byref(self.desc), ctypes.byref(self._h)))
        self.lib = lib
        self.ndims = ndims
        self.dtype = dtype
        self.n_params = int(lib.reni_param_count(self._h))
        self.n_map_params = int(lib.reni_film_map_param_count(self._h))
        self.in_features = int(lib.reni_in_features(self._h))
        self.n_first = hidden_features * self.in_features + hidden_features
        self._ws = {}

    def __del__(self):
        try:
            if getattr(self, "_h", None) and self._h.value:
                self.lib.reni_plan_destroy(self._h)
                self._h = ctypes.c_void_p()
        except Exception:
            pass

    def workspace(self, B: int, P: int, flags: int, device) -> torch.Tensor:
        n = int(self.lib.reni_workspace_bytes(self._h, B, P, flags))
        if n == 0:
            raise _lib.RENILibraryError("reni_workspace_bytes returned 0 (unsupported configuration)")
        key = (torch.device(device).index, )
        ws = self._ws.get(key)
        if ws is None or ws.numel() < n:
            ws = torch.empty(n + 256, dtype=torch.uint8, device=device)
            self._ws[key] = ws
        self._ws_gen = getattr(self, "_ws_gen", 0) + 1
        return ws

    @staticmethod
    def _aligned_ptr(ws: torch.Tensor) -> Tuple[int, int]:
        p = ws.data_ptr()
        ap = (p + 255) & ~255
        return ap, ws.numel() - (ap - p)

    def _ws_args(self, B, P, flags, device):
        wp, wn = self._aligned_ptr(self.workspace(B, P, flags, device))
        return wp, wn, torch.cuda.current_stream(device).cuda_stream

    def launch_info(self, B: int, P: int):
        info = (ctypes.c_int32 * 4)()
        _lib.check(self.lib.reni_launch_info(self._h, B, P, info))
        return {"workgroups": info[0], "threads": info[1], "lds_bytes": info[2], "tiles": info[3]}

    def path_info(self, B: int, P: int, need_dw: bool = True, need_dz: bool = True):
        info = (ctypes.c_int32 * 8)()
        flags = (_lib.NEED_DW if need_dw else 0) | (_lib.NEED_DZ if need_dz else 0)
        _lib.check(self.lib.reni_path_info(self._h, B, P, flags, info))
        env = [n for b, n in ((1, "RENI_NO_PERSIST"), (2, "RENI_NO_SIDE_STREAM"), (4, "RENI_FRAG_WS_CAP_MB"), (8, "RENI_DW1_OLD"),
                              (16, "RENI_NO_L0X")) if info[6] & b]
        return {"persistent_kernels": bool(info[0]), "dw1_kernel": ("none", "k_reni_dw1_ring", "k_reni_dw1", "k_reni_l0_ring")[info[1]],
                "side_stream": bool(info[2]), "images_per_chunk": info[3], "operand_stream": bool(info[4]),
                "fragment_stream": ("none", "bf16", "f32")[info[5]], "env_overrides": env, "workgroups": info[7]}

    def _grid_args(self, Z, D):
        B = Z.shape[0]
        if D.dim() == 2:
            D = D.unsqueeze(0)
        if D.shape[0] not in (1, B):
            raise ValueError(f"directions batch {D.shape[0]} does not match latent batch {B}")
        P = D.shape[1]
        dbs = 0 if D.shape[0] == 1 or D.stride(0) == 0 else P * 3
        if dbs == 0:
            D = D[:1]
        return B, P, _f32c(D), dbs

    def _check_zp(self, Z, params, map_params=None):
        if Z.dim() != 3 or tuple(Z.shape[1:]) != (self.ndims, 3):
            raise ValueError(f"Z must be [B,{self.ndims},3], got {tuple(Z.shape)}")
        if params.numel() != self.n_params:
            raise ValueError(f"params must hold {self.n_params} floats, got {params.numel()}")
        if map_params is not None and map_params.numel() != self.n_map_params:
            raise ValueError(f"map_params must hold {self.n_map_params} floats, got {map_params.numel()}")

    def forward(self, Z: torch.Tensor, D: torch.Tensor, params: torch.Tensor) -> torch.Tensor:
        _require_cuda(Z, D, params)
        Z = _f32c(Z); params = _f32c(params)
        self._check_zp(Z, params)
        B, P, Dc, dbs = self._grid_args(Z, D)
        out = torch.empty(B, P, 3, dtype=torch.float32, device=Z.device)
        wp, wn, stream = self._ws_args(B, P, 0, Z.device)
        _lib.check(self.lib.reni_forward(self._h, B, P, Z.data_ptr(), Dc.data_ptr(), dbs, params.data_ptr(),
                                         out.data_ptr(), wp, wn, stream))
        return out

    def forward_loss_backward(self, Z, D, params, target, weight, loss_kind="mse", alpha=0.0, beta=0.0,
                              need_dw=True, need_dz=True, want_out=False, idx=None, sparse_weight=False):
        _require_cuda(Z, D, params, target, weight, idx)
        Z = _f32c(Z); params = _f32c(params)
        self._check_zp(Z, params)
        if idx is not None:
            if idx.dtype != torch.int64 or idx.dim() != 1 or idx.numel() < 1:
                raise ValueError("idx must be a non-empty 1-D int64 tensor")
            idx = idx.contiguous()
            B, P, Dc, dbs = self._grid_args(Z[:1].expand(idx.numel(), -1, -1), D)
        else:
            B, P, Dc, dbs = self._grid_args(Z, D)
        target, weight, ts, wst = _loss_views(target, weight, B, P)
        flags = (_lib.NEED_DW if need_dw else 0) | (_lib.NEED_DZ if need_dz else 0) | _sparse_flags(sparse_weight)
        dev = Z.device
        loss_terms = torch.empty(4, dtype=torch.float32, device=dev)
        dZ = torch.empty(B, self.ndims, 3, dtype=torch.float32, device=dev) if need_dz else None
        dparams = torch.empty(self.n_params, dtype=torch.float32, device=dev) if need_dw else None
        out = torch.empty(B, P, 3, dtype=torch.float32, device=dev) if want_out else None
        wp, wn, stream = self._ws_args(B, P, flags, dev)
        kind = _lib.LOSS_KIND[loss_kind]
        tail = (Dc.data_ptr(), dbs, params.data_ptr(), target.data_ptr(), ts, weight.data_ptr(), wst, kind, float(alpha),
                float(beta), flags, out.data_ptr() if out is not None else None, loss_terms.data_ptr(),
                dZ.data_ptr() if dZ is not None else None, dparams.data_ptr() if dparams is not None else None, wp, wn, stream)
        if idx is not None:
            _lib.check(self.lib.reni_forward_loss_backward_rows(self._h, B, P, Z.data_ptr(), Z.shape[0], idx.data_ptr(), *tail))
        else:
            _lib.check(self.lib.reni_forward_loss_backward(self._h, B, P, Z.data_ptr(), *tail))
        return loss_terms, dZ, dparams, out

    def train_step(self, Z_table, idx, D, params, target, weight, m_dec, v_dec, m_lat, v_lat, step, lr, stage_state, idx_next=None,
                   loss_kind="mse", alpha=0.0, beta=0.0, betas=(0.9, 0.999), eps=1e-8, grad_scale=1.0, comm=None, overlap=False):
        _require_cuda(Z_table, D, params, target, weight, idx, idx_next, m_dec, v_dec, m_lat, v_lat)
        for t in (Z_table, params, m_dec, v_dec, m_lat, v_lat):
            if t.dtype != torch.float32 or not t.is_contiguous():
                raise ValueError("train_step updates its buffers in place: contiguous float32 tensors only")
        self._check_zp(Z_table, params)
        for ix in (idx, idx_next):
            if ix is not None and (ix.dtype != torch.int64 or ix.dim() != 1 or ix.numel() != idx.numel() or not ix.is_contiguous()):
                raise ValueError("idx / idx_next must be contiguous 1-D int64 tensors of the same length")
        B, P, Dc, dbs = self._grid_args(Z_table[:1].expand(idx.numel(), -1, -1), D)
        target, weight, ts, wst = _loss_views(target, weight, B, P)
        dev = Z_table.device
        loss_terms = torch.empty(4, dtype=torch.float32, device=dev)
        dZ = torch.empty(B, self.ndims, 3, dtype=torch.float32, device=dev)
        dparams = torch.empty(self.n_params, dtype=torch.float32, device=dev)
        if stage_state.value & 1 and getattr(self, "_stage_gen", None) != (getattr(self, "_ws_gen", 0), dev.index):
            stage_state.value = 0
        wp, wn, stream = self._ws_args(B, P, _lib.NEED_DW | _lib.NEED_DZ, dev)
        self._stage_gen = (self._ws_gen, dev.index)
        kind = _lib.LOSS_KIND[loss_kind]
        head = (self._h, B, P, Z_table.data_ptr(), Z_table.shape[0], idx.data_ptr(), idx_next.data_ptr() if idx_next is not None else None,
                Dc.data_ptr(), dbs, params.data_ptr(), target.data_ptr(), ts, weight.data_ptr(), wst, kind, float(alpha), float(beta),
                m_dec.data_ptr(), v_dec.data_ptr(), m_lat.data_ptr(), v_lat.data_ptr(), float(lr), float(betas[0]), float(betas[1]),
                float(eps), int(step), float(grad_scale))
        tail = (ctypes.byref(stage_state), loss_terms.data_ptr(), dZ.data_ptr(), dparams.data_ptr(), wp, wn, stream)
        with torch.cuda.device(dev):
            if comm is not None:
                _lib.check(self.lib.reni_train_step_rows_dp(*head, comm._comm, 1 if overlap else 0, *tail))
            else:
                _lib.check(self.lib.reni_train_step_rows(*head, *tail))
        return loss_terms, dZ, dparams

    def weight_lists(self, B, P, weight, mode):
        try:
            version = weight._version
        except RuntimeError:
            return None
        key = (weight.data_ptr(), version, tuple(weight.shape), tuple(weight.stride()), int(B), int(P), int(mode), weight.device.index)
        cache = self.__dict__.setdefault("_wlists", {})
        hit = cache.get("key") == key
        if not hit:
            n = int(self.lib.reni_weight_lists_bytes(B, P))
            buf = cache.get("buf")
            if buf is None or buf.numel() < n + 256 or buf.device != weight.device:
                buf = torch.empty(n + 256, dtype=torch.uint8, device=weight.device)
            lp = (buf.data_ptr() + 255) & ~255
            wst = (ctypes.c_int64 * 3)(*weight.stride())
            summary = (ctypes.c_int32 * 3)()
            _call(self.lib.reni_weight_lists_build, weight.device, B, P, weight.data_ptr(), wst, int(mode), lp,
                  buf.numel() - (lp - buf.data_ptr()), summary)
            cache.update(key=key, buf=buf, ptr=lp, weight=weight, cos_constant=summary[2] == 0,
                         summary=tuple(summary))
        return cache["ptr"], (_lib.WEIGHT_COS_CONSTANT if cache["cos_constant"] else 0)

    def invalidate_weight_lists(self):
        self.__dict__.pop("_wlists", None)

    def latent_step(self, Z_table, idx, D, params, target, weight, m_lat, v_lat, step, lr, loss_kind="test", alpha=0.0, beta=0.0,
                    betas=(0.9, 0.999), eps=1e-8, sparse_weight=False, cache_lists=True):
        _require_cuda(Z_table, D, params, target, weight, idx, m_lat, v_lat)
        for t in (Z_table, m_lat, v_lat):
            if t.dtype != torch.float32 or not t.is_contiguous():
                raise ValueError("latent_step updates its buffers in place: contiguous float32 tensors only")
        params = _f32c(params)
        self._check_zp(Z_table, params)
        if idx.dtype != torch.int64 or idx.dim() != 1 or idx.numel() < 1 or not idx.is_contiguous():
            raise ValueError("idx must be a non-empty contiguous 1-D int64 tensor")
        flags = _sparse_flags(sparse_weight)
        B, P, Dc, dbs = self._grid_args(Z_table[:1].expand(idx.numel(), -1, -1), D)
        target, weight, ts, wst = _loss_views(target, weight, B, P)
        dev = Z_table.device
        loss_terms = torch.empty(4, dtype=torch.float32, device=dev)
        dZ = torch.empty(B, self.ndims, 3, dtype=torch.float32, device=dev)
        wp, wn, stream = self._ws_args(B, P, _lib.NEED_DZ | flags, dev)
        kind = _lib.LOSS_KIND[loss_kind]
        head = (self._h, B, P, Z_table.data_ptr(), Z_table.shape[0], idx.data_ptr(), Dc.data_ptr(), dbs, params.data_ptr(),
                target.data_ptr(), ts, weight.data_ptr(), wst, kind, float(alpha), float(beta), flags)
        tail = (m_lat.data_ptr(), v_lat.data_ptr(), float(lr), float(betas[0]), float(betas[1]), float(eps), int(step),
                loss_terms.data_ptr(), dZ.data_ptr(), wp, wn, stream)
        chunked = False
        if flags:
            cc = self.__dict__.setdefault("_chunk_cache", {})
            if (B, P) not in cc:
                cc[(B, P)] = self.path_info(B, P, need_dw=False)["images_per_chunk"] < B
            chunked = cc[(B, P)]
        if flags and cache_lists and not chunked:
            wl = self.weight_lists(B, P, weight, flags)
# ... 1546 lines not shown
```

Before: 1.248 billion.

## Share swizzled forward weight image for backward transposed reads in L0X train path

New measurement: 1.278 billion, median of 6. +2.4%, better.

```diff
diff --git a/reni_amd/csrc/reni_capi.inc b/reni_amd/csrc/reni_capi.inc
--- a/reni_amd/csrc/reni_capi.inc
+++ b/reni_amd/csrc/reni_capi.inc
@@ -25,6 +25,7 @@
   unsigned mw_off[reni::MAX_MAP_LAYERS + 1], mb_off[reni::MAX_MAP_LAYERS + 1];
   int no_persist, no_side_stream, dw1_old;
   int no_l0x;
+  int train_wg;
   int env_overrides;
   size_t frag_ws_cap;
 };
@@ -139,6 +140,7 @@
     const int rounds = (l.n_tiles + cap - 1) / cap;
     l.nwg = (l.n_tiles + rounds - 1) / rounds;
   }
+  if (l.pdw && p->train_wg > 0 && p->train_wg < l.nwg) l.nwg = p->train_wg;
   if (l.nwg < 1) l.nwg = 1;
   size_t o = 0;
   for (int st = 0; st < 2; ++st) {
@@ -395,7 +397,7 @@
 
 int run_prologue(const reni_plan* p, const GeoRt& g, const Layout& l, int64_t B, const float* Z,
                  const float* params, char* ws, bool backward, hipStream_t s, const int64_t* idx = nullptr,
-                 const float* film_A = nullptr, int64_t n_rows = 0) {
+                 const float* film_A = nullptr, int64_t n_rows = 0, bool shared_img = false) {
   const int H = p->d.hidden_features, L = p->d.hidden_layers;
   const bool film = p->d.conditioning == RENI_COND_FILM;
   reni::PrepArgs pa;
@@ -417,14 +419,14 @@
     const bool head = (i == L + 1);
     reni::PackDesc d;
     d.src = p->p_off_w[i]; d.bias_src = p->p_off_b[i]; d.dst = l.fwd_off[i];
-    d.M = head ? 3 : H; d.K = H; d.transposed = 0;
+    d.M = head ? 3 : H; d.K = H; d.transposed = 0; d.swz = (shared_img && !head) ? 1 : 0;
     d.nrb = head ? 1 : g.nrb; d.nks = g.nks;
     d.bias_n = head ? 3 : H; d.bias_n_pad = head ? 32 : H;
     d.scale = (l.persist && !head && !film) ? p->d.hidden_omega_0 * 0.15915494309189535f : 1.f;
     if (film && l.persist && H == 256 && !head) d.scale = 0.15915494309189535f;
     ka.d[n++] = d;
-    if (backward) {
-      d.dst = l.bwd_off[i]; d.transposed = 1;
+    if (backward && !(shared_img && i >= 2 && !head)) {
+      d.dst = l.bwd_off[i]; d.transposed = 1; d.swz = 0;
       d.nrb = g.nrb; d.nks = head ? g.head_bwd_ks : g.nks;
       d.bias_n = 0; d.bias_n_pad = 0;
       d.scale = !l.persist ? 1.f : film ? ((i == 1 || H == 256) ? 1.f : 6.283185307179586f) : (i == 1 ? p->d.first_omega_0 : p->d.hidden_omega_0);
@@ -645,6 +647,7 @@
   hipStream_t s, se;
   const float* Z;
   int stage_in;
+  bool staged_shared;
   float *img_loss, *stats, *dA, *part2;
   ListDst ld;
   reni::LayerScale lsc;
@@ -701,6 +704,7 @@
   const BwdCall& c = x.c;
   const bool staged = c.fuse && (*c.fuse->state & 1u);
   x.stage_in = staged ? (int)((*c.fuse->state >> 1) & 1u) : -1;
+  x.staged_shared = staged && ((*c.fuse->state >> 2) & 1u);
   x.l = make_layout(x.p, x.g, c.B, c.P, c.flags, true, true, staged ? x.stage_in : 0);
   const Layout& l = x.l;
   if (c.ws_bytes < l.total) return fail(RENI_EWORKSPACE, "workspace too small: need %zu bytes, got %zu", l.total, c.ws_bytes);
@@ -746,6 +750,13 @@
   }
   a.loss_kind = (c.loss_kind == LOSS_DOUT) ? LOSS_DOUT : (call_uses_cos(c) ? 1 : 0);
   x.path = bwd_path(x.p, x.l, c, a, x.stage_in);
+  if (x.path.l0x) {
+    const int L = x.p->d.hidden_layers;
+    float up = 1.f;
+    for (int i = 1; i < L; ++i) { up *= 8.f; x.lsc.c[i] /= up; }
+    a.gy_scale *= up;
+    x.lsc.c[L] /= up;
+  }
 }
 
 int bwd_weight_lists(Bwd& x) {
@@ -969,8 +980,8 @@
   RENI_LAUNCH(reni::k_adam2, dim3((unsigned)(ad.nb_dec + (ad.tn + 255) / 256 + ad.nb_l1)), dim3(256), 0, s, ad);
   if (fu.idx_next) {
     const Layout ln = make_layout(p, x.g, c.B, c.P, c.flags, true, true, 1 - path.stage);
-    if (const int rc = run_prologue(p, x.g, ln, c.B, fu.table, fu.params, x.ws, true, s, fu.idx_next, nullptr, c.n_rows)) return rc;
-    *fu.state = 1u | ((uint32_t)(1 - path.stage) << 1);
+    if (const int rc = run_prologue(p, x.g, ln, c.B, fu.table, fu.params, x.ws, true, s, fu.idx_next, nullptr, c.n_rows, path.l0x)) return rc;
+    *fu.state = 1u | ((uint32_t)(1 - path.stage) << 1) | (path.l0x ? 4u : 0u);
   }
   return RENI_OK;
 }
@@ -984,7 +995,8 @@
   if ((rc = bwd_layout(x))) return rc;
   bwd_layer_scales(x);
   bwd_main_args(x);
-  if (!x.path.staged && (rc = run_prologue(p, x.g, x.l, c.B, c.Z, c.params, x.ws, true, x.s, c.idx, c.fio ? c.fio->A : nullptr, c.n_rows))) return rc;
+  if (x.path.staged && x.staged_shared != x.path.l0x) x.path.staged = false;
+  if (!x.path.staged && (rc = run_prologue(p, x.g, x.l, c.B, c.Z, c.params, x.ws, true, x.s, c.idx, c.fio ? c.fio->A : nullptr, c.n_rows, x.path.l0x))) return rc;
   if ((rc = bwd_weight_lists(x))) return rc;
   if ((rc = bwd_stats_pass(x))) return rc;
   rc = x.l.persist ? launch_train(p, x.a, x.l.nwg, x.s, false, x.path.l0x) : launch_main(p, reni::MODE_FWD_BWD, x.a, x.l.nwg, x.s);
@@ -1250,6 +1262,7 @@
     }
   }
   if (const char* e = getenv("RENI_FRAG_WS_CAP_MB")) { const long long mb = atoll(e); if (mb > 0) { p->frag_ws_cap = (size_t)mb << 20; p->env_overrides |= 4; } }
+  if (const char* e = getenv("RENI_TRAIN_WG")) { const int n = atoi(e); if (n > 0) { p->train_wg = n; p->env_overrides |= 32; } }
   p->env_overrides |= (p->no_persist ? 1 : 0) | (p->no_side_stream ? 2 : 0) | (p->dw1_old ? 8 : 0) | (p->no_l0x ? 16 : 0);
   const int nd = d->ndims, H = d->hidden_features, L = d->hidden_layers;
   if (d->conditioning == RENI_COND_FILM) {
diff --git a/reni_amd/csrc/reni_dev_small.inc b/reni_amd/csrc/reni_dev_small.inc
--- a/reni_amd/csrc/reni_dev_small.inc
+++ b/reni_amd/csrc/reni_dev_small.inc
@@ -384,7 +384,8 @@
         else { if (Fk < d.M && R < d.K) val = a.params[d.src + (size_t)Fk * d.K + R]; }
         o[e] = (__bf16)(val * d.scale);
       }
-      *(bf16x8*)(a.wimg + d.dst + (size_t)t * 16) = o;
+      const int cell = d.swz ? (t ^ ((hi << 2) | ((ks & 1) << 3))) : t;
+      *(bf16x8*)(a.wimg + d.dst + (size_t)cell * 16) = o;
     } else {
       const int Fk = kfeat<Pol>(ks, hi, 0);
       float val = 0.f;
diff --git a/reni_amd/csrc/reni_dev_train.inc b/reni_amd/csrc/reni_dev_train.inc
--- a/reni_amd/csrc/reni_dev_train.inc
+++ b/reni_amd/csrc/reni_dev_train.inc
@@ -67,6 +67,11 @@
 }
 constexpr int DMA_GROUPS = 3;
 struct NoFill { DEV void operator()(int) const {} DEV void operator()(int, int) const {} };
+DEV int wimg_cell(int lane, int ks) { return lane ^ (((lane >> 5) << 2) | ((ks & 1) << 3)); }
+DEV unsigned wimg_tr_base(int lane) {
+  const int khi = lane >> 5, g = (lane >> 4) & 1, u = lane & 15, h = u & 1;
+  return (unsigned)(g * 1024 + h * 512 + (((4 * khi + (u >> 2)) ^ (4 * h + 8 * g)) << 4) + ((u >> 1) & 1) * 8);
+}
 
 template <int NKS>
 DEV f32x16 gemm_rb(const char* wb, int rbo, const bf16x8 (&bop)[NKS], f32x16 acc, int lane) {
@@ -85,10 +90,20 @@
   return acc;
 }
 
-template <int NKS, class F = NoFill, bool ZERO = false>
+template <int NKS, class F = NoFill, bool ZERO = false, bool SWZ = false>
 DEV void gemm_rb2(const char* wb, int rbo0, const bf16x8 (&bop)[NKS], f32x16& acc0, f32x16& acc1, int lane,
                   const F& fill = F()) {
-  auto fa = [&](int r, int ks) { return *(const bf16x8*)(wb + (((rbo0 + r) * NKS + ks) * 64 + lane) * 16); };
+  typedef __attribute__((address_space(3))) const bf16x8* lbp;
+  unsigned sb = SWZ ? (unsigned)(size_t)wb + (unsigned)(wimg_cell(lane, 0) * 16) : 0u, sb1 = sb ^ 0x80u;
+  if constexpr (SWZ) asm volatile("" : "+v"(sb), "+v"(sb1));
+  auto fa = [&](int r, int ks) {
+    if constexpr (SWZ) {
+      const unsigned ad = (ks & 1) ? sb1 : sb;
+      return *(lbp)(uintptr_t)(ad + (unsigned)(((rbo0 + r) * NKS + ks) * 1024));
+    } else {
+      return *(const bf16x8*)(wb + (((rbo0 + r) * NKS + ks) * 64 + lane) * 16);
+    }
+  };
   constexpr int D = NKS >= 2 ? 2 : 1;
   bf16x8 q0[D], q1[D];
 #pragma unroll
@@ -188,10 +203,10 @@
   asm volatile("" : "+v"(b.q[0]), "+v"(b.q[1]));
   return b;
 }
-DEV bf16x8 ts_read(const TsBase& b, int blk, int ks) {
+DEV bf16x8 ts_read(const TsBase& b, int blk, int ks, unsigned img_off = 0) {
   typedef __attribute__((address_space(3))) s16x4* lp;
-  const s16x4 lo = __builtin_amdgcn_ds_read_tr16_b64_v4i16((lp)(uintptr_t)((b.q[0] ^ (unsigned)(blk << 6)) + (unsigned)(ks * 4096)));
-  const s16x4 hi = __builtin_amdgcn_ds_read_tr16_b64_v4i16((lp)(uintptr_t)((b.q[1] ^ (unsigned)(blk << 6)) + (unsigned)(ks * 4096)));
+  const s16x4 lo = __builtin_amdgcn_ds_read_tr16_b64_v4i16((lp)(uintptr_t)((b.q[0] ^ (unsigned)(blk << 6)) + (unsigned)(ks * 4096) + img_off));
+  const s16x4 hi = __builtin_amdgcn_ds_read_tr16_b64_v4i16((lp)(uintptr_t)((b.q[1] ^ (unsigned)(blk << 6)) + (unsigned)(ks * 4096) + img_off));
   typedef short s16x8 __attribute__((ext_vector_type(8)));
   const s16x8 v = {lo[0], lo[1], lo[2], lo[3], hi[0], hi[1], hi[2], hi[3]};
   return __builtin_bit_cast(bf16x8, v);
@@ -284,7 +299,6 @@
   float* const dwp = a.dwp + (size_t)blockIdx.x * a.dwp_per_wg;
   const int L = a.L;
   const int nstep = L0X ? 2 * L + 1 : 2 * L + 2;
-  int wpar_v = 0;
 
   static_assert(MYB_H == 4, "sixteen AGPR tiles = 4 layers x 4 column blocks");
   if constexpr (DW) agpr_zero_seq(std::make_integer_sequence<int, 256>{});
@@ -311,10 +325,14 @@
   int lane16 = lane * 16, tid16 = tid * 16;
   const char* wimg_f1 = a.wimg + a.fwd_off[1];
   const char* wimg_b1 = a.wimg + a.bwd_off[1];
-  auto make_job = [&](int k, bool next_tile = false) -> DmaJob {
+  auto make_job = [&](int k) -> DmaJob {
     if (k == L || k == L + 1) k = STATS ? 0 : L + 2;
-    const int wpar = L0X ? (wpar_v ^ (next_tile ? 1 : 0)) : 0;
-    const unsigned dst = __builtin_amdgcn_readfirstlane((unsigned)(size_t)(smem + ((k ^ wpar) & 1) * GP::WBSZ));
+    if constexpr (L0X) {
+      const int layer = k < L ? k + 1 : 2 * L + 2 - k;
+      const unsigned dst = __builtin_amdgcn_readfirstlane((unsigned)(size_t)(smem + ((layer - 1) & 1) * GP::WBSZ));
+      return DmaJob{wimg_f1 + (unsigned)(layer - 1) * GP::FWD_STRIDE, (unsigned)lane16, dst, (G::IMG_HID + G::BIAS_HID + 3071) / 3072};
+    }
+    const unsigned dst = __builtin_amdgcn_readfirstlane((unsigned)(size_t)(smem + (k & 1) * GP::WBSZ));
     const char* img;
     int bytes;
     if constexpr (FILM && DW && !SPEC) {
@@ -410,6 +428,7 @@
     asm volatile("" : "+v"(lane16), "+v"(tid16));
     const int jx = L0X ? (int)(((unsigned)lane16 >> 4) & 31u) : j, hix = L0X ? (int)((unsigned)lane16 >> 9) : hi;
     const int j = jx, hi = hix;
+    const int lanex = L0X ? (int)((unsigned)lane16 >> 4) : lane;
     TRACE(1);
     const bool tvalid = tile0 + half < t_stop;
     const int tile = CONTIG ? (tvalid ? tile0 + half : t_stop - 1) : tile_pref;
@@ -575,12 +594,13 @@
       }
       TRACE(10 + l);
       DmaJob jb = make_job(l);
+      if (L0X && (l == L || (l == 1 && tile0 != t_first))) jb.ng = 0;
       if (STATS && l == L && ((L & 1) || last_tile)) jb.ng = 0;
       const StashAt sl_prev = stash_mid(l - 1);
       const float* const tp_prev = FILM ? ftab + (l - 1) * 2 * H : nullptr;
       const float* const tp_cur = FILM ? ftab + l * 2 * H : nullptr;
       FilmQ fs0, fsA, fsB;
-      const char* wb = smem + (((l - 1) ^ (L0X ? wpar_v : 0)) & 1) * GP::WBSZ;
+      const char* wb = smem + ((l - 1) & 1) * GP::WBSZ;
       const float* bias = (const float*)(wb + G::IMG_HID);
       auto fill = [&](int ks, int part) {
         if (part == 0 && ks < DG) dma_group(jb, ks, wave, NW);
@@ -628,16 +648,17 @@
         acc1[r] = bias[32 + rowmap(r, hi)];
       }
       TRACE(100 + l);
-      gemm_rb2<NKS>(wb, 0, hin, acc0, acc1, lane, fill);
+      gemm_rb2<NKS, std::decay_t<decltype(fill)>, false, L0X>(wb, 0, hin, acc0, acc1, lanex, fill);
       TRACE(110 + l);
-      gemm_rb2<NKS>(wb, 2, hin, poa, pob, lane, [&](int ks, int part) {
+      auto fill2 = [&](int ks, int part) {
         if constexpr (FILM) {
           if ((ks & 1) == 0) act_pair(acc0, 0, ks + part, hout, tp_cur, &fs0);
           else act_pair(acc1, 1, ks - 1 + part, hout, tp_cur, &fs0);
         } else {
           if (part == 0) act_pair(acc0, 0, ks, hout); else act_pair(acc1, 1, ks, hout);
         }
-      });
+      };
+      gemm_rb2<NKS, decltype(fill2), false, L0X>(wb, 2, hin, poa, pob, lanex, fill2);
       TRACE(120 + l);
       if (STATS && l == L && (L & 1) && !last_tile) {
         __syncthreads();
@@ -675,7 +696,7 @@
       f32x16 acc;
 #pragma unroll
       for (int r = 0; r < 16; ++r) acc[r] = bias[rowmap(r, hi)];
-      acc = gemm_rb<NKS>(wb, 0, hb, acc, lane);
+      acc = gemm_rb<NKS>(wb, 0, hb, acc, lanex);
 #pragma unroll
       for (int c = 0; c < 3; ++c) {
         ylin[c] = acc[c];
@@ -771,7 +792,7 @@
                              const float* tq = nullptr) {
       constexpr int NK = decltype(nks_tag)::value;
       f32x16 acc0, acc1;
-      gemm_rb2<NK, std::decay_t<decltype(fill)>, true>(wb, rbi, bop, acc0, acc1, lane, fill);
+      gemm_rb2<NK, std::decay_t<decltype(fill)>, true>(wb, rbi, bop, acc0, acc1, lanex, fill);
 #pragma unroll
       for (int r = 0; r < 16; r += 2) {
         float r0, r1;
@@ -840,13 +861,32 @@
         const unsigned off = ((t ^ ((t >> 3) & 64u)) ^ (unsigned)((c & 1) << 7)) + (unsigned)(c * 4096);
         asm volatile("global_store_dwordx4 %0, %1, %2" :: "v"(off), "v"(ghb[c]), "s"(g1b) : "memory");
       };
-      const TsBase bA = ts_base(TA, lane), bB = ts_base(TB, lane);
-      auto fx = [&](int i) { return *(const bf16x8*)(wb + (((i >> 3) * NKS + (i & 7)) * 64 + lane) * 16); };
+      const TsBase bA = ts_base(TA, lanex), bB = L0X ? bA : ts_base(TB, lanex);
+      auto rdB = [&](int m, int ks) { return L0X ? ts_read(bA, m, ks, (unsigned)GP::TSZ) : ts_read(bB, m, ks); };
+      unsigned xq = 0, xq1 = 0;
+      if constexpr (L0X) {
+        xq = lds_u32(wb) + wimg_tr_base(lanex);
+        xq1 = xq ^ 0x80u;
+        asm volatile("" : "+v"(xq), "+v"(xq1));
+      }
+      auto fx = [&](int i) {
+        if constexpr (L0X) {
+          typedef __attribute__((address_space(3))) s16x4* lp;
+          typedef short s16x8 __attribute__((ext_vector_type(8)));
+          const unsigned off = (unsigned)((i >> 3) * 2048 + ((i & 7) >> 1) * 8192 + (i & 1) * 256);
+          const s16x4 lo = __builtin_amdgcn_ds_read_tr16_b64_v4i16((lp)(uintptr_t)(xq + off));
+          const s16x4 up = __builtin_amdgcn_ds_read_tr16_b64_v4i16((lp)(uintptr_t)(xq1 + off));
+          const s16x8 v = {lo[0], lo[1], lo[2], lo[3], up[0], up[1], up[2], up[3]};
+          return __builtin_bit_cast(bf16x8, v);
+        } else {
+          return *(const bf16x8*)(wb + (((i >> 3) * NKS + (i & 7)) * 64 + lane) * 16);
+        }
+      };
       constexpr int D = 2;
       bf16x8 q[D];
 #pragma unroll
       for (int d = 0; d < D; ++d) q[d] = fx(d);
-      bf16x8 fa = ts_read(bA, wave, 0), fan = fa, fb0 = ts_read(bB, 0, 0), fb1 = ts_read(bB, 1, 0), fb2 = ts_read(bB, 2, 0), fb3 = ts_read(bB, 3, 0);
+      bf16x8 fa = ts_read(bA, wave, 0), fan = fa, fb0 = rdB(0, 0), fb1 = rdB(1, 0), fb2 = rdB(2, 0), fb3 = rdB(3, 0);
       f32x16 a0, a1, a2, a3;
       f32x4 fq4;
       auto slot = [&](auto ic, f32x16& acc, const f32x16& accp) {
@@ -862,10 +902,10 @@
         if (i == 31) mfma_bf16_agpr_tile<BASE + m, true, TAIL_DWDX_A>(fa, bx);
         else mfma_bf16_agpr_tile<BASE + m, false>(fa, bx);
         if constexpr (kk < 7) {
-          if (m == 0) { fb0 = ts_read(bB, 0, kk + 1); fan = ts_read(bA, wave, kk + 1); }
-          else if (m == 1) fb1 = ts_read(bB, 1, kk + 1);
-          else if (m == 2) fb2 = ts_read(bB, 2, kk + 1);
-          else fb3 = ts_read(bB, 3, kk + 1);
+          if (m == 0) { fb0 = rdB(0, kk + 1); fan = ts_read(bA, wave, kk + 1); }
+          else if (m == 1) fb1 = rdB(1, kk + 1);
+          else if (m == 2) fb2 = rdB(2, kk + 1);
+          else fb3 = rdB(3, kk + 1);
         }
         if constexpr (m == 3) { dbacc = frag_sum<PolBF16>(fa, dbacc); fa = fan; }
         if constexpr (i % 4 == 2 && i / 4 < DG) dma_group(jb, i / 4, wave, NW);
@@ -1002,8 +1042,9 @@
           load_phases(stash_mid(l - 2), wnx);
         }
       }
-      DmaJob jb = make_job(k + 1 < nstep ? k + 1 : 0, LASTSTEP);
+      DmaJob jb = make_job(k + 1 < nstep ? k + 1 : 0);
       if (k + 1 >= nstep && last_tile) jb.ng = 0;
+      if (L0X && l == L) jb.ng = 0;
       TRACE(70 + l);
       const StashAt sl_nx = [&]() -> StashAt {
         if constexpr (L0X) { if (l == 2) return StashAt{(gchar*)(unsigned long long)(a.afrag + (size_t)(last_tile ? cur_b : nxt_b) * (NRB * 1024)), (unsigned)lane16}; }
@@ -1014,7 +1055,7 @@
       if constexpr (!L0X) { if (l == 1) load_d(dre); }
       if constexpr (L0X) { if (l == 2) dma_dirs(last_tile ? cur_b : nxt_b, last_tile ? cur_tin : nxt_tin); }
       if constexpr (L0X) { if (l == L) dma_tw(last_tile ? cur_b : nxt_b, last_tile ? cur_tin : nxt_tin); }
-      const char* wb = smem + ((k ^ (L0X ? wpar_v : 0)) & 1) * GP::WBSZ;
+      const char* wb = smem + ((L0X ? l - 1 : k) & 1) * GP::WBSZ;
       const float* const tq_prev = FILM ? ftab + (l - 1) * 2 * H : nullptr;
       {
         const bool had_dw = DW && l >= 2;
@@ -1066,9 +1107,7 @@
     if constexpr (L0X) {
       asm volatile("s_waitcnt vmcnt(8)" ::: "memory");
 #pragma unroll
-      for (int rbo = 0; rbo < NRB; ++rbo) aop0_n[rbo] = __builtin_bit_cast(bf16x8, wB[2 * rbo]);
-      wpar_v ^= 1;
-    } else
+      for (int rbo = 0; rbo < NRB; ++rbo) aop0_n[rbo] = __builtin_bit_cast(bf16x8, wB[2 * rbo]);    } else
     {
       bf16x8 xcb[2];
 #pragma unroll
diff --git a/reni_amd/csrc/reni_internal.h b/reni_amd/csrc/reni_internal.h
--- a/reni_amd/csrc/reni_internal.h
+++ b/reni_amd/csrc/reni_internal.h
@@ -103,6 +103,7 @@
   int nrb, nks;
   int bias_n, bias_n_pad;
   float scale;
+  int swz;
 };
 
 struct PackArgs {
diff --git a/reni_amd/ops.py b/reni_amd/ops.py
--- a/reni_amd/ops.py
+++ b/reni_amd/ops.py
@@ -110,7 +110,7 @@
         flags = (_lib.NEED_DW if need_dw else 0) | (_lib.NEED_DZ if need_dz else 0)
         _lib.check(self.lib.reni_path_info(self._h, B, P, flags, info))
         env = [n for b, n in ((1, "RENI_NO_PERSIST"), (2, "RENI_NO_SIDE_STREAM"), (4, "RENI_FRAG_WS_CAP_MB"), (8, "RENI_DW1_OLD"),
-                              (16, "RENI_NO_L0X")) if info[6] & b]
+                              (16, "RENI_NO_L0X"), (32, "RENI_TRAIN_WG")) if info[6] & b]
         return {"persistent_kernels": bool(info[0]), "dw1_kernel": ("none", "k_reni_dw1_ring", "k_reni_dw1", "k_reni_l0_ring")[info[1]],
                 "side_stream": bool(info[2]), "images_per_chunk": info[3], "operand_stream": bool(info[4]),
                 "fragment_stream": ("none", "bf16", "f32")[info[5]], "env_overrides": env, "workgroups": info[7]}
```
